# MCG-NJU/SparseBEV

Hardware: AMD Instinct MI355X
Metric: decoder samples/sec (6-cam T=8 900q r50_704x256, 6 layers, features resident in HBM) (higher is better)
Workload: dtype f32 (the two mixing GEMMs: f16x3 = fp32-class (default): fp32 operands as scaled fp16 hi + lo images, 3 products (hl, lh, hh), f32 accumulate on the 16-bit matrix core (csrc/gemm_bf16s.hip); max and rms error vs fp64 below the exact f32 MFMA kernels (tests/test_gpu_bf16s.py); mixing generator + out-; 1 GPU; c2: r50_704x256, 900 queries, T=8, bs=1 per GPU, 6 decoder layers, random-init weights, NCHW (reference layout, relayout inside the step: on demand -- only the feature units the sample points read) feature input; global_batch=1, parallelism=sample-sharded x1, launches_per_layer=6, query_order=False, shuffled_queries=False, relayout=on-demand

## Files before the change

### include/sbev_hip.h

```cpp
#ifndef SBEV_HIP_H
#define SBEV_HIP_H

#include <stdint.h>

#ifdef __cplusplus
extern "C" {
#endif

#define SBEV_ABI_VERSION 1
#define SBEV_MAX_LEVELS 5
#define SBEV_MAX_POINTS 32
#define SBEV_MAX_FRAMES 16

typedef void* sbev_stream_t;

enum sbev_status {
    SBEV_OK = 0,
    SBEV_EINVAL = -1,
    SBEV_ELAUNCH = -2,
    SBEV_ENODEV = -3,
    SBEV_EFAULT = -4
};

enum sbev_dtype { SBEV_F32 = 0, SBEV_BF16 = 1, SBEV_F16 = 2, SBEV_U8 = 3 };
// ... 108 lines not shown
int sbev_adaptive_mixing_f32(const float* x, const float* params, float* y,
                             int64_t BQ, int G, int Pin, int C, int Pout, float eps, sbev_stream_t stream);

int sbev_sasa_f32(const float* qkvt, int64_t ld, const float* query_bbox, const double* pc_range,
                  const uint8_t* mask, float* out, int B, int Q, int H, int head_dim, sbev_stream_t stream);

int sbev_refine_bbox(const float* query_bbox, const float* reg, const float* vel_div, float* out,
                     int B, int Q, int code_size, sbev_stream_t stream);


int sbev_head_prepare(const float* init_query_bbox, const float* label_row, float* query_bbox, float* query_feat,
                      int B, int Q, int D, sbev_stream_t stream);

int sbev_head_denorm(const float* bbox_norm, const double* pc_range, float* out, int64_t n, sbev_stream_t stream);

int sbev_nms_free_decode(const float* cls_scores, const float* bbox_preds, int B, int Q, int num_classes, int max_num,
                         float score_threshold, int use_score_threshold, const double* post_center_range,
                         int bottom_center, float* boxes, float* scores, int32_t* labels, int32_t* count,
                         sbev_stream_t stream);


int sbev_head_dn_prepare(const float* init_query_bbox, const float* label_enc, const float* gt_boxes, const int32_t* gt_labels,
                         const int32_t* gt_offsets, const float* u_box, const float* u_lab, const int32_t* new_lab,
                         const double* pc_range, float box_noise_scale, float label_noise_scale, int B, int Q, int D,
                         int num_classes, int G, int N, int single, float* query_bbox, float* query_feat,
                         int32_t* noised_label, uint8_t* attn_mask, sbev_stream_t stream);

int sbev_head_dn_prepare_bwd(const float* grad_query_bbox, const float* grad_query_feat, const int32_t* noised_label,
                             const int32_t* gt_offsets, int B, int Q, int D, int num_classes, int G, int N, int single,
                             float* grad_init_query_bbox, float* grad_label_enc, sbev_stream_t stream);

int sbev_head_match_cost(const float* cls_scores, const float* bbox_preds, int64_t ld_rows, const float* gt_boxes,
                         const int32_t* gt_labels, const int32_t* gt_offsets, const float* code_weights, float w_cls,
                         float w_reg, float alpha, float gamma, int L, int B, int Q, int num_classes, int Gmax, float* cost,
                         sbev_stream_t stream);

int sbev_lsa_solve(const float* cost, int64_t ld, int n_rows, int n_cols, int32_t* col_of_row);

int sbev_head_assign(const float* cost, const int32_t* gt_counts, int L, int B, int Q, int Gmax, int32_t* assign);

int64_t sbev_head_assign_device_workspace(int L, int B, int Q, int Gmax);
int sbev_head_assign_device_plan(int Q, int Gmax);
int sbev_head_assign_device(const float* cost, const int32_t* gt_offsets, int L, int B, int Q, int Gmax,
                            int32_t* assign, int32_t* status, void* workspace, sbev_stream_t stream);

int sbev_head_capacity_plan(const int32_t* gt_offsets, int B, int Q, int capacity, int N, double bg_cls_weight, int32_t* codes,
                            float* avg_factors, int32_t* status, sbev_stream_t stream);

#define SBEV_OPTIM_CHUNK 8192
#define SBEV_OPTIM_MAX_TENSORS 64
#define SBEV_OPTIM_MAX_GROUPS 16
#define SBEV_OPTIM_HYPER_FLOATS 68
#define SBEV_OPTIM_HEADER_BYTES 64
int sbev_optim_plan(const int64_t* numel, int n, int64_t* out);
int sbev_optim_sumsq(const void* const* g, const int64_t* numel, int n, const float* hyper, float* partials, sbev_stream_t stream);
int sbev_optim_finish(const float* partials, int64_t n_partials, const float* hyper, void* header, double beta1, double beta2,
                      sbev_stream_t stream);
int sbev_optim_adamw(void* const* p, const void* const* g, void* const* m, void* const* v, const int64_t* numel, const int32_t* group,
                     int n, int n_groups, double beta1, double beta2, double eps, const float* hyper, const void* header,
                     sbev_stream_t stream);

int64_t sbev_head_set_loss_workspace(int B, int rows);

int sbev_head_set_loss(const float* cls_scores, const float* bbox_preds, int64_t ld_rows, const int32_t* codes,
                       int64_t code_layer_stride, const float* gt_boxes, const int32_t* gt_labels, const int32_t* gt_offsets,
                       const float* code_weights, const float* avg_factors, float w_focal, float alpha, float gamma,
                       float w_l1, float scale, int L, int B, int rows, int num_classes, float* loss, float* loss_finite,
                       float* grad_cls, float* grad_bbox, float* workspace, sbev_stream_t stream);


int sbev_nchw_to_nhwc_f32(const float* in, float* out, int64_t n_images, int channels, int hw, sbev_stream_t stream);

int sbev_nchw_to_nhwc_f32_indirect(const void* const* table, int index, float* out, int64_t n_images, int channels, int hw,
                                   sbev_stream_t stream);
int sbev_nchw_to_nhwc_f32_multi_indirect(const void* const* table, int n_levels, const int32_t* index, float* const* out,
                                         int64_t n_images, int channels, const int32_t* hw, sbev_stream_t stream);
int sbev_nchw_to_nhwc_b16(const void* in, void* out, int64_t n_images, int channels, int hw, sbev_stream_t stream);
int sbev_nchw_to_nhwc_b16_indirect(const void* const* table, int index, void* out, int64_t n_images, int channels, int hw,
                                   sbev_stream_t stream);
int sbev_copy_indirect(const void* const* table, int nseg, const int32_t* index, void* const* dst, const int64_t* nbytes,
                       sbev_stream_t stream);

int sbev_finish_outputs(const float* cls_src, const float* box_src, float* cls_dst, float* box_dst, int64_t n_cls, int64_t n_box,
                        sbev_stream_t stream);
int sbev_finish_outputs_indirect(const void* const* table, int idx_cls, int idx_box, const float* cls_src, const float* box_src,
                                 int64_t n_cls, int64_t n_box, sbev_stream_t stream);


int sbev_linear3_ln_relu_f32(const float* x, int64_t ldx, const float* w, const float* b,
                             const float* ln_w, const float* ln_b, float eps, float* y,
                             int64_t M, int N, sbev_stream_t stream);

int sbev_splitk_reduce_f32(const float* slabs, int splits, const float* bias, const float* residual,
                           const float* ln_w, const float* ln_b, float ln_eps, float* Y,
                           int64_t M, int N, int relu, sbev_stream_t stream);

int sbev_split_bf16x3_weights(const float* W, uint16_t* W2, int64_t N, int K, sbev_stream_t stream);
int sbev_linear_bf16x3(const float* X, const uint16_t* W2, const float* bias, const float* residual, float* Y,
                       int64_t M, int N, int K, int64_t ldx, int64_t ldy, int relu, sbev_stream_t stream);
int sbev_linear_bf16x3_strip_ok(int64_t M, int N, int K);
int sbev_linear_bf16x3_strip(const uint16_t* X2, const uint16_t* W2, const float* bias, float* Y, int64_t M, int N, int K,
                             int64_t ldy, int relu, sbev_stream_t stream);
int sbev_linear_splitk_bf16x3(const float* X, const uint16_t* W2, const float* bias, const float* residual,
                              const float* ln_w, const float* ln_b, float ln_eps, float* Y,
                              int64_t M, int N, int K, int64_t ldx, int relu, int splits, float* workspace,
                              sbev_stream_t stream);

int64_t sbev_bf16s_image_elems(int64_t rows, int K, int nimg);
int sbev_split_bf16s_rows(const float* X, int64_t ldx, uint16_t* out, int64_t rows, int K, int nimg, sbev_stream_t stream);
int sbev_pack_bf16s_frags(const float* W, int64_t ldw, uint16_t* out, int N, int K, int nimg, sbev_stream_t stream);
int sbev_linear_bf16s_gen_ok(int64_t M, int N, int K);
int sbev_linear_bf16s_gen(const uint16_t* Xs, const uint16_t* Ws, const float* bias, float* Y, int64_t M, int N, int K,
                          int64_t ldy, int relu, int nimg, sbev_stream_t stream);
int sbev_linear_bf16s_out_ok(int64_t M, int N, int K);
int sbev_linear_bf16s_out_plan(int64_t M, int N, int K);
int sbev_linear_gen_plan(int64_t M, int N, int K, int64_t ldy, int nimg, int weight_stationary, int cus, int32_t* out, int capacity);
int sbev_linear_splitk_bf16s(const float* X, const uint16_t* Wp, const float* bias, const float* residual,
                             const float* ln_w, const float* ln_b, float ln_eps, float* Y,
                             int64_t M, int N, int K, int64_t ldx, int relu, int nimg, float* workspace,
                             sbev_stream_t stream);

int sbev_pack_f16s_frags(const float* W, int64_t ldw, uint16_t* out, float* scales, int N, int K, int per_tensor, sbev_stream_t stream);
int sbev_linear_f16s_gen(const uint16_t* Xs, const float* xscale, const uint16_t* Ws, const float* wdown, const float* bias, float* Y,
                         int64_t M, int N, int K, int64_t ldy, int relu, int nprod, sbev_stream_t stream);

int sbev_linear_gen_weight_stationary(int enable);

int sbev_linear_splitk_f16s(const float* X, int x_is_pairs, int x_up_log2, const uint16_t* Wp, const float* nscale, const float* bias, const float* residual,
                            const float* ln_w, const float* ln_b, float ln_eps, float* Y,
                            int64_t M, int N, int K, int64_t ldx, int relu, int nprod, float* workspace, sbev_stream_t stream);
int sbev_f16s_out_scale(const float* wdown, int x_up_log2, float* nscale, int N, sbev_stream_t stream);
int sbev_linear_splitk_f16s_xdev(const float* X, const float* x_scale, const uint16_t* Wp, const float* wdown, const float* bias,
                                 const float* residual, const float* ln_w, const float* ln_b, float ln_eps, float* Y,
                                 int64_t M, int N, int K, int64_t ldx, int relu, int nprod, float* workspace, sbev_stream_t stream);
int sbev_f16s_pairs(const float* X, void* out, int64_t n, int up_log2, sbev_stream_t stream);
int sbev_f16s_tensor_scale(const float* X, int64_t ldx, int64_t rows, int K, float* updown, sbev_stream_t stream);
int sbev_adaptive_mixing_pairs_f16(const float* x, const float* params, void* y, int64_t BQ, int G, int Pin, int Cg, int Pout, float eps,
                                   int up_log2, sbev_stream_t stream);
int sbev_sample_mix_pairs_f16(const void* const* feats, const int32_t* hw, int L, int feat_dtype,
                              int64_t B, int N, int Q, int T, int G, int P, int Cg,
                              const int64_t* stride_bo, int64_t stride_g, const int64_t* stride_v, int64_t stride_px,
                              const float* loc, const float* weights, const int32_t* frame_slots, int n_slots,
                              const float* params, void* y, int Pout, float eps, int up_log2, sbev_stream_t stream);

int sbev_copy_widen_f32(const void* src, int src_dtype, float* dst, int64_t n, sbev_stream_t stream);

int sbev_sample_mix_supported(int L, int C, int P, int T, int gdiv, int G);
int sbev_sample_mix_slabs_ok(const int32_t* hw, int L, int feat_dtype, int N, int C, const int64_t* stride_v, int64_t stride_px);
int sbev_sample_mix_f32(const void* const* feats, const int32_t* hw, int L, int feat_dtype,
                        int64_t B, int N, int Q, int T, int G, int P, int C,
                        const int64_t* stride_bo, int64_t stride_g, const int64_t* stride_v, int64_t stride_px,
                        const float* loc, const float* weights, const int32_t* frame_slots, int n_slots,
                        const float* params, float* y, int Pout, float eps, sbev_stream_t stream);
int sbev_decoder_fuse_sample_mix(int enable);

int sbev_query_order_max(void);
int sbev_query_order(const float* query_bbox, int64_t ld, const double* pc_range, int B, int Q, int32_t* order, sbev_stream_t stream);
int sbev_sample_mix_f32_ordered(const void* const* feats, const int32_t* hw, int L, int feat_dtype,
                                int64_t B, int N, int Q, int T, int G, int P, int C,
                                const int64_t* stride_bo, int64_t stride_g, const int64_t* stride_v, int64_t stride_px,
                                const float* loc, const float* weights, const int32_t* frame_slots, int n_slots,
                                const float* params, float* y, int Pout, float eps, const int32_t* order, sbev_stream_t stream);
int sbev_sample_mix_pairs_f16_ordered(const void* const* feats, const int32_t* hw, int L, int feat_dtype,
                                      int64_t B, int N, int Q, int T, int G, int P, int Cg,
                                      const int64_t* stride_bo, int64_t stride_g, const int64_t* stride_v, int64_t stride_px,
                                      const float* loc, const float* weights, const int32_t* frame_slots, int n_slots,
                                      const float* params, void* y, int Pout, float eps, int up_log2, const int32_t* order,
                                      sbev_stream_t stream);
int sbev_decoder_query_order(int enable);
int sbev_sample_mix_pool(const void* const* feats, const int32_t* hw, int L, int feat_dtype,
                         int64_t B, int N, int Q, int T, int G, int P, int C,
                         const int64_t* stride_bo, int64_t stride_g, const int64_t* stride_v, int64_t stride_px,
                         const float* loc, const float* weights, const int32_t* frame_slots, const int32_t* slot_table_dev, int n_slots,
                         const float* params, void* y, int Pout, float eps, int y_pairs, int up_log2, const int32_t* order,
                         sbev_stream_t stream);


int64_t sbev_gemm_f32_workspace(int64_t M, int N, int64_t K);
int sbev_gemm_f32(const float* A, int a_kmajor, int64_t lda, const float* B, int b_kmajor, int64_t ldb,
                  float* C, int64_t ldc, int64_t M, int N, int64_t K, int accumulate,
                  float* workspace, sbev_stream_t stream);
int64_t sbev_gemm_f32_multi_workspace(int64_t M, int N, int64_t K, int nseg);
int sbev_gemm_f32_multi(const float* const* A, int a_kmajor, int64_t lda, const float* const* B, int b_kmajor, int64_t ldb,
                        int nseg, float* C, int64_t ldc, int64_t M, int N, int64_t K, int accumulate,
                        float* workspace, sbev_stream_t stream);

int sbev_gemm_tn_f16s_ok(int64_t M, int64_t N, int64_t K);
int sbev_gemm_tn_f16s(const float* A, int64_t lda, const float* a_scale, const float* B, int64_t ldb, const float* b_scale,
                      float* C, int64_t ldc, int64_t M, int64_t N, int64_t K, int accumulate, sbev_stream_t stream);

int64_t sbev_colsum_workspace(int64_t M, int N);
int sbev_bias_relu_bwd(const float* dY, const float* Y, float* dZ, float* db, int64_t M, int N, int64_t ld,
                       float* workspace, sbev_stream_t stream);

int64_t sbev_layer_norm_bwd_workspace(int64_t M, int N);
int sbev_layer_norm_bwd(const float* dY, const float* X, const float* gamma, const float* beta, float eps, int relu,
                        float* dX, float* dgamma, float* dbeta, float* workspace, int64_t M, int N, sbev_stream_t stream);
int sbev_layer_norm_bwd_rows(const float* dY, const float* X, const float* gamma, const float* beta, float eps, int relu,
                             float* dX, float* workspace, int64_t M, int N, sbev_stream_t stream);
int sbev_layer_norm_param_group(const float* const* dYs, const float* const* Xs, const float* const* stats,
                                const float* const* gammas, const float* const* betas, float* const* dgammas, float* const* dbetas,
                                const int32_t* Ns, const int32_t* nsegs, const int32_t* relus, const int32_t* accumulate,
                                int ng, int64_t M, sbev_stream_t stream);
int sbev_colsum_group(const float* const* segs, float* const* outs, const int32_t* Ns, const int32_t* nsegs,
                      const int32_t* accumulate, int ng, int64_t M, sbev_stream_t stream);
int sbev_bias_relu_bwd_acc(const float* dY, const float* Y, float* dZ, float* db, int64_t M, int N, int64_t ld,
                           float* workspace, int accumulate, sbev_stream_t stream);
int sbev_layer_norm_bwd_acc(const float* dY, const float* X, const float* gamma, const float* beta, float eps, int relu,
                            float* dX, float* dgamma, float* dbeta, float* workspace, int64_t M, int N, int accumulate, sbev_stream_t stream);

int sbev_linear3_ln_relu_ex_f32(const float* x, int64_t ldx, const float* w, const float* b,
                                const float* ln_w, const float* ln_b, float eps, float* y, float* pre,
                                int64_t M, int N, sbev_stream_t stream);

int sbev_adaptive_mixing_bwd_f32(const float* x, const float* params, const float* grad_y, float* grad_x, float* grad_params,
                                 int64_t BQ, int G, int Pin, int C, int Pout, float eps, sbev_stream_t stream);
int sbev_adaptive_mixing_bwd_max_f32(const float* x, const float* params, const float* grad_y, float* grad_x, float* grad_params,
                                     float* item_max, int64_t BQ, int G, int Pin, int C, int Pout, float eps, sbev_stream_t stream);

int sbev_sasa_train_fwd_f32(const float* qkvt, int64_t ld, const float* query_bbox, const double* pc_range,
                            const uint8_t* mask, float* out, int B, int Q, int H, int head_dim,
                            float attn_drop, uint64_t seed, sbev_stream_t stream);
int sbev_sasa_bwd_f32(const float* qkvt, int64_t ld, const float* query_bbox, const double* pc_range,
                      const uint8_t* mask, const float* out, const float* grad_out, float* grad_qkvt,
                      float* workspace, int B, int Q, int H, int head_dim, float attn_drop, uint64_t seed,
                      sbev_stream_t stream);

int sbev_msmv_bwd_ex(const void* const* feats, void* const* grad_feats, const int32_t* hw, int L,
                     int64_t Bp, int N, int C, int Q, int P,
                     int gdiv, const int64_t* stride_bo, int64_t stride_g, const int64_t* stride_v, int64_t stride_px,
                     const float* loc, const float* weights, const float* grad_out, int grad_out_layout, int T, int G,
                     float* grad_loc, float* grad_weights, sbev_stream_t stream);

int64_t sbev_msmv_bwd_tap_count(int64_t Bp, int Q, int P, int L);
int sbev_msmv_bwd_taps(const void* const* feats, const int32_t* hw, int L,
                       int64_t Bp, int N, int C, int Q, int P,
                       int gdiv, const int64_t* stride_bo, int64_t stride_g, const int64_t* stride_v, int64_t stride_px,
                       const float* loc, const float* weights, int64_t* keys, float* coefs, sbev_stream_t stream);
int sbev_msmv_bwd_sum_sorted(void* const* grad_feats, int L, const int64_t* sorted_keys, const int64_t* order,
                             const float* coefs, int64_t n, const float* grad_out, int grad_out_layout,
                             int64_t Bp, int C, int Q, int P, int T, int G, sbev_stream_t stream);

int sbev_project_select_bwd(const float* sample_points, const float* lidar2img, const float* grad_loc,
                            int B, int Q, int T, int N, int G, int P, float image_h, float image_w, float eps,
                            float* grad_points, sbev_stream_t stream);

int sbev_sampling_front_bwd(const float* query_bbox, const float* offset, int64_t ld_off, const float* logits, int64_t ld_logit,
                            const double* pc_range, int B, int Q, int T, int G, int P, int L,
                            const float* grad_points, const float* grad_weights_bp,
                            float* grad_offset, float* grad_logits, int64_t ld_grad, float* grad_bbox, sbev_stream_t stream);

int sbev_refine_bbox_bwd(const float* grad_out, const float* out, const float* query_bbox, const float* vel_div,
                         float* grad_reg, float* grad_bbox, int B, int Q, sbev_stream_t stream);

int sbev_dropout_f32(const float* x, float* y, int64_t n, uint64_t seed, float p, sbev_stream_t stream);

int sbev_sasa_train_fwd_f32_ds(const float* qkvt, int64_t ld, const float* query_bbox, const double* pc_range, const uint8_t* mask,
                               float* out, int B, int Q, int H, int head_dim, float attn_drop, uint64_t seed, const uint64_t* seed_dev,
                               sbev_stream_t stream);
int sbev_sasa_bwd_f32_ds(const float* qkvt, int64_t ld, const float* query_bbox, const double* pc_range, const uint8_t* mask,
                         const float* out, const float* grad_out, float* grad_qkvt, float* workspace, int B, int Q, int H, int head_dim,
                         float attn_drop, uint64_t seed, const uint64_t* seed_dev, sbev_stream_t stream);
int sbev_dropout_f32_ds(const float* x, float* y, int64_t n, uint64_t seed, const uint64_t* seed_dev, float p, sbev_stream_t stream);

typedef struct sbev_decoder_config {
    int32_t B, Q, T, N, G, P, L;
    int32_t D, H, ffn;
    int32_t num_classes, code_size, num_layers, out_points;
    int32_t attn_in_rows;
    int32_t feat_dtype;
    int32_t hw[SBEV_MAX_LEVELS][2];
    float image_h, image_w, eps_homo;
    int32_t gemm_mode;
    int32_t n_slots;
    int32_t frame_slots[SBEV_MAX_FRAMES];
    int32_t overlap;
    double pc_range[6];
    const int32_t* slot_table;
} sbev_decoder_config;

typedef struct sbev_decoder_weights {
    const float *pe0_w, *pe0_b, *pe1_g, *pe1_b, *pe3_w, *pe3_b, *pe4_g, *pe4_b;
    const float *attn_in_w, *attn_in_b;
    const float *attn_out_w, *attn_out_b;
    const float *samp_w, *samp_b;
    const float *pg_w, *pg_b, *op_w, *op_b;
    const uint16_t *pg_w2, *op_w2;
    const float *ffn0_w, *ffn0_b, *ffn1_w, *ffn1_b;
    const float *norm1_g, *norm1_b, *norm2_g, *norm2_b, *norm3_g, *norm3_b;
    const float *cls0_w, *cls0_b, *cls1_g, *cls1_b, *cls3_w, *cls3_b, *cls4_g, *cls4_b, *cls6_w, *cls6_b;
    const float *reg0_w, *reg0_b, *reg2_w, *reg2_b, *reg4_w, *reg4_b;
    const float *chain_pack;
    const uint16_t *pg_ws;
    const uint16_t *op_wp;
    const float *pg_wdown;
    const float *op_nscale;
    const float *pg_xscale;
} sbev_decoder_weights;

int64_t sbev_decoder_chain_pack_floats(const sbev_decoder_config* cfg);
int sbev_decoder_chain_pack(const sbev_decoder_config* cfg, const sbev_decoder_weights* weights, float* out, sbev_stream_t stream);
int sbev_decoder_row_chain(int enable);
int sbev_decoder_chain_plan(const sbev_decoder_config* cfg, int kind, int with_front, int pair_ok, int cus, int32_t* out, int capacity);

int sbev_decoder_chain_pair(int enable);
int64_t sbev_decoder_chain_pair_timeouts(void);
int64_t sbev_decoder_chain_pair_faults(void);
int64_t sbev_decoder_chain_pair_faults_ack(void);
int sbev_decoder_out_fold(int enable);
int sbev_linear_out8_min_rows(int rows);
int sbev_debug_out_fold_drop(int enable);
int sbev_init(void);
int sbev_debug_chain_pair_drop(int enable);

int sbev_decoder_launches_per_layer(const sbev_decoder_config* cfg, const sbev_decoder_weights* weights);

int sbev_decoder_switches(int32_t* out, int capacity);

int sbev_decoder_mixed_up_log2(const sbev_decoder_config* cfg);

int64_t sbev_decoder_workspace_bytes(const sbev_decoder_config* cfg);

int sbev_decoder_forward(const sbev_decoder_config* cfg, const sbev_decoder_weights* weights,
                         const void* const* feats_nhwc, const float* query_bbox, const float* query_feat,
                         const float* time_diff, const float* lidar2img, const float* vel_div,
                         const uint8_t* attn_mask, float* cls_out, float* bbox_out,
                         void* workspace, int64_t workspace_bytes, sbev_stream_t stream);

typedef struct sbev_lazy_feats {
    const void* const* table;
    int32_t index[SBEV_MAX_LEVELS];
    const void* src[SBEV_MAX_LEVELS];
} sbev_lazy_feats;
int sbev_decoder_lazy_supported(const sbev_decoder_config* cfg);
int sbev_decoder_lazy_scan_launch(int enable);
int sbev_decoder_forward_lazy(const sbev_decoder_config* cfg, const sbev_decoder_weights* weights, void* const* feats_nhwc,
                              const sbev_lazy_feats* lazy, const float* query_bbox, const float* query_feat,
                              const float* time_diff, const float* lidar2img, const float* vel_div,
                              const uint8_t* attn_mask, float* cls_out, float* bbox_out,
                              void* workspace, int64_t workspace_bytes, sbev_stream_t stream);
int64_t sbev_prefix_cache_bytes(const sbev_decoder_config* cfg);
int sbev_decoder_forward_cached(const sbev_decoder_config* cfg, const sbev_decoder_weights* weights, void* const* feats_nhwc,
                                const sbev_lazy_feats* lazy, const float* query_bbox, const float* query_feat,
                                const float* time_diff, const float* lidar2img, const float* vel_div,
                                const uint8_t* attn_mask, float* cls_out, float* bbox_out,
                                void* workspace, int64_t workspace_bytes, sbev_stream_t stream, void* cache, int64_t cache_bytes);
int sbev_decoder_prefix_planned(const sbev_decoder_config* cfg, const sbev_decoder_weights* weights, int cache_given, int mask_given,
                                int lazy_given);
int64_t sbev_lazy_relayout_tiles(int n_levels, const int32_t* hw_pixels, int64_t n_images, int channels);
int sbev_sample_and_project_touch(const float* query_bbox, const float* offset, int64_t ld_offset,
                                  const float* scale_logits, int64_t ld_logits,
                                  const float* time_diff, const float* lidar2img, const double* pc_range,
                                  int B, int Q, int T, int N, int G, int P, int L,
                                  float image_h, float image_w, float eps,
                                  float* loc_bp, float* weights_bp, const int32_t* hw, uint32_t* need, sbev_stream_t stream);
int sbev_nchw_to_nhwc_lazy(const void* const* table, const int32_t* index, const void* const* src, void* const* out, int n_levels,
                           const int32_t* hw_pixels, int64_t n_images, int channels, int dtype, uint32_t* need, uint32_t* done, int first,
                           int last, sbev_stream_t stream);

typedef struct sbev_graph sbev_graph;
int sbev_decoder_capture(const sbev_decoder_config* cfg, const sbev_decoder_weights* weights,
                         const void* const* feats_nhwc, const float* query_bbox, const float* query_feat,
                         const float* time_diff, const float* lidar2img, const float* vel_div,
                         const uint8_t* attn_mask, float* cls_out, float* bbox_out,
                         void* workspace, int64_t workspace_bytes, sbev_stream_t stream, sbev_graph** out);
int sbev_capture_begin(sbev_stream_t stream);
int sbev_capture_end(sbev_stream_t stream, sbev_graph** out);
int sbev_graph_launch(sbev_graph* graph, sbev_stream_t stream);
int64_t sbev_graph_num_nodes(const sbev_graph* graph);
int sbev_graph_destroy(sbev_graph* graph);

int sbev_profile_sampler(int enable);
int sbev_profile_sampler_read(float* ms, int max_n);
int sbev_profile_stride(int every_n_calls);
int sbev_profile_read(int kind, float* ms, int max_n);

enum sbev_frames_layout { SBEV_FRAMES_NCHW = 0, SBEV_FRAMES_NHWC = 1 };
int sbev_pool_insert_frames(const void* const* table, const int32_t* index, const void* const* src, void* const* out, int n_frames,
                            int n_levels, const int32_t* hw_pixels, int B, int n_views, int channels, int src_layout, int src_dtype,
                            int dst_dtype, const int32_t* insert, int n_slots, sbev_stream_t stream);

int sbev_pool_insert(const void* const* table, const int32_t* index, const void* const* src, void* const* out, int n_levels,
                     const int32_t* hw_pixels, int B, int n_views, int channels, int dtype, const int32_t* insert, int n_slots,
                     sbev_stream_t stream);

#define SBEV_FRONT_ROW_BYTES 64
int sbev_image_front_plan(int n, int H, int W, int div, int64_t* out);
int sbev_image_front(const void* src, int src_dtype, void* dst, int dst_dtype, int n, int H, int W, int div, const float* mean,
                     const float* std, int to_rgb, int colour_on, const void* table, sbev_stream_t stream);

#define SBEV_GEOM_KMAX 16
int sbev_image_geom_plan(int H, int W, int fH, int fW, int resize_w, int resize_h, int crop_x, int crop_y, int flip, int32_t* table_out,
                         int64_t* out);
int sbev_image_geom(const void* src, void* dst, int n, int H, int W, int fH, int fW, const void* table, const void* image_rows,
                    int n_transforms, sbev_stream_t stream);

#define SBEV_FPN_MAX_IN 4
#define SBEV_FPN_MAX_OUT 5
#define SBEV_FPN_PLAN_WORDS 18
int sbev_fpn_plan(int n_levels, const int32_t* chw, int64_t n, int num_outs, int64_t* out);
int sbev_fpn_pack_weights(int n_levels, const int32_t* chw, const void* const* lateral_w, const void* const* fpn_w, int w_dtype, void* pack,
                          sbev_stream_t stream);
int sbev_fpn_forward(int n_levels, const int32_t* chw, int64_t n, int num_outs, const void* const* inputs, int in_dtype, const void* pack,
                     const float* const* lateral_bias, const float* const* fpn_bias, void* workspace, void* const* outs, int out_dtype,
                     sbev_stream_t stream);

#define SBEV_FPN_GRAD_WINDOW_LOG2 3
#define SBEV_FPN_BWD_PLAN_WORDS 16
int sbev_fpn_backward_plan(int n_levels, const int32_t* chw, int64_t n, int num_outs, int want_input_grads, int64_t* out);
int sbev_fpn_pack_weights_bwd(int n_levels, const int32_t* chw, const void* const* lateral_w, const void* const* fpn_w, int w_dtype,
                              void* pack, sbev_stream_t stream);
int sbev_fpn_backward(int n_levels, const int32_t* chw, int64_t n, int num_outs, const void* const* inputs, int in_dtype,
                      const void* merged, const void* const* grad_outs, int g_dtype, const void* pack_bwd, void* workspace,
                      void* const* grad_inputs, float* const* grad_lateral_w, float* const* grad_lateral_bias, float* const* grad_fpn_w,
                      float* const* grad_fpn_bias, sbev_stream_t stream);

#define SBEV_RESNET_MAX_LAYERS 160
#define SBEV_RESNET_PLAN_HEAD 18
#define SBEV_RESNET_LAYER_WORDS 12
#define SBEV_RESNET_PLAN_WORDS (SBEV_RESNET_PLAN_HEAD + SBEV_RESNET_LAYER_WORDS * SBEV_RESNET_MAX_LAYERS)
int sbev_resnet_plan(int depth, const int32_t* stage_blocks, int num_stages, int base_channels, int64_t n, int H, int W, int n_out,
                     const int32_t* out_indices, int keep, int64_t* out);
int sbev_resnet_pack_weights(int n_layers, const int32_t* desc, const void* const* w, const float* const* gamma, const float* const* beta,
                             const float* const* mean, const float* const* var, float eps, int w_dtype, void* pack, sbev_stream_t stream);
int sbev_conv_f16(const void* x, const void* pack, const void* residual, void* y, int64_t n, int H, int W, int Cin, int Cout, int taps,
                  int stride, int epilogue, int col_tile, sbev_stream_t stream);
int sbev_resnet_forward(int depth, const int32_t* stage_blocks, int num_stages, int base_channels, int64_t n, int H, int W, int n_out,
                        const int32_t* out_indices, int keep, const void* x, int x_dtype, const void* pack, void* workspace,
                        void* const* outs, sbev_stream_t stream);

#define SBEV_RESNET_GRAD_WINDOW_LOG2 3
#define SBEV_RESNET_BWD_PLAN_HEAD 16
#define SBEV_RESNET_BWD_LAYER_WORDS 6
#define SBEV_RESNET_BWD_PLAN_WORDS (SBEV_RESNET_BWD_PLAN_HEAD + SBEV_RESNET_BWD_LAYER_WORDS * SBEV_RESNET_MAX_LAYERS)
int sbev_resnet_backward_plan(int depth, const int32_t* stage_blocks, int num_stages, int base_channels, int64_t n, int H, int W, int n_out,
                              const int32_t* out_indices, int first_trainable_stage, int64_t* out);
int sbev_resnet_forward_train(int depth, const int32_t* stage_blocks, int num_stages, int base_channels, int64_t n, int H, int W, int n_out,
                              const int32_t* out_indices, int first_trainable_stage, const void* x, int x_dtype, const void* pack,
                              void* workspace, void* acts, void* const* outs, sbev_stream_t stream);
int sbev_resnet_pack_weights_bwd(int n_layers, const int32_t* desc, const void* const* w, const float* const* gamma, const float* const* var,
                                 float eps, int w_dtype, void* pack, sbev_stream_t stream);
int sbev_resnet_backward(int depth, const int32_t* stage_blocks, int num_stages, int base_channels, int64_t n, int H, int W, int n_out,
                         const int32_t* out_indices, int first_trainable_stage, const void* acts, const void* const* outs,
                         const void* const* grad_outs, int g_dtype, const void* pack_bwd, void* workspace, const void* const* w, int w_dtype,
                         const float* const* gamma, const float* const* mean, const float* const* var, float eps, float* const* grad_w,
                         float* const* grad_gamma, float* const* grad_beta, sbev_stream_t stream);
int sbev_conv_dgrad_f16(const void* gy, const void* gy2, const void* pack, const void* mask, const void* res, const void* gp, int gp_dtype,
                        const float* scale, void* gx, int64_t n, int H, int W, int Cin, int Cout, int taps, int stride, int Cout2, int stride2,
                        int col_tile, sbev_stream_t stream);
int sbev_conv_wgrad_f16(const void* gy, const void* x, float* part, int64_t n, int H, int W, int Cin, int Cout, int taps, int stride,
                        int slab_len, sbev_stream_t stream);
int sbev_bn_fold_backward(const float* part, int slabs, const float* scale, const void* w, int w_dtype, const float* gamma, const float* mean,
                          const float* var, float eps, int Cin, int Cout, int taps, float* grad_w, float* grad_gamma, float* grad_beta,
                          sbev_stream_t stream);

#ifdef __cplusplus
}
#endif
#endif
```

### sparsebev_amd/_lib.py

```python
import ctypes
import os

import torch

_HERE = os.path.dirname(os.path.abspath(__file__))
LIB_PATH = os.environ.get('SBEV_LIB_PATH') or os.path.join(_HERE, 'csrc', 'libsbev_hip.so')

_c_i64p = ctypes.POINTER(ctypes.c_int64)
_c_i32p = ctypes.POINTER(ctypes.c_int32)
_vp = ctypes.c_void_p

SIGNATURES = {
    'sbev_abi_version': (ctypes.c_int, []),
    'sbev_set_box_convention': (ctypes.c_int, [ctypes.c_int]),
    'sbev_get_box_convention': (ctypes.c_int, []),
    'sbev_last_error': (ctypes.c_char_p, []),
    'sbev_device_count': (ctypes.c_int, []),
    'sbev_msmv_fwd': (ctypes.c_int, [ctypes.POINTER(_vp), _c_i32p, ctypes.c_int, ctypes.c_int,
                                     ctypes.c_int64, ctypes.c_int, ctypes.c_int, ctypes.c_int, ctypes.c_int,
                                     ctypes.c_int, _c_i64p, ctypes.c_int64, _c_i64p, ctypes.c_int64,
                                     _vp, _vp, _vp, ctypes.c_int, ctypes.c_int, ctypes.c_int, _vp]),
    'sbev_project_select': (ctypes.c_int, [_vp, _vp, ctypes.c_int, ctypes.c_int, ctypes.c_int, ctypes.c_int,
                                           ctypes.c_int, ctypes.c_int, ctypes.c_float, ctypes.c_float, ctypes.c_float,
                                           _vp, _vp, _vp, _vp, _vp]),
    'sbev_sampling_front': (ctypes.c_int, [_vp, _vp, ctypes.c_int64, _vp, ctypes.c_int64, _vp, ctypes.POINTER(ctypes.c_double),
                                           ctypes.c_int, ctypes.c_int, ctypes.c_int, ctypes.c_int, ctypes.c_int, ctypes.c_int,
                                           _vp, _vp, _vp]),
    'sbev_linear_f32': (ctypes.c_int, [_vp, _vp, _vp, _vp, _vp, ctypes.c_int64, ctypes.c_int, ctypes.c_int,
                                       ctypes.c_int64, ctypes.c_int64, ctypes.c_int64, ctypes.c_int, _vp]),
    'sbev_linear_splitk_workspace': (ctypes.c_int64, [ctypes.c_int64, ctypes.c_int, ctypes.c_int]),
    'sbev_linear_splitk_f32': (ctypes.c_int, [_vp, _vp, _vp, _vp, _vp, _vp, ctypes.c_float, _vp,
                                              ctypes.c_int64, ctypes.c_int, ctypes.c_int, ctypes.c_int64, ctypes.c_int64,
                                              ctypes.c_int, ctypes.c_int, _vp, _vp]),
    'sbev_layer_norm_f32': (ctypes.c_int, [_vp, _vp, _vp, ctypes.c_float, _vp, _vp, ctypes.c_int64, ctypes.c_int,
                                           ctypes.c_int, _vp]),
    'sbev_ln_linear_f32': (ctypes.c_int, [_vp, _vp, _vp, ctypes.c_float, ctypes.c_int, _vp, _vp, _vp, _vp, _vp, _vp,
                                          ctypes.c_int64, ctypes.c_int, ctypes.c_int, ctypes.c_int64, ctypes.c_int64,
                                          ctypes.c_int, _vp]),
    'sbev_adaptive_mixing_f32': (ctypes.c_int, [_vp, _vp, _vp, ctypes.c_int64, ctypes.c_int, ctypes.c_int, ctypes.c_int,
                                                ctypes.c_int, ctypes.c_float, _vp]),
    'sbev_sasa_f32': (ctypes.c_int, [_vp, ctypes.c_int64, _vp, ctypes.POINTER(ctypes.c_double), _vp, _vp,
                                     ctypes.c_int, ctypes.c_int, ctypes.c_int, ctypes.c_int, _vp]),
    'sbev_refine_bbox': (ctypes.c_int, [_vp, _vp, _vp, _vp, ctypes.c_int, ctypes.c_int, ctypes.c_int, _vp]),
    'sbev_nchw_to_nhwc_f32': (ctypes.c_int, [_vp, _vp, ctypes.c_int64, ctypes.c_int, ctypes.c_int, _vp]),
    'sbev_nchw_to_nhwc_f32_indirect': (ctypes.c_int, [_vp, ctypes.c_int, _vp, ctypes.c_int64, ctypes.c_int, ctypes.c_int, _vp]),
    'sbev_nchw_to_nhwc_f32_multi_indirect': (ctypes.c_int, [_vp, ctypes.c_int, _c_i32p, ctypes.POINTER(_vp), ctypes.c_int64, ctypes.c_int, _c_i32p, _vp]),
    'sbev_nchw_to_nhwc_b16': (ctypes.c_int, [_vp, _vp, ctypes.c_int64, ctypes.c_int, ctypes.c_int, _vp]),
    'sbev_nchw_to_nhwc_b16_indirect': (ctypes.c_int, [_vp, ctypes.c_int, _vp, ctypes.c_int64, ctypes.c_int, ctypes.c_int, _vp]),
    'sbev_copy_indirect': (ctypes.c_int, [_vp, ctypes.c_int, _c_i32p, ctypes.POINTER(_vp), _c_i64p, _vp]),
    'sbev_finish_outputs': (ctypes.c_int, [_vp, _vp, _vp, _vp, ctypes.c_int64, ctypes.c_int64, _vp]),
    'sbev_finish_outputs_indirect': (ctypes.c_int, [_vp, ctypes.c_int, ctypes.c_int, _vp, _vp, ctypes.c_int64, ctypes.c_int64, _vp]),
    'sbev_linear3_ln_relu_f32': (ctypes.c_int, [_vp, ctypes.c_int64, _vp, _vp, _vp, _vp, ctypes.c_float, _vp,
                                                ctypes.c_int64, ctypes.c_int, _vp]),
    'sbev_decoder_workspace_bytes': (ctypes.c_int64, [_vp]),
    'sbev_decoder_launches_per_layer': (ctypes.c_int, [_vp, _vp]),
    'sbev_decoder_switches': (ctypes.c_int, [_c_i32p, ctypes.c_int]),
    'sbev_decoder_forward': (ctypes.c_int, [_vp, _vp, ctypes.POINTER(_vp), _vp, _vp, _vp, _vp, _vp, _vp, _vp, _vp,
                                            _vp, ctypes.c_int64, _vp]),
    'sbev_decoder_forward_lazy': (ctypes.c_int, [_vp, _vp, ctypes.POINTER(_vp), _vp, _vp, _vp, _vp, _vp, _vp, _vp, _vp, _vp,
                                                 _vp, ctypes.c_int64, _vp]),
    'sbev_decoder_forward_cached': (ctypes.c_int, [_vp, _vp, ctypes.POINTER(_vp), _vp, _vp, _vp, _vp, _vp, _vp, _vp, _vp, _vp,
                                                   _vp, ctypes.c_int64, _vp, _vp, ctypes.c_int64]),
    'sbev_prefix_cache_bytes': (ctypes.c_int64, [_vp]),
    'sbev_decoder_prefix_planned': (ctypes.c_int, [_vp, _vp, ctypes.c_int, ctypes.c_int, ctypes.c_int]),
    'sbev_decoder_lazy_supported': (ctypes.c_int, [_vp]),
    'sbev_decoder_lazy_scan_launch': (ctypes.c_int, [ctypes.c_int]),
    'sbev_lazy_relayout_tiles': (ctypes.c_int64, [ctypes.c_int, _c_i32p, ctypes.c_int64, ctypes.c_int]),
    'sbev_sample_and_project_touch': (ctypes.c_int, [_vp, _vp, ctypes.c_int64, _vp, ctypes.c_int64, _vp, _vp,
                                                     ctypes.POINTER(ctypes.c_double), ctypes.c_int, ctypes.c_int, ctypes.c_int,
                                                     ctypes.c_int, ctypes.c_int, ctypes.c_int, ctypes.c_int,
                                                     ctypes.c_float, ctypes.c_float, ctypes.c_float, _vp, _vp, _c_i32p, _vp, _vp]),
    'sbev_nchw_to_nhwc_lazy': (ctypes.c_int, [_vp, _c_i32p, ctypes.POINTER(_vp), ctypes.POINTER(_vp), ctypes.c_int, _c_i32p, ctypes.c_int64,
                                              ctypes.c_int, ctypes.c_int, _vp, _vp, ctypes.c_int, ctypes.c_int, _vp]),
    'sbev_init': (ctypes.c_int, []),
    'sbev_decoder_out_fold': (ctypes.c_int, [ctypes.c_int]),
    'sbev_linear_out8_min_rows': (ctypes.c_int, [ctypes.c_int]),
    'sbev_debug_out_fold_drop': (ctypes.c_int, [ctypes.c_int]),
    'sbev_profile_sampler': (ctypes.c_int, [ctypes.c_int]),
    'sbev_profile_stride': (ctypes.c_int, [ctypes.c_int]),
    'sbev_profile_sampler_read': (ctypes.c_int, [ctypes.POINTER(ctypes.c_float), ctypes.c_int]),
    'sbev_splitk_reduce_f32': (ctypes.c_int, [_vp, ctypes.c_int, _vp, _vp, _vp, _vp, ctypes.c_float, _vp, ctypes.c_int64,
                                              ctypes.c_int, ctypes.c_int, _vp]),
    'sbev_split_bf16x3_weights': (ctypes.c_int, [_vp, _vp, ctypes.c_int64, ctypes.c_int, _vp]),
    'sbev_linear_bf16x3_strip_ok': (ctypes.c_int, [ctypes.c_int64, ctypes.c_int, ctypes.c_int]),
    'sbev_linear_bf16x3_strip': (ctypes.c_int, [_vp, _vp, _vp, _vp, ctypes.c_int64, ctypes.c_int, ctypes.c_int, ctypes.c_int64,
                                                ctypes.c_int, _vp]),
    'sbev_linear_bf16x3': (ctypes.c_int, [_vp, _vp, _vp, _vp, _vp, ctypes.c_int64, ctypes.c_int, ctypes.c_int,
                                          ctypes.c_int64, ctypes.c_int64, ctypes.c_int, _vp]),
    'sbev_linear_splitk_bf16x3': (ctypes.c_int, [_vp, _vp, _vp, _vp, _vp, _vp, ctypes.c_float, _vp, ctypes.c_int64, ctypes.c_int,
                                                 ctypes.c_int, ctypes.c_int64, ctypes.c_int, ctypes.c_int, _vp, _vp]),
    'sbev_bf16s_image_elems': (ctypes.c_int64, [ctypes.c_int64, ctypes.c_int, ctypes.c_int]),
    'sbev_split_bf16s_rows': (ctypes.c_int, [_vp, ctypes.c_int64, _vp, ctypes.c_int64, ctypes.c_int, ctypes.c_int, _vp]),
    'sbev_pack_bf16s_frags': (ctypes.c_int, [_vp, ctypes.c_int64, _vp, ctypes.c_int, ctypes.c_int, ctypes.c_int, _vp]),
    'sbev_linear_gen_weight_stationary': (ctypes.c_int, [ctypes.c_int]),
    'sbev_linear_bf16s_gen_ok': (ctypes.c_int, [ctypes.c_int64, ctypes.c_int, ctypes.c_int]),
    'sbev_linear_bf16s_gen': (ctypes.c_int, [_vp, _vp, _vp, _vp, ctypes.c_int64, ctypes.c_int, ctypes.c_int, ctypes.c_int64,
                                             ctypes.c_int, ctypes.c_int, _vp]),
    'sbev_decoder_mixed_up_log2': (ctypes.c_int, [_vp]),
    'sbev_pack_f16s_frags': (ctypes.c_int, [_vp, ctypes.c_int64, _vp, _vp, ctypes.c_int, ctypes.c_int, ctypes.c_int, _vp]),
    'sbev_linear_f16s_gen': (ctypes.c_int, [_vp, _vp, _vp, _vp, _vp, _vp, ctypes.c_int64, ctypes.c_int, ctypes.c_int, ctypes.c_int64,
                                            ctypes.c_int, ctypes.c_int, _vp]),
    'sbev_f16s_pairs': (ctypes.c_int, [_vp, _vp, ctypes.c_int64, ctypes.c_int, _vp]),
    'sbev_f16s_tensor_scale': (ctypes.c_int, [_vp, ctypes.c_int64, ctypes.c_int64, ctypes.c_int, _vp, _vp]),
    'sbev_gemm_tn_f16s_ok': (ctypes.c_int, [ctypes.c_int64, ctypes.c_int64, ctypes.c_int64]),
    'sbev_gemm_tn_f16s': (ctypes.c_int, [_vp, ctypes.c_int64, _vp, _vp, ctypes.c_int64, _vp, _vp, ctypes.c_int64,
                                         ctypes.c_int64, ctypes.c_int64, ctypes.c_int64, ctypes.c_int, _vp]),
    'sbev_adaptive_mixing_bwd_max_f32': (ctypes.c_int, [_vp, _vp, _vp, _vp, _vp, _vp, ctypes.c_int64, ctypes.c_int, ctypes.c_int, ctypes.c_int,
                                                        ctypes.c_int, ctypes.c_float, _vp]),
    'sbev_adaptive_mixing_pairs_f16': (ctypes.c_int, [_vp, _vp, _vp, ctypes.c_int64, ctypes.c_int, ctypes.c_int, ctypes.c_int, ctypes.c_int,
                                                      ctypes.c_float, ctypes.c_int, _vp]),
    'sbev_linear_splitk_f16s': (ctypes.c_int, [_vp, ctypes.c_int, ctypes.c_int, _vp, _vp, _vp, _vp, _vp, _vp, ctypes.c_float, _vp, ctypes.c_int64, ctypes.c_int,
                                               ctypes.c_int, ctypes.c_int64, ctypes.c_int, ctypes.c_int, _vp, _vp]),
    'sbev_f16s_out_scale': (ctypes.c_int, [_vp, ctypes.c_int, _vp, ctypes.c_int, _vp]),
    'sbev_linear_splitk_f16s_xdev': (ctypes.c_int, [_vp, _vp, _vp, _vp, _vp, _vp, _vp, _vp, ctypes.c_float, _vp, ctypes.c_int64, ctypes.c_int,
                                                    ctypes.c_int, ctypes.c_int64, ctypes.c_int, ctypes.c_int, _vp, _vp]),
    'sbev_linear_bf16s_out_ok': (ctypes.c_int, [ctypes.c_int64, ctypes.c_int, ctypes.c_int]),
    'sbev_linear_bf16s_out_plan': (ctypes.c_int, [ctypes.c_int64, ctypes.c_int, ctypes.c_int]),
    'sbev_linear_gen_plan': (ctypes.c_int, [ctypes.c_int64, ctypes.c_int, ctypes.c_int, ctypes.c_int64, ctypes.c_int, ctypes.c_int, ctypes.c_int,
                                            _c_i32p, ctypes.c_int]),
    'sbev_linear_splitk_bf16s': (ctypes.c_int, [_vp, _vp, _vp, _vp, _vp, _vp, ctypes.c_float, _vp, ctypes.c_int64, ctypes.c_int,
                                                ctypes.c_int, ctypes.c_int64, ctypes.c_int, ctypes.c_int, _vp, _vp]),
    'sbev_msmv_bwd': (ctypes.c_int, [ctypes.POINTER(_vp), ctypes.POINTER(_vp), _c_i32p, ctypes.c_int,
                                     ctypes.c_int64, ctypes.c_int, ctypes.c_int, ctypes.c_int, ctypes.c_int,
                                     ctypes.c_int, _c_i64p, ctypes.c_int64, _c_i64p, ctypes.c_int64,
                                     _vp, _vp, _vp, _vp, _vp, _vp]),
    'sbev_msmv_fwd_ring': (ctypes.c_int, [ctypes.POINTER(_vp), _c_i32p, ctypes.c_int, ctypes.c_int,
                                          ctypes.c_int64, ctypes.c_int, ctypes.c_int, ctypes.c_int, ctypes.c_int,
                                          ctypes.c_int, _c_i64p, ctypes.c_int64, _c_i64p, ctypes.c_int64,
                                          _vp, _vp, _vp, ctypes.c_int, ctypes.c_int, ctypes.c_int, _c_i32p, ctypes.c_int, _vp]),
    'sbev_msmv_fwd_pool': (ctypes.c_int, [ctypes.POINTER(_vp), _c_i32p, ctypes.c_int, ctypes.c_int,
                                          ctypes.c_int64, ctypes.c_int, ctypes.c_int, ctypes.c_int, ctypes.c_int,
                                          ctypes.c_int, _c_i64p, ctypes.c_int64, _c_i64p, ctypes.c_int64,
                                          _vp, _vp, _vp, ctypes.c_int, ctypes.c_int, ctypes.c_int, _vp, ctypes.c_int, _vp]),
    'sbev_sample_mix_pool': (ctypes.c_int, [ctypes.POINTER(_vp), _c_i32p, ctypes.c_int, ctypes.c_int,
                                            ctypes.c_int64, ctypes.c_int, ctypes.c_int, ctypes.c_int, ctypes.c_int, ctypes.c_int, ctypes.c_int,
                                            _c_i64p, ctypes.c_int64, _c_i64p, ctypes.c_int64, _vp, _vp, _c_i32p, _vp, ctypes.c_int,
                                            _vp, _vp, ctypes.c_int, ctypes.c_float, ctypes.c_int, ctypes.c_int, _vp, _vp]),
    'sbev_sample_and_project': (ctypes.c_int, [_vp, _vp, ctypes.c_int64, _vp, ctypes.c_int64, _vp, _vp,
                                               ctypes.POINTER(ctypes.c_double), ctypes.c_int, ctypes.c_int, ctypes.c_int,
                                               ctypes.c_int, ctypes.c_int, ctypes.c_int, ctypes.c_int,
                                               ctypes.c_float, ctypes.c_float, ctypes.c_float, _vp, _vp, _vp]),
    'sbev_decoder_capture': (ctypes.c_int, [_vp, _vp, ctypes.POINTER(_vp), _vp, _vp, _vp, _vp, _vp, _vp, _vp, _vp, _vp, ctypes.c_int64, _vp, _vp]),
    'sbev_capture_begin': (ctypes.c_int, [_vp]),
    'sbev_capture_end': (ctypes.c_int, [_vp, _vp]),
    'sbev_graph_launch': (ctypes.c_int, [_vp, _vp]),
    'sbev_graph_num_nodes': (ctypes.c_int64, [_vp]),
    'sbev_graph_destroy': (ctypes.c_int, [_vp]),
    'sbev_head_prepare': (ctypes.c_int, [_vp, _vp, _vp, _vp, ctypes.c_int, ctypes.c_int, ctypes.c_int, _vp]),
    'sbev_head_denorm': (ctypes.c_int, [_vp, ctypes.POINTER(ctypes.c_double), _vp, ctypes.c_int64, _vp]),
    'sbev_nms_free_decode': (ctypes.c_int, [_vp, _vp, ctypes.c_int, ctypes.c_int, ctypes.c_int, ctypes.c_int, ctypes.c_float, ctypes.c_int,
                                            ctypes.POINTER(ctypes.c_double), ctypes.c_int, _vp, _vp, _vp, _vp, _vp]),
    'sbev_head_dn_prepare': (ctypes.c_int, [_vp] * 8 + [ctypes.POINTER(ctypes.c_double), ctypes.c_float, ctypes.c_float] + [ctypes.c_int] * 7
                             + [_vp] * 5),
    'sbev_head_dn_prepare_bwd': (ctypes.c_int, [_vp] * 4 + [ctypes.c_int] * 7 + [_vp] * 3),
    'sbev_head_match_cost': (ctypes.c_int, [_vp, _vp, ctypes.c_int64, _vp, _vp, _vp, _vp] + [ctypes.c_float] * 4 + [ctypes.c_int] * 5 + [_vp, _vp]),
    'sbev_lsa_solve': (ctypes.c_int, [_vp, ctypes.c_int64, ctypes.c_int, ctypes.c_int, _vp]),
    'sbev_head_assign': (ctypes.c_int, [_vp, _vp, ctypes.c_int, ctypes.c_int, ctypes.c_int, ctypes.c_int, _vp]),
    'sbev_head_assign_device_workspace': (ctypes.c_int64, [ctypes.c_int] * 4),
    'sbev_head_assign_device_plan': (ctypes.c_int, [ctypes.c_int, ctypes.c_int]),
    'sbev_head_assign_device': (ctypes.c_int, [_vp, _vp, ctypes.c_int, ctypes.c_int, ctypes.c_int, ctypes.c_int, _vp, _vp, _vp, _vp]),
    'sbev_head_capacity_plan': (ctypes.c_int, [_vp] + [ctypes.c_int] * 4 + [ctypes.c_double] + [_vp] * 4),
    'sbev_head_set_loss_workspace': (ctypes.c_int64, [ctypes.c_int, ctypes.c_int]),
    'sbev_head_set_loss': (ctypes.c_int, [_vp, _vp, ctypes.c_int64, _vp, ctypes.c_int64, _vp, _vp, _vp, _vp, _vp] + [ctypes.c_float] * 5
                           + [ctypes.c_int] * 4 + [_vp] * 6),
    'sbev_optim_plan': (ctypes.c_int, [_c_i64p, ctypes.c_int, _c_i64p]),
    'sbev_optim_sumsq': (ctypes.c_int, [ctypes.POINTER(_vp), _c_i64p, ctypes.c_int, _vp, _vp, _vp]),
    'sbev_optim_finish': (ctypes.c_int, [_vp, ctypes.c_int64, _vp, _vp, ctypes.c_double, ctypes.c_double, _vp]),
    'sbev_optim_adamw': (ctypes.c_int, [ctypes.POINTER(_vp)] * 4 + [_c_i64p, _c_i32p, ctypes.c_int, ctypes.c_int] + [ctypes.c_double] * 3
                         + [_vp, _vp, _vp]),
    'sbev_image_front_plan': (ctypes.c_int, [ctypes.c_int] * 4 + [_c_i64p]),
    'sbev_image_front': (ctypes.c_int, [_vp, ctypes.c_int, _vp, ctypes.c_int] + [ctypes.c_int] * 4 + [ctypes.POINTER(ctypes.c_float)] * 2
                         + [ctypes.c_int, ctypes.c_int, _vp, _vp]),
    'sbev_image_geom_plan': (ctypes.c_int, [ctypes.c_int] * 9 + [_c_i32p, _c_i64p]),
    'sbev_image_geom': (ctypes.c_int, [_vp, _vp] + [ctypes.c_int] * 5 + [_vp, _vp, ctypes.c_int, _vp]),
    'sbev_fpn_plan': (ctypes.c_int, [ctypes.c_int, _c_i32p, ctypes.c_int64, ctypes.c_int, _c_i64p]),
    'sbev_fpn_pack_weights': (ctypes.c_int, [ctypes.c_int, _c_i32p, ctypes.POINTER(_vp), ctypes.POINTER(_vp), ctypes.c_int, _vp, _vp]),
    'sbev_fpn_forward': (ctypes.c_int, [ctypes.c_int, _c_i32p, ctypes.c_int64, ctypes.c_int, ctypes.POINTER(_vp), ctypes.c_int, _vp,
                                        ctypes.POINTER(_vp), ctypes.POINTER(_vp), _vp, ctypes.POINTER(_vp), ctypes.c_int, _vp]),
    'sbev_fpn_backward_plan': (ctypes.c_int, [ctypes.c_int, _c_i32p, ctypes.c_int64, ctypes.c_int, ctypes.c_int, _c_i64p]),
    'sbev_fpn_pack_weights_bwd': (ctypes.c_int, [ctypes.c_int, _c_i32p, ctypes.POINTER(_vp), ctypes.POINTER(_vp), ctypes.c_int, _vp, _vp]),
    'sbev_fpn_backward': (ctypes.c_int, [ctypes.c_int, _c_i32p, ctypes.c_int64, ctypes.c_int, ctypes.POINTER(_vp), ctypes.c_int, _vp,
                                         ctypes.POINTER(_vp), ctypes.c_int, _vp, _vp] + [ctypes.POINTER(_vp)] * 5 + [_vp]),
    'sbev_resnet_plan': (ctypes.c_int, [ctypes.c_int, _c_i32p, ctypes.c_int, ctypes.c_int, ctypes.c_int64, ctypes.c_int, ctypes.c_int,
                                        ctypes.c_int, _c_i32p, ctypes.c_int, _c_i64p]),
    'sbev_resnet_pack_weights': (ctypes.c_int, [ctypes.c_int, _c_i32p] + [ctypes.POINTER(_vp)] * 5 + [ctypes.c_float, ctypes.c_int, _vp, _vp]),
    'sbev_conv_f16': (ctypes.c_int, [_vp, _vp, _vp, _vp, ctypes.c_int64] + [ctypes.c_int] * 8 + [_vp]),
    'sbev_resnet_forward': (ctypes.c_int, [ctypes.c_int, _c_i32p, ctypes.c_int, ctypes.c_int, ctypes.c_int64, ctypes.c_int, ctypes.c_int,
                                           ctypes.c_int, _c_i32p, ctypes.c_int, _vp, ctypes.c_int, _vp, _vp, ctypes.POINTER(_vp), _vp]),
    'sbev_resnet_backward_plan': (ctypes.c_int, [ctypes.c_int, _c_i32p, ctypes.c_int, ctypes.c_int, ctypes.c_int64, ctypes.c_int, ctypes.c_int,
                                                 ctypes.c_int, _c_i32p, ctypes.c_int, _c_i64p]),
    'sbev_resnet_forward_train': (ctypes.c_int, [ctypes.c_int, _c_i32p, ctypes.c_int, ctypes.c_int, ctypes.c_int64, ctypes.c_int, ctypes.c_int,
                                                 ctypes.c_int, _c_i32p, ctypes.c_int, _vp, ctypes.c_int, _vp, _vp, _vp, ctypes.POINTER(_vp), _vp]),
    'sbev_resnet_pack_weights_bwd': (ctypes.c_int, [ctypes.c_int, _c_i32p] + [ctypes.POINTER(_vp)] * 3 + [ctypes.c_float, ctypes.c_int, _vp, _vp]),
    'sbev_resnet_backward': (ctypes.c_int, [ctypes.c_int, _c_i32p, ctypes.c_int, ctypes.c_int, ctypes.c_int64, ctypes.c_int, ctypes.c_int,
                                            ctypes.c_int, _c_i32p, ctypes.c_int, _vp, ctypes.POINTER(_vp), ctypes.POINTER(_vp), ctypes.c_int, _vp, _vp,
                                            ctypes.POINTER(_vp), ctypes.c_int] + [ctypes.POINTER(_vp)] * 3 + [ctypes.c_float] +
                                           [ctypes.POINTER(_vp)] * 3 + [_vp]),
    'sbev_conv_dgrad_f16': (ctypes.c_int, [_vp] * 6 + [ctypes.c_int, _vp, _vp, ctypes.c_int64] + [ctypes.c_int] * 9 + [_vp]),
    'sbev_conv_wgrad_f16': (ctypes.c_int, [_vp, _vp, _vp, ctypes.c_int64] + [ctypes.c_int] * 7 + [_vp]),
    'sbev_bn_fold_backward': (ctypes.c_int, [_vp, ctypes.c_int, _vp, _vp, ctypes.c_int, _vp, _vp, _vp, ctypes.c_float] + [ctypes.c_int] * 3 +
                                            [_vp] * 4),
    'sbev_profile_read': (ctypes.c_int, [ctypes.c_int, _vp, ctypes.c_int]),
    'sbev_linear_splitk_plan': (ctypes.c_int, [ctypes.c_int64, ctypes.c_int, ctypes.c_int]),
    'sbev_linear_f32_path': (ctypes.c_int, [ctypes.c_int64, ctypes.c_int, ctypes.c_int, ctypes.c_int64, ctypes.c_int, ctypes.c_int]),
    'sbev_linear_splitk_path': (ctypes.c_int, [ctypes.c_int64, ctypes.c_int, ctypes.c_int, ctypes.c_int, _c_i32p]),
    'sbev_linear_group_f32': (ctypes.c_int, [_vp, ctypes.c_int, _vp]),
    'sbev_copy_widen_f32': (ctypes.c_int, [_vp, ctypes.c_int, _vp, ctypes.c_int64, _vp]),
    'sbev_msmv_buffer_taps': (ctypes.c_int, [ctypes.c_int]),
    'sbev_sample_mix_supported': (ctypes.c_int, [ctypes.c_int] * 6),
    'sbev_sample_mix_slabs_ok': (ctypes.c_int, [_c_i32p, ctypes.c_int, ctypes.c_int, ctypes.c_int, ctypes.c_int, _c_i64p, ctypes.c_int64]),
    'sbev_sample_mix_f32': (ctypes.c_int, [ctypes.POINTER(_vp), _c_i32p, ctypes.c_int, ctypes.c_int,
                                           ctypes.c_int64, ctypes.c_int, ctypes.c_int, ctypes.c_int, ctypes.c_int, ctypes.c_int, ctypes.c_int,
                                           _c_i64p, ctypes.c_int64, _c_i64p, ctypes.c_int64, _vp, _vp, _c_i32p, ctypes.c_int,
                                           _vp, _vp, ctypes.c_int, ctypes.c_float, _vp]),
    'sbev_sample_mix_pairs_f16': (ctypes.c_int, [ctypes.POINTER(_vp), _c_i32p, ctypes.c_int, ctypes.c_int,
                                                 ctypes.c_int64, ctypes.c_int, ctypes.c_int, ctypes.c_int, ctypes.c_int, ctypes.c_int, ctypes.c_int,
                                                 _c_i64p, ctypes.c_int64, _c_i64p, ctypes.c_int64, _vp, _vp, _c_i32p, ctypes.c_int,
                                                 _vp, _vp, ctypes.c_int, ctypes.c_float, ctypes.c_int, _vp]),
    'sbev_decoder_fuse_sample_mix': (ctypes.c_int, [ctypes.c_int]),
    'sbev_query_order_max': (ctypes.c_int, []),
    'sbev_query_order': (ctypes.c_int, [_vp, ctypes.c_int64, ctypes.POINTER(ctypes.c_double), ctypes.c_int, ctypes.c_int, _vp, _vp]),
    'sbev_sample_mix_f32_ordered': (ctypes.c_int, [ctypes.POINTER(_vp), _c_i32p, ctypes.c_int, ctypes.c_int,
                                                   ctypes.c_int64, ctypes.c_int, ctypes.c_int, ctypes.c_int, ctypes.c_int, ctypes.c_int, ctypes.c_int,
                                                   _c_i64p, ctypes.c_int64, _c_i64p, ctypes.c_int64, _vp, _vp, _c_i32p, ctypes.c_int,
                                                   _vp, _vp, ctypes.c_int, ctypes.c_float, _vp, _vp]),
    'sbev_sample_mix_pairs_f16_ordered': (ctypes.c_int, [ctypes.POINTER(_vp), _c_i32p, ctypes.c_int, ctypes.c_int,
                                                         ctypes.c_int64, ctypes.c_int, ctypes.c_int, ctypes.c_int, ctypes.c_int, ctypes.c_int, ctypes.c_int,
                                                         _c_i64p, ctypes.c_int64, _c_i64p, ctypes.c_int64, _vp, _vp, _c_i32p, ctypes.c_int,
                                                         _vp, _vp, ctypes.c_int, ctypes.c_float, ctypes.c_int, _vp, _vp]),
    'sbev_decoder_query_order': (ctypes.c_int, [ctypes.c_int]),
    'sbev_decoder_chain_pack_floats': (ctypes.c_int64, [_vp]),
    'sbev_decoder_chain_pack': (ctypes.c_int, [_vp, _vp, _vp, _vp]),
    'sbev_decoder_chain_plan': (ctypes.c_int, [_vp, ctypes.c_int, ctypes.c_int, ctypes.c_int, ctypes.c_int, _c_i32p, ctypes.c_int]),
    'sbev_decoder_row_chain': (ctypes.c_int, [ctypes.c_int]),
    'sbev_decoder_chain_pair': (ctypes.c_int, [ctypes.c_int]),
    'sbev_decoder_chain_pair_timeouts': (ctypes.c_int64, []),
    'sbev_decoder_chain_pair_faults': (ctypes.c_int64, []),
    'sbev_decoder_chain_pair_faults_ack': (ctypes.c_int64, []),
    'sbev_debug_chain_pair_drop': (ctypes.c_int, [ctypes.c_int]),
    'sbev_gemm_f32_workspace': (ctypes.c_int64, [ctypes.c_int64, ctypes.c_int, ctypes.c_int64]),
    'sbev_gemm_f32': (ctypes.c_int, [_vp, ctypes.c_int, ctypes.c_int64, _vp, ctypes.c_int, ctypes.c_int64, _vp, ctypes.c_int64,
                                     ctypes.c_int64, ctypes.c_int, ctypes.c_int64, ctypes.c_int, _vp, _vp]),
    'sbev_colsum_workspace': (ctypes.c_int64, [ctypes.c_int64, ctypes.c_int]),
    'sbev_layer_norm_bwd_workspace': (ctypes.c_int64, [ctypes.c_int64, ctypes.c_int]),
    'sbev_gemm_f32_multi_workspace': (ctypes.c_int64, [ctypes.c_int64, ctypes.c_int, ctypes.c_int64, ctypes.c_int]),
    'sbev_gemm_f32_multi': (ctypes.c_int, [ctypes.POINTER(_vp), ctypes.c_int, ctypes.c_int64, ctypes.POINTER(_vp), ctypes.c_int, ctypes.c_int64,
                                           ctypes.c_int, _vp, ctypes.c_int64, ctypes.c_int64, ctypes.c_int, ctypes.c_int64, ctypes.c_int, _vp, _vp]),
    'sbev_layer_norm_bwd_rows': (ctypes.c_int, [_vp, _vp, _vp, _vp, ctypes.c_float, ctypes.c_int, _vp, _vp, ctypes.c_int64, ctypes.c_int, _vp]),
    'sbev_layer_norm_param_group': (ctypes.c_int, [ctypes.POINTER(_vp)] * 7 + [_c_i32p] * 4 + [ctypes.c_int, ctypes.c_int64, _vp]),
    'sbev_colsum_group': (ctypes.c_int, [ctypes.POINTER(_vp), ctypes.POINTER(_vp), _c_i32p, _c_i32p, _c_i32p, ctypes.c_int, ctypes.c_int64, _vp]),
    'sbev_bias_relu_bwd_acc': (ctypes.c_int, [_vp, _vp, _vp, _vp, ctypes.c_int64, ctypes.c_int, ctypes.c_int64, _vp, ctypes.c_int, _vp]),
    'sbev_layer_norm_bwd_acc': (ctypes.c_int, [_vp, _vp, _vp, _vp, ctypes.c_float, ctypes.c_int, _vp, _vp, _vp, _vp,
                                               ctypes.c_int64, ctypes.c_int, ctypes.c_int, _vp]),
    'sbev_bias_relu_bwd': (ctypes.c_int, [_vp, _vp, _vp, _vp, ctypes.c_int64, ctypes.c_int, ctypes.c_int64, _vp, _vp]),
    'sbev_layer_norm_bwd': (ctypes.c_int, [_vp, _vp, _vp, _vp, ctypes.c_float, ctypes.c_int, _vp, _vp, _vp, _vp,
                                           ctypes.c_int64, ctypes.c_int, _vp]),
    'sbev_linear3_ln_relu_ex_f32': (ctypes.c_int, [_vp, ctypes.c_int64, _vp, _vp, _vp, _vp, ctypes.c_float, _vp, _vp,
                                                   ctypes.c_int64, ctypes.c_int, _vp]),
    'sbev_adaptive_mixing_bwd_f32': (ctypes.c_int, [_vp, _vp, _vp, _vp, _vp, ctypes.c_int64, ctypes.c_int, ctypes.c_int, ctypes.c_int,
                                                    ctypes.c_int, ctypes.c_float, _vp]),
    'sbev_sasa_train_fwd_f32': (ctypes.c_int, [_vp, ctypes.c_int64, _vp, ctypes.POINTER(ctypes.c_double), _vp, _vp,
                                               ctypes.c_int, ctypes.c_int, ctypes.c_int, ctypes.c_int, ctypes.c_float, ctypes.c_uint64, _vp]),
    'sbev_sasa_bwd_f32': (ctypes.c_int, [_vp, ctypes.c_int64, _vp, ctypes.POINTER(ctypes.c_double), _vp, _vp, _vp, _vp, _vp,
                                         ctypes.c_int, ctypes.c_int, ctypes.c_int, ctypes.c_int, ctypes.c_float, ctypes.c_uint64, _vp]),
    'sbev_msmv_bwd_ex': (ctypes.c_int, [ctypes.POINTER(_vp), ctypes.POINTER(_vp), _c_i32p, ctypes.c_int,
                                        ctypes.c_int64, ctypes.c_int, ctypes.c_int, ctypes.c_int, ctypes.c_int,
                                        ctypes.c_int, _c_i64p, ctypes.c_int64, _c_i64p, ctypes.c_int64,
                                        _vp, _vp, _vp, ctypes.c_int, ctypes.c_int, ctypes.c_int, _vp, _vp, _vp]),
    'sbev_msmv_bwd_tap_count': (ctypes.c_int64, [ctypes.c_int64, ctypes.c_int, ctypes.c_int, ctypes.c_int]),
    'sbev_msmv_bwd_taps': (ctypes.c_int, [ctypes.POINTER(_vp), _c_i32p, ctypes.c_int,
                                          ctypes.c_int64, ctypes.c_int, ctypes.c_int, ctypes.c_int, ctypes.c_int,
                                          ctypes.c_int, _c_i64p, ctypes.c_int64, _c_i64p, ctypes.c_int64,
                                          _vp, _vp, _vp, _vp, _vp]),
    'sbev_msmv_bwd_sum_sorted': (ctypes.c_int, [ctypes.POINTER(_vp), ctypes.c_int, _vp, _vp, _vp, ctypes.c_int64, _vp, ctypes.c_int,
                                                ctypes.c_int64, ctypes.c_int, ctypes.c_int, ctypes.c_int, ctypes.c_int, ctypes.c_int, _vp]),
    'sbev_project_select_bwd': (ctypes.c_int, [_vp, _vp, _vp, ctypes.c_int, ctypes.c_int, ctypes.c_int, ctypes.c_int, ctypes.c_int,
                                               ctypes.c_int, ctypes.c_float, ctypes.c_float, ctypes.c_float, _vp, _vp]),
    'sbev_sampling_front_bwd': (ctypes.c_int, [_vp, _vp, ctypes.c_int64, _vp, ctypes.c_int64, ctypes.POINTER(ctypes.c_double),
                                               ctypes.c_int, ctypes.c_int, ctypes.c_int, ctypes.c_int, ctypes.c_int, ctypes.c_int,
                                               _vp, _vp, _vp, _vp, ctypes.c_int64, _vp, _vp]),
    'sbev_refine_bbox_bwd': (ctypes.c_int, [_vp, _vp, _vp, _vp, _vp, _vp, ctypes.c_int, ctypes.c_int, _vp]),
    'sbev_dropout_f32': (ctypes.c_int, [_vp, _vp, ctypes.c_int64, ctypes.c_uint64, ctypes.c_float, _vp]),
    'sbev_sasa_train_fwd_f32_ds': (ctypes.c_int, [_vp, ctypes.c_int64, _vp, ctypes.POINTER(ctypes.c_double), _vp, _vp,
                                                  ctypes.c_int, ctypes.c_int, ctypes.c_int, ctypes.c_int, ctypes.c_float, ctypes.c_uint64, _vp, _vp]),
    'sbev_sasa_bwd_f32_ds': (ctypes.c_int, [_vp, ctypes.c_int64, _vp, ctypes.POINTER(ctypes.c_double), _vp, _vp, _vp, _vp, _vp,
                                            ctypes.c_int, ctypes.c_int, ctypes.c_int, ctypes.c_int, ctypes.c_float, ctypes.c_uint64, _vp, _vp]),
    'sbev_dropout_f32_ds': (ctypes.c_int, [_vp, _vp, ctypes.c_int64, ctypes.c_uint64, _vp, ctypes.c_float, _vp]),
    'sbev_pool_insert_frames': (ctypes.c_int, [_vp, _c_i32p, ctypes.POINTER(_vp), ctypes.POINTER(_vp), ctypes.c_int, ctypes.c_int, _c_i32p, ctypes.c_int,
                                               ctypes.c_int, ctypes.c_int, ctypes.c_int, ctypes.c_int, ctypes.c_int, _vp, ctypes.c_int, _vp]),
    'sbev_pool_insert': (ctypes.c_int, [_vp, _c_i32p, ctypes.POINTER(_vp), ctypes.POINTER(_vp), ctypes.c_int, _c_i32p, ctypes.c_int, ctypes.c_int,
                                        ctypes.c_int, ctypes.c_int, _vp, ctypes.c_int, _vp]),
}

_lib = None


class SbevError(RuntimeError):
    """A libsbev_hip.so entry point returned a negative status (message from sbev_last_error())."""


def load():
    global _lib
    if _lib is not None:
        return _lib
    if not os.path.exists(LIB_PATH):
        try:
            from .csrc import build as _build
            _build.build()
        except Exception as e:
            raise ImportError(
                'sparsebev_amd: %s not found and building it failed (%s). Build it with `python -m sparsebev_amd.csrc.build` '
                '(needs hipcc, targets gfx950). There is no CPU / PyTorch fallback for this path.' % (LIB_PATH, e))
    lib = ctypes.CDLL(LIB_PATH)
    for name, (res, args) in SIGNATURES.items():
        fn = getattr(lib, name)
        fn.restype = res
        fn.argtypes = args
    if lib.sbev_abi_version() != 1:
        raise ImportError('sparsebev_amd: libsbev_hip.so ABI %d != 1 (stale build?)' % lib.sbev_abi_version())
    _lib = lib
    if torch.cuda.is_available() and torch.cuda.is_initialized():
        lib.sbev_init()
    return lib


class PairFaultError(SbevError):
    """SBEV_EFAULT: an EARLIER decoder step lost a pair-mode hand-off (the GPU was shared or preempted for about a second) -- that
    step's outputs are invalid.  By the time this is raised pair mode is off and the fault acknowledged: repeat the step(s) since
    the last result you synchronised on and verified with ``runtime.check_pair_faults()``."""


EFAULT = -4


def check(status, what):
    if status == EFAULT:
        from . import runtime
        msg = load().sbev_last_error().decode('utf-8', 'replace')
        runtime._on_pair_fault()
        raise PairFaultError('%s refused (%d): %s' % (what, status, msg))
    if status != 0:
        msg = load().sbev_last_error().decode('utf-8', 'replace')
        raise SbevError('%s failed (%d): %s' % (what, status, msg))
```

### sparsebev_amd/csrc/row_chain.hip

```cpp
#include "sbev_common.hpp"
#include "sample_point.hpp"
#include <atomic>
#include <cstdlib>

namespace {

constexpr int NWAVE = 8;
constexpr int DM = 256, FF = 512;
constexpr int LDX = DM + 8;
constexpr int LDH = FF + 8;
static_assert(2 * LDX >= LDH, "branch rows alias the ffn hidden rows");

constexpr int PV_OP_B = 0, PV_N2G = 256, PV_N2B = 512, PV_FFN0_B = 768, PV_FFN1_B = 1280, PV_N3G = 1536, PV_N3B = 1792,
              PV_CLS0_B = 2048, PV_CLS1G = 2304, PV_CLS1B = 2560, PV_CLS3_B = 2816, PV_CLS4G = 3072, PV_CLS4B = 3328,
              PV_CLS6_B = 3584, PV_REG0_B = 3648, PV_REG2_B = 3904, PV_REG4_B = 4160, PV_TAIL_END = 4224;
constexpr int PV_PE0_W = PV_TAIL_END, PV_PE0_B = PV_PE0_W + 768, PV_PE1G = PV_PE0_B + 256, PV_PE1B = PV_PE1G + 256,
              PV_PE3_B = PV_PE1B + 256, PV_PE4G = PV_PE3_B + 256, PV_PE4B = PV_PE4G + 256, PV_QKV_B = PV_PE4B + 256, PV_QKV_PAD = 832,
              PV_FRONT_END = PV_QKV_B + PV_QKV_PAD;
constexpr int PV_AOUT_B = 0, PV_N1G = 256, PV_N1B = 512, PV_SAMP_B = 768, PV_ATTN_END = 1024;
constexpr int PV_IMAGE_FLOATS = PV_FRONT_END + PV_ATTN_END;

enum Epi { EPI_FFN0, EPI_FFN1, EPI_BR1, EPI_BR2, EPI_OUT, EPI_PE3, EPI_QKV, EPI_AOUT, EPI_SAMP };
enum Pre { PRE_SLABS, PRE_FRONT, PRE_ATT };

struct Lin {
    const float* wp;
    int in_off, ld;
    int KH;
    int items;
    int chunks;
    int kh0, KHT;
};
struct Unit {
    Lin a, b;
    int epi;
    int col0;
};

#ifdef SBEV_CHAIN_TRACE
#define SBEV_TRACE(i) if ((blockIdx.x == 7 || blockIdx.x == 15) && lane == 0) a.trace[(blockIdx.x == 15 ? 64 * 512 : 0) + wave * 64 + (i)] = (long long)__builtin_amdgcn_s_memrealtime();
#else
#define SBEV_TRACE(i)
#endif

struct ChainArgs {
#ifdef SBEV_CHAIN_TRACE
    long long* trace;
#endif
    Unit units[8];
    Unit units_b[8];
    int n_units, pre, front;
    int n_pairs;
    float* pair_x;
    unsigned* pair_sync;
    unsigned* zero_words; int n_zero;
    int debug_drop;
    const float* warm;
    int warm_lines;
    const float* vec;
    int vec_off, vec_n;
    long long M;
    int Q;
    const float* slabs; int splits;
    const float* x1;
    float* x3;
    const float* bbox;
    const float* vel_div;
    float* cls_out;
    float* box_out;
    int num_classes;
    const float* feat;
    float* x;
    float* qkvt; int attn_in_rows;
    const float* att;
    float* x1_out;
    unsigned short* x1_frag;
    const float* x1_scale;
    float* so; int soN;
    sbev_ops::SamplePointArgs proj;
    float eps;
    uint32_t* skip_hdr;
};

constexpr int RING_SLOTS = 3;
constexpr int CHUNK_FLOATS = 1024;

template <int RG>
struct Lay {
    static constexpr int R = 4 * RG;
    static constexpr bool WIDE = RG > 1;
    static constexpr int MAX_SLOTS = WIDE ? 12 : 16;
    static constexpr int OFF_X2 = 0;
    static constexpr int OFF_X3 = OFF_X2 + R * LDX;
    static constexpr int OFF_H = OFF_X3 + R * LDX;
    static constexpr int OFF_C = OFF_H;
    static constexpr int OFF_R = OFF_H + R * LDX;
    static constexpr int OFF_P = OFF_H + 2 * R * LDX;
    static constexpr int LDS_FLOATS = OFF_P + MAX_SLOTS * R * 64;
    static constexpr int OFF_RING = LDS_FLOATS;
    static constexpr int OFF_DUMP = OFF_RING + (WIDE ? 0 : NWAVE * RING_SLOTS * CHUNK_FLOATS);
    static constexpr int OFF_PARAM = OFF_DUMP + NWAVE * 64;
    static constexpr int LDS_TOTAL_FLOATS = OFF_PARAM + PV_FRONT_END;
    static constexpr int RPW = (R + NWAVE - 1) / NWAVE;
    static_assert(LDS_TOTAL_FLOATS * 4 <= 160 * 1024, "LDS budget of one CU");
};
struct Offs { int x2, x3, h, c, r; };
template <int RG> constexpr Offs offs_of() { return Offs{Lay<RG>::OFF_X2, Lay<RG>::OFF_X3, Lay<RG>::OFF_H, Lay<RG>::OFF_C, Lay<RG>::OFF_R}; }

template <int RG>
__device__ __forceinline__ void warm_l2(const ChainArgs& a, int wave, int lane) {
    const int per_xcd = ((int)gridDim.x + 7) / 8;
    const int parts = per_xcd < 32 ? per_xcd : 32;
    const int part = ((int)blockIdx.x / 8) % parts;
    const int n = (a.warm_lines + parts - 1) / parts;
    const int l0 = part * n;
    const int l1 = min(a.warm_lines, l0 + n);
    const unsigned dump = (unsigned)(Lay<RG>::OFF_DUMP + wave * 64) * 4u;
    for (int l = l0 + wave * 64; l < l1; l += NWAVE * 64) {
        const int line = min(l + lane, l1 - 1);
        const unsigned voff = (unsigned)line * 128u;
        asm volatile(
            "s_mov_b32 m0, %0\n\t"
            "s_nop 0\n\t"
            "global_load_lds_dword %1, %2\n\t"
            :
            : "s"(dump), "v"(voff), "s"(a.warm)
            : "memory");
    }
}

struct Walk {
    int u, it, step;
};

__device__ __forceinline__ int unit_items(const Unit* U, int u) { return U[u].a.items + U[u].b.items; }

__device__ __forceinline__ void walk_settle(const ChainArgs& a, const Unit* U, Walk& w, int wave) {
    while (w.u < a.n_units && w.it >= unit_items(U, w.u)) {
        ++w.u;
        w.it = wave;
    }
}

__device__ __forceinline__ const float* item_weights(const Unit& un, int it) {
    const bool second = it >= un.a.items;
    const Lin& l = second ? un.b : un.a;
    const int j = it - (second ? un.a.items : 0);
    const int piece = l.KHT == l.KH ? j : (j / l.KH) * l.KHT + l.kh0 + j % l.KH;
    return l.wp + (long long)piece * (l.chunks * CHUNK_FLOATS);
}

__device__ __forceinline__ void issue_chunk(const float* g, unsigned lds_byte, unsigned voff) {
    asm volatile(
        "s_mov_b32 m0, %0\n\t"
        "s_nop 0\n\t"
        "global_load_lds_dwordx4 %1, %2\n\t"
        "global_load_lds_dwordx4 %1, %2 offset:1024\n\t"
        "global_load_lds_dwordx4 %1, %2 offset:2048\n\t"
        "global_load_lds_dwordx4 %1, %2 offset:3072\n\t"
        :
        : "s"(lds_byte), "v"(voff), "s"(g)
        : "memory");
}

struct Stream {
    const Unit* U;
    Walk iw;
    const float* g;
    int nchunk;
    int issued, used;
    int islot, uslot;
    unsigned ring_byte;
    unsigned voff;
};

__device__ __forceinline__ void stream_seek(const ChainArgs& a, Stream& st, int wave) {
    walk_settle(a, st.U, st.iw, wave);
    st.iw.step = 0;
    if (st.iw.u < a.n_units) {
        const Unit& un = st.U[st.iw.u];
        st.g = item_weights(un, st.iw.it);
        st.nchunk = st.iw.it >= un.a.items ? un.b.chunks : un.a.chunks;
    }
}

__device__ __forceinline__ void stream_issue(const ChainArgs& a, Stream& st, int wave) {
    if (st.iw.u >= a.n_units) return;
    issue_chunk(st.g + st.iw.step * CHUNK_FLOATS, st.ring_byte + (unsigned)st.islot * (CHUNK_FLOATS * 4), st.voff);
    ++st.issued;
    st.islot = st.islot == RING_SLOTS - 1 ? 0 : st.islot + 1;
    if (++st.iw.step == st.nchunk) {
        st.iw.it += NWAVE;
        stream_seek(a, st, wave);
    }
}

struct RChunk { float4 q[4]; };
__device__ __forceinline__ void stream_load(const ChainArgs& a, Stream& st, int wave, int lane, RChunk& c) {
    const float* g = st.g + st.iw.step * CHUNK_FLOATS + lane * 4;
#pragma unroll
    for (int m = 0; m < 4; ++m) c.q[m] = *reinterpret_cast<const float4*>(g + 256 * m);
    if (st.iw.u < a.n_units && ++st.iw.step == st.nchunk) {
        st.iw.it += NWAVE;
        stream_seek(a, st, wave);
    }
}
constexpr int RDEPTH = 4;

#define SBEV_MF(KK, BV) acc[(KK) & 1] = __builtin_amdgcn_mfma_f32_4x4x1f32(av, BV, acc[(KK) & 1], 4, KK, 0);
#define SBEV_MSTEP(m, q) SBEV_MF(4 * (m) + 0, q.x) SBEV_MF(4 * (m) + 1, q.y) SBEV_MF(4 * (m) + 2, q.z) SBEV_MF(4 * (m) + 3, q.w)

typedef float f32x4 __attribute__((ext_vector_type(4)));

__device__ __forceinline__ void mma_item(const ChainArgs& a, Stream& st, const Lin& l, int j, float* smem, int pslot, int lane, int wave) {
    constexpr int R = 4, OFF_RING = Lay<1>::OFF_RING, OFF_P = Lay<1>::OFF_P;
    f32x4 acc[2] = {{0.f, 0.f, 0.f, 0.f}, {0.f, 0.f, 0.f, 0.f}};
    const int kh = j % l.KH;
    const float* arow = smem + l.in_off + kh * 128 + (lane & 3) * l.ld + (lane >> 2);
    const float* ring = smem + OFF_RING + wave * (RING_SLOTS * CHUNK_FLOATS) + lane * 4;
    for (int s = 0; s < 8; ++s) {
        const int ahead = st.issued - st.used;
        if (ahead >= 3) asm volatile("s_waitcnt vmcnt(8)" ::: "memory");
        else if (ahead == 2) asm volatile("s_waitcnt vmcnt(4)" ::: "memory");
        else asm volatile("s_waitcnt vmcnt(0)" ::: "memory");
        const float av = arow[s * 16];
        const float* slot = ring + st.uslot * CHUNK_FLOATS;
        const float4 q0 = *reinterpret_cast<const float4*>(slot);
        const float4 q1 = *reinterpret_cast<const float4*>(slot + 256);
        const float4 q2 = *reinterpret_cast<const float4*>(slot + 512);
        const float4 q3 = *reinterpret_cast<const float4*>(slot + 768);
        asm volatile("s_waitcnt lgkmcnt(0)" ::: "memory");
        ++st.used;
        st.uslot = st.uslot == RING_SLOTS - 1 ? 0 : st.uslot + 1;
        stream_issue(a, st, wave);
        __builtin_amdgcn_sched_barrier(0);
        SBEV_MSTEP(0, q0) SBEV_MSTEP(1, q1) SBEV_MSTEP(2, q2) SBEV_MSTEP(3, q3)
    }
    const f32x4 t = acc[0] + acc[1];
    float* p = smem + OFF_P + pslot * (R * 64) + lane;
    p[0] = t.x; p[64] = t.y; p[128] = t.z; p[192] = t.w;
}

template <int RG>
__device__ __forceinline__ void mma_item_wide(const ChainArgs& a, Stream& st, RChunk (&rb)[RDEPTH], const Lin& l, int j, float* smem, int pslot,
                                              int lane, int wave) {
    constexpr int NACC = RG >= 4 ? 1 : 2;
    f32x4 acc[RG][NACC];
#pragma unroll
    for (int rg = 0; rg < RG; ++rg)
#pragma unroll
        for (int i = 0; i < NACC; ++i) acc[rg][i] = f32x4{0.f, 0.f, 0.f, 0.f};
    const int kh = l.kh0 + j % l.KH;
    const float* arow = smem + l.in_off + kh * (l.chunks * 16) + (lane & 3) * l.ld + (lane >> 2);
    float avn[RG];
#pragma unroll
    for (int rg = 0; rg < RG; ++rg) avn[rg] = arow[rg * 4 * l.ld];
    for (int s0 = 0; s0 < l.chunks; s0 += RDEPTH) {
#pragma unroll
        for (int d = 0; d < RDEPTH; ++d) {
            float av[RG];
            const int nxt = min(s0 + d + 1, l.chunks - 1);
#pragma unroll
            for (int rg = 0; rg < RG; ++rg) { av[rg] = avn[rg]; avn[rg] = arow[nxt * 16 + rg * 4 * l.ld]; }
            __builtin_amdgcn_sched_barrier(0);
#define SBEV_MW(KK, BV)                                                                                                     \
    _Pragma("unroll") for (int rg = 0; rg < RG; ++rg)                                                                        \
        acc[rg][(KK) % NACC] = __builtin_amdgcn_mfma_f32_4x4x1f32(av[rg], BV, acc[rg][(KK) % NACC], 4, KK, 0);
#define SBEV_MWSTEP(m, q) SBEV_MW(4 * (m) + 0, q.x) SBEV_MW(4 * (m) + 1, q.y) SBEV_MW(4 * (m) + 2, q.z) SBEV_MW(4 * (m) + 3, q.w)
            SBEV_MWSTEP(0, rb[d].q[0]) SBEV_MWSTEP(1, rb[d].q[1]) SBEV_MWSTEP(2, rb[d].q[2]) SBEV_MWSTEP(3, rb[d].q[3])
#undef SBEV_MWSTEP
#undef SBEV_MW
            __builtin_amdgcn_sched_barrier(0);
            stream_load(a, st, wave, lane, rb[d]);
        }
    }
    float* p = smem + Lay<RG>::OFF_P + pslot * (Lay<RG>::R * 64) + lane;
#pragma unroll
    for (int rg = 0; rg < RG; ++rg) {
        f32x4 t = acc[rg][0];
        if (NACC == 2) t += acc[rg][NACC - 1];
        p[(rg * 4 + 0) * 64] = t.x; p[(rg * 4 + 1) * 64] = t.y; p[(rg * 4 + 2) * 64] = t.z; p[(rg * 4 + 3) * 64] = t.w;
    }
}

__device__ __forceinline__ float wsum(float v) { return sbev::wave_sum_dpp(v); }

struct LnW {
    float g[4], b[4];
    __device__ __forceinline__ LnW(const float* gp, const float* bp, int lane) {
#pragma unroll
        for (int c = 0; c < 4; ++c) { g[c] = gp[lane + 64 * c]; b[c] = bp[lane + 64 * c]; }
    }
};
__device__ __forceinline__ void ln4(float (&v)[4], const LnW& w, float eps, bool relu) {
    const float mean = wsum((v[0] + v[1]) + (v[2] + v[3])) * (1.f / DM);
    float q = 0.f;
#pragma unroll
    for (int c = 0; c < 4; ++c) { const float d = v[c] - mean; q += d * d; }
    const float rstd = rsqrtf(wsum(q) * (1.f / DM) + eps);
#pragma unroll
    for (int c = 0; c < 4; ++c) {
        float o = (v[c] - mean) * rstd * w.g[c] + w.b[c];
        v[c] = relu ? fmaxf(o, 0.f) : o;
    }
}

template <int KH, int R>
__device__ __forceinline__ void gather4_t(float (&v)[4], const float* P, int base, int cg0, int row, int lane, const float* bias, int bias0) {
    float t[4][KH];
#pragma unroll
    for (int c = 0; c < 4; ++c)
#pragma unroll
        for (int kh = 0; kh < KH; ++kh) t[c][kh] = P[(base + (cg0 + c) * KH + kh) * (R * 64) + row * 64 + lane];
#pragma unroll
    for (int c = 0; c < 4; ++c) {
        float s = 0.f;
#pragma unroll
        for (int kh = 0; kh < KH; ++kh) s += t[c][kh];
        v[c] = s + bias[bias0 + lane + 64 * c];
    }
}
template <int R>
__device__ __forceinline__ void gather4(float (&v)[4], const float* P, int base, int KH, int cg0, int row, int lane, const float* bias,
                                        int bias0) {
    if (KH == 1) gather4_t<1, R>(v, P, base, cg0, row, lane, bias, bias0);
    else if (KH == 2) gather4_t<2, R>(v, P, base, cg0, row, lane, bias, bias0);
    else gather4_t<4, R>(v, P, base, cg0, row, lane, bias, bias0);
}

template <int R>
__device__ __forceinline__ void gather4_raw(float (&v)[4], const float* P, int KH, int row, int lane) {
#pragma unroll
    for (int c = 0; c < 4; ++c) {
        float s = 0.f;
        for (int kh = 0; kh < KH; ++kh) s += P[(c * KH + kh) * (R * 64) + row * 64 + lane];
        v[c] = s;
    }
}

__device__ unsigned g_chain_pair_timeouts;
__device__ unsigned* g_chain_pair_fault_host;
constexpr unsigned PAIR_POLL_LIMIT = 1u << 20;

__device__ __forceinline__ void pair_store4(float* p, const float (&v)[4]) {
    const f32x4 q = {v[0], v[1], v[2], v[3]};
    asm volatile("global_store_dwordx4 %0, %1, off sc0 sc1\n\ts_nop 1" ::"v"(p), "v"(q) : "memory");
}
__device__ __forceinline__ void pair_load4(const float* p, float (&v)[4]) {
    f32x4 q;
    asm volatile("global_load_dwordx4 %0, %1, off sc0 sc1\n\ts_waitcnt vmcnt(0)" : "=v"(q) : "v"(p) : "memory");
    v[0] = q.x; v[1] = q.y; v[2] = q.z; v[3] = q.w;
}
__device__ __forceinline__ void pair_arrive(unsigned* word) {
    asm volatile("s_waitcnt vmcnt(0)" ::: "memory");
    __syncthreads();
    if (threadIdx.x == 0) __hip_atomic_fetch_add(word, 1u, __ATOMIC_RELAXED, __HIP_MEMORY_SCOPE_AGENT);
}
__device__ __forceinline__ void pair_wait(unsigned* word, unsigned arrivals) {
    if (threadIdx.x == 0) {
        unsigned n = 0;
        while (__hip_atomic_load(word, __ATOMIC_RELAXED, __HIP_MEMORY_SCOPE_AGENT) < arrivals) {
            __builtin_amdgcn_s_sleep(2);
            if (++n > PAIR_POLL_LIMIT) {
                __hip_atomic_fetch_add(&g_chain_pair_timeouts, 1u, __ATOMIC_RELAXED, __HIP_MEMORY_SCOPE_AGENT);
                unsigned* const host_word = g_chain_pair_fault_host;
                if (host_word) __hip_atomic_fetch_add(host_word, 1u, __ATOMIC_RELAXED, __HIP_MEMORY_SCOPE_SYSTEM);
                break;
            }
        }
    }
    __syncthreads();
}

__device__ __forceinline__ void store_rows(float* smem, int off, int ld, int row, int lane, const float (&v)[4]) {
#pragma unroll
    for (int c = 0; c < 4; ++c) smem[off + row * ld + lane + 64 * c] = v[c];
}

template <int RG>
__device__ __forceinline__ void pe0_row(const ChainArgs& a, float* smem, int row, int lane, float x0, float x1, float x2) {
    constexpr int OFF_PARAM = Lay<RG>::OFF_PARAM, OFF_C = Lay<RG>::OFF_C;
    const float* pv = smem + OFF_PARAM;
    const LnW lw(pv + PV_PE1G, pv + PV_PE1B, lane);
    float v[4];
#pragma unroll
    for (int c = 0; c < 4; ++c) {
        const int n = lane + 64 * c;
        const float* w = pv + PV_PE0_W + n * 3;
        v[c] = ((x0 * w[0] + x1 * w[1]) + x2 * w[2]) + pv[PV_PE0_B + n];
    }
    ln4(v, lw, a.eps, true);
    store_rows(smem, OFF_C, LDX, row, lane, v);
}

template <int PRE, int RG, bool PAIR = false>
__global__ __launch_bounds__(64 * NWAVE) void row_chain_kernel(const ChainArgs a) {
    using L = Lay<RG>;
    static_assert(!PAIR || (PRE == PRE_SLABS && RG > 1), "pair mode: the tail, wide row blocks");
    constexpr int R = L::R, RPW = L::RPW, OFF_X2 = L::OFF_X2, OFF_X3 = L::OFF_X3, OFF_H = L::OFF_H, OFF_C = L::OFF_C, OFF_R = L::OFF_R,
                  OFF_P = L::OFF_P, OFF_PARAM = L::OFF_PARAM;
    extern __shared__ __attribute__((aligned(16))) float smem[];
    const int lane = threadIdx.x & 63;
    const int wave = __builtin_amdgcn_readfirstlane(threadIdx.x >> 6);
    int pair = (int)blockIdx.x, member = 0;
    if constexpr (PAIR) {
        const int li = (int)blockIdx.x >> 3;
        pair = (li >> 1) * 8 + ((int)blockIdx.x & 7);
        member = li & 1;
        if (pair >= a.n_pairs) return;
        if (a.debug_drop && pair == 0 && member == 1) return;
    }
    const Unit* const U = (PAIR && member) ? a.units_b : a.units;
    unsigned* const pword = PAIR ? a.pair_sync + pair : nullptr;
    float* const px = PAIR ? a.pair_x + (long long)pair * (3 * R * DM) : nullptr;
    const long long row0 = (long long)pair * R;
    float* P = smem + OFF_P;
    if constexpr (PRE == PRE_FRONT) {
        if (a.skip_hdr) {
            const bool clean = sbev::prefix_clean(a.skip_hdr);
            if (blockIdx.x == 0 && threadIdx.x == 0) {
                uint32_t* n = a.skip_hdr + (clean ? sbev::PFX_HITS : sbev::PFX_MISSES);
                *n = *n + 1u;
            }
            if (clean) return;
        }
    }
    if (PRE == PRE_ATT && a.zero_words && blockIdx.x == 0)
        for (int i = threadIdx.x; i < a.n_zero; i += 64 * NWAVE) a.zero_words[i] = 0u;

    SBEV_TRACE(0)
    warm_l2<RG>(a, wave, lane);
    Stream st;
    st.U = U;
    st.iw = Walk{0, wave, 0};
    st.issued = st.used = st.islot = st.uslot = 0;
    st.ring_byte = (unsigned)(L::OFF_RING + wave * (RING_SLOTS * CHUNK_FLOATS)) * 4u;
    st.voff = (unsigned)lane * 16u;
    st.g = a.warm;
    st.nchunk = 8;
    stream_seek(a, st, wave);
    RChunk rb[RDEPTH];
    if constexpr (L::WIDE) {
#pragma unroll
        for (int d = 0; d < RDEPTH; ++d) {
#pragma unroll
            for (int m = 0; m < 4; ++m) rb[d].q[m] = make_float4(0.f, 0.f, 0.f, 0.f);
            stream_load(a, st, wave, lane, rb[d]);
        }
    } else {
        stream_issue(a, st, wave);
        stream_issue(a, st, wave);
        stream_issue(a, st, wave);
    }

    const float* pv = smem + OFF_PARAM;
    constexpr int PASSES = (PV_FRONT_END / 4 + 64 * NWAVE - 1) / (64 * NWAVE);
    float4 pq[PASSES];
#pragma unroll
    for (int j = 0; j < PASSES; ++j) {
        const int i4 = (int)threadIdx.x + j * 64 * NWAVE;
        pq[j] = *reinterpret_cast<const float4*>(a.vec + 4 * min(i4, a.vec_n / 4 - 1));
    }
    float4 t[RPW], r4[RPW];
    float v0[RPW][4], v1[RPW][4];
    float bx[RPW], by[RPW], bz[RPW];
    bool plive[RPW];
#pragma unroll
    for (int pi = 0; pi < RPW; ++pi) {
        const int prow = wave + pi * NWAVE;
        const long long pg = row0 + prow;
        plive[pi] = prow < R && pg < a.M;
        t[pi] = make_float4(0.f, 0.f, 0.f, 0.f); r4[pi] = t[pi];
#pragma unroll
        for (int c = 0; c < 4; ++c) v0[pi][c] = v1[pi][c] = 0.f;
        bx[pi] = by[pi] = bz[pi] = 0.f;
        if (PRE == PRE_SLABS) {
            if (plive[pi]) r4[pi] = *reinterpret_cast<const float4*>(a.x1 + pg * DM + lane * 4);
        } else if (plive[pi]) {
            const float* src = PRE == PRE_FRONT ? a.feat : a.att;
#pragma unroll
            for (int c = 0; c < 4; ++c) v0[pi][c] = src[pg * DM + lane + 64 * c];
            if (PRE == PRE_FRONT) { bx[pi] = a.bbox[pg * 10]; by[pi] = a.bbox[pg * 10 + 1]; bz[pi] = a.bbox[pg * 10 + 2]; }
            if (PRE == PRE_ATT) {
#pragma unroll
                for (int c = 0; c < 4; ++c) v1[pi][c] = a.x[pg * DM + lane + 64 * c];
            }
        }
    }
    if (PRE == PRE_SLABS) {
        constexpr int NB = 32 / RPW;
        for (int z0 = 0; z0 < a.splits; z0 += NB) {
            float4 q[RPW][NB];
#pragma unroll
            for (int pi = 0; pi < RPW; ++pi) {
                const long long pg = min(row0 + wave + pi * NWAVE, a.M - 1);
#pragma unroll
                for (int j = 0; j < NB; ++j)
                    q[pi][j] = *reinterpret_cast<const float4*>(a.slabs + ((long long)min(z0 + j, a.splits - 1) * a.M + pg) * DM + lane * 4);
            }
#pragma unroll
            for (int pi = 0; pi < RPW; ++pi)
#pragma unroll
                for (int j = 0; j < NB; ++j) asm volatile("" ::"v"(q[pi][j].x), "v"(q[pi][j].y), "v"(q[pi][j].z), "v"(q[pi][j].w));
#pragma unroll
            for (int pi = 0; pi < RPW; ++pi)
#pragma unroll
                for (int j = 0; j < NB; ++j) {
                    const float m = (z0 + j < a.splits && plive[pi]) ? 1.f : 0.f;
                    t[pi].x += q[pi][j].x * m; t[pi].y += q[pi][j].y * m; t[pi].z += q[pi][j].z * m; t[pi].w += q[pi][j].w * m;
                }
        }
    }
#pragma unroll
    for (int j = 0; j < PASSES; ++j) asm volatile("" ::"v"(pq[j].x), "v"(pq[j].y), "v"(pq[j].z), "v"(pq[j].w));
#pragma unroll
    for (int j = 0; j < PASSES; ++j) {
        const int i4 = (int)threadIdx.x + j * 64 * NWAVE;
        if (i4 < a.vec_n / 4) *reinterpret_cast<float4*>(smem + OFF_PARAM + a.vec_off + 4 * i4) = pq[j];
    }
    __syncthreads();
#pragma unroll
    for (int pi = 0; pi < RPW; ++pi) {
        const int prow = wave + pi * NWAVE;
        if (prow >= R) continue;
        if (PRE == PRE_SLABS) {
            float4 tt = t[pi];
            const float4 rr = r4[pi];
            const float4 b4 = *reinterpret_cast<const float4*>(pv + PV_OP_B + lane * 4);
            if (plive[pi]) { tt.x = (tt.x + b4.x) + rr.x; tt.y = (tt.y + b4.y) + rr.y; tt.z = (tt.z + b4.z) + rr.z; tt.w = (tt.w + b4.w) + rr.w; }
            const float mean = wsum((tt.x + tt.y) + (tt.z + tt.w)) * (1.f / DM);
            const float dx = tt.x - mean, dy = tt.y - mean, dz = tt.z - mean, dw = tt.w - mean;
            const float rstd = rsqrtf(wsum((dx * dx + dy * dy) + (dz * dz + dw * dw)) * (1.f / DM) + a.eps);
            const float4 g4 = *reinterpret_cast<const float4*>(pv + PV_N2G + lane * 4);
            const float4 n4 = *reinterpret_cast<const float4*>(pv + PV_N2B + lane * 4);
            *reinterpret_cast<float4*>(smem + OFF_X2 + prow * LDX + lane * 4) =
                make_float4(dx * rstd * g4.x + n4.x, dy * rstd * g4.y + n4.y, dz * rstd * g4.z + n4.z, dw * rstd * g4.w + n4.w);
        } else {
            store_rows(smem, PRE == PRE_FRONT ? OFF_X3 : OFF_X2, LDX, prow, lane, v0[pi]);
            if (PRE == PRE_ATT) store_rows(smem, OFF_R, LDX, prow, lane, v1[pi]);
            if (PRE == PRE_FRONT) pe0_row<RG>(a, smem, prow, lane, bx[pi], by[pi], bz[pi]);
        }
    }
    __syncthreads();

    SBEV_TRACE(1)
    for (int u = 0; u < a.n_units; ++u) {
        const Unit& un = U[u];
        const int items = un.a.items + un.b.items;
        for (int it = wave; it < items; it += NWAVE) {
            const bool second = it >= un.a.items;
            if constexpr (L::WIDE) mma_item_wide<RG>(a, st, rb, second ? un.b : un.a, it - (second ? un.a.items : 0), smem, it, lane, wave);
            else mma_item(a, st, second ? un.b : un.a, it - (second ? un.a.items : 0), smem, it, lane, wave);
        }
        SBEV_TRACE(2 + 4 * u)
        __syncthreads();
        SBEV_TRACE(3 + 4 * u)
        if constexpr (PAIR) {
            if (un.epi == EPI_FFN1) {
                for (int row = wave; row < R; row += NWAVE) {
                    float v[4];
                    gather4_raw<R>(v, P, un.a.KH, row, lane);
                    pair_store4(px + (member * R + row) * DM + lane * 4, v);
                }
                pair_arrive(pword);
                pair_wait(pword, 2u);
            } else if (un.epi == EPI_PE3 && member == 0) {
                pair_wait(pword, 3u);
            }
        }
        for (int task = wave; task < 2 * R; task += NWAVE) {
            const int row = task % R, side = task / R;
            const long long g = row0 + row;
            const bool live = g < a.M;
            float v[4];
            if (PAIR && side != member && (un.epi == EPI_FFN0 || un.epi == EPI_BR1 || un.epi == EPI_BR2 || un.epi == EPI_OUT)) continue;
            switch (un.epi) {
            case EPI_FFN0: {
                gather4<R>(v, P, 0, un.a.KH, PAIR ? 0 : side * 4, row, lane, pv + PV_FFN0_B, side * 256);
#pragma unroll
                for (int c = 0; c < 4; ++c) smem[OFF_H + row * LDH + side * 256 + lane + 64 * c] = fmaxf(v[c], 0.f);
            } break;
            case EPI_FFN1: {
                if (side) break;
                const LnW lw(pv + PV_N3G, pv + PV_N3B, lane);
                float res[4];
#pragma unroll
                for (int c = 0; c < 4; ++c) res[c] = smem[OFF_X2 + row * LDX + lane + 64 * c];
                if constexpr (PAIR) {
                    float own[4], oth[4];
                    gather4_raw<R>(own, P, un.a.KH, row, lane);
                    pair_load4(px + ((1 - member) * R + row) * DM + lane * 4, oth);
#pragma unroll
                    for (int c = 0; c < 4; ++c) v[c] = ((member ? oth[c] : own[c]) + (member ? own[c] : oth[c])) + pv[PV_FFN1_B + lane + 64 * c];
                } else {
                    gather4<R>(v, P, 0, un.a.KH, 0, row, lane, pv + PV_FFN1_B, 0);
                }
#pragma unroll
                for (int c = 0; c < 4; ++c) v[c] += res[c];
                ln4(v, lw, a.eps, false);
                store_rows(smem, OFF_X3, LDX, row, lane, v);
                if (live && member == 0) {
#pragma unroll
                    for (int c = 0; c < 4; ++c) a.x3[g * DM + lane + 64 * c] = v[c];
                }
            } break;
            case EPI_BR1:
            case EPI_BR2: {
                const bool first = un.epi == EPI_BR1;
                if (side == 0) {
                    const LnW lw(pv + (first ? PV_CLS1G : PV_CLS4G), pv + (first ? PV_CLS1B : PV_CLS4B), lane);
                    gather4<R>(v, P, 0, un.a.KH, 0, row, lane, pv + (first ? PV_CLS0_B : PV_CLS3_B), 0);
                    ln4(v, lw, a.eps, true);
                    store_rows(smem, OFF_C, LDX, row, lane, v);
                } else {
                    gather4<R>(v, P, un.a.items, un.b.KH, 0, row, lane, pv + (first ? PV_REG0_B : PV_REG2_B), 0);
#pragma unroll
                    for (int c = 0; c < 4; ++c) v[c] = fmaxf(v[c], 0.f);
                    store_rows(smem, OFF_R, LDX, row, lane, v);
                }
            } break;
            case EPI_OUT: {
                if (side == 0) {
                    if (lane < a.num_classes) {
                        float s = 0.f;
                        for (int kh = 0; kh < un.a.KH; ++kh) s += P[kh * (R * 64) + row * 64 + lane];
                        if (live) a.cls_out[g * a.num_classes + lane] = s + pv[PV_CLS6_B + lane];
                    }
                } else {
                    float o = 0.f;
                    if (lane < 10) {
                        float s = 0.f;
                        for (int kh = 0; kh < un.b.KH; ++kh) s += P[(un.a.items + kh) * (R * 64) + row * 64 + lane];
                        const float r = s + pv[PV_REG4_B + lane];
                        const long long gi = live ? g : 0;
                        if (lane < 3) {
                            float p = a.bbox[gi * 10 + lane];
                            p = fminf(fmaxf(p, 0.f), 1.f);
                            const float logit = logf(fmaxf(p, 1e-5f) / fmaxf(1.f - p, 1e-5f));
                            o = 1.f / (1.f + expf(-(r + logit)));
                        } else {
                            o = r;
                            if (lane >= 8 && a.vel_div) o = r / a.vel_div[(unsigned)gi / (unsigned)a.Q];
                        }
                        if (live) a.box_out[g * 10 + lane] = o;
                    }
                    if (a.front) {
                        const int ob = (int)__float_as_uint(o);
                        const float x0 = __uint_as_float((unsigned)__builtin_amdgcn_readlane(ob, 0));
                        const float x1 = __uint_as_float((unsigned)__builtin_amdgcn_readlane(ob, 1));
                        const float x2 = __uint_as_float((unsigned)__builtin_amdgcn_readlane(ob, 2));
                        pe0_row<RG>(a, smem, row, lane, x0, x1, x2);
                    }
                }
            } break;
            case EPI_PE3: {
                if (side) break;
                if (PAIR && member == 0) {
                    pair_load4(px + (2 * R + row) * DM + lane * 4, v);
                    store_rows(smem, OFF_X2, LDX, row, lane, v);
                    break;
                }
                const LnW lw(pv + PV_PE4G, pv + PV_PE4B, lane);
                float res[4];
#pragma unroll
                for (int c = 0; c < 4; ++c) res[c] = smem[OFF_X3 + row * LDX + lane + 64 * c];
                gather4<R>(v, P, 0, un.a.KH, 0, row, lane, pv + PV_PE3_B, 0);
                ln4(v, lw, a.eps, true);
#pragma unroll
                for (int c = 0; c < 4; ++c) v[c] += res[c];
                store_rows(smem, OFF_X2, LDX, row, lane, v);
                if (PAIR) pair_store4(px + (2 * R + row) * DM + lane * 4, v);
                if (live) {
#pragma unroll
                    for (int c = 0; c < 4; ++c) a.x[g * DM + lane + 64 * c] = v[c];
                }
            } break;
            case EPI_QKV: {
                const int ncg = un.a.items / un.a.KH;
#pragma unroll
                for (int c = 0; c < 4; ++c) {
                    const int cg = side * 4 + c;
                    const int n = un.col0 + cg * 64 + lane;
                    if (cg < ncg && n < a.attn_in_rows) {
                        float s = 0.f;
                        for (int kh = 0; kh < un.a.KH; ++kh) s += P[(cg * un.a.KH + kh) * (R * 64) + row * 64 + lane];
                        if (live) a.qkvt[g * a.attn_in_rows + n] = s + pv[PV_QKV_B + n];
                    }
                }
            } break;
            case EPI_AOUT: {
                if (side) break;
                const LnW lw(pv + PV_N1G, pv + PV_N1B, lane);
                float res[4];
#pragma unroll
                for (int c = 0; c < 4; ++c) res[c] = smem[OFF_R + row * LDX + lane + 64 * c];
                gather4<R>(v, P, 0, un.a.KH, 0, row, lane, pv + PV_AOUT_B, 0);
#pragma unroll
                for (int c = 0; c < 4; ++c) v[c] += res[c];
                ln4(v, lw, a.eps, false);
                store_rows(smem, OFF_X3, LDX, row, lane, v);
                if (live) {
#pragma unroll
                    for (int c = 0; c < 4; ++c) a.x1_out[g * DM + lane + 64 * c] = v[c];
                }
                if (a.x1_frag && live) {
                    __builtin_amdgcn_wave_barrier();
                    const int k8 = lane & 31, im = lane >> 5;
                    const float up = a.x1_scale[0];
                    const float4 p0 = *reinterpret_cast<const float4*>(smem + OFF_X3 + row * LDX + 8 * k8);
                    const float4 p1 = *reinterpret_cast<const float4*>(smem + OFF_X3 + row * LDX + 8 * k8 + 4);
                    const float f[8] = {p0.x * up, p0.y * up, p0.z * up, p0.w * up, p1.x * up, p1.y * up, p1.z * up, p1.w * up};
                    unsigned w4[4];
#pragma unroll
                    for (int i = 0; i < 4; ++i) {
                        const _Float16 h0 = (_Float16)f[2 * i], h1 = (_Float16)f[2 * i + 1];
                        const _Float16 l0 = (_Float16)(f[2 * i] - (float)h0), l1 = (_Float16)(f[2 * i + 1] - (float)h1);
                        const _Float16 e0 = im ? l0 : h0, e1 = im ? l1 : h1;
                        w4[i] = (unsigned)__builtin_bit_cast(unsigned short, e0) | ((unsigned)__builtin_bit_cast(unsigned short, e1) << 16);
                    }
                    const long long frag = ((g >> 5) * (DM / 16) + (k8 >> 1)) * 2 + im;
                    uint4* dst = reinterpret_cast<uint4*>(a.x1_frag + frag * 512 + (((int)(g & 31) + 32 * (k8 & 1)) * 8));
                    *dst = make_uint4(w4[0], w4[1], w4[2], w4[3]);
                }
            } break;
            case EPI_SAMP: {
                if (side) break;
                const int ncg = un.a.items / un.a.KH;
#pragma unroll
                for (int c = 0; c < 4; ++c) {
                    const int n = c * 64 + lane;
                    if (c < ncg && n < a.soN) {
                        float s = 0.f;
                        for (int kh = 0; kh < un.a.KH; ++kh) s += P[(c * un.a.KH + kh) * (R * 64) + row * 64 + lane];
                        s += pv[PV_SAMP_B + n];
                        smem[OFF_H + row * 256 + n] = s;
                        if (live && a.so) a.so[g * a.soN + n] = s;
                    }
                }
            } break;
            }
        }
        SBEV_TRACE(4 + 4 * u)
        if (PAIR && un.epi == EPI_PE3 && member == 1) pair_arrive(pword);
        __syncthreads();
        SBEV_TRACE(5 + 4 * u)
    }
    if (PRE == PRE_ATT && a.proj.loc_bp) {
        const int GP = a.proj.G * a.proj.P;
        for (int i = threadIdx.x; i < R * a.proj.T * GP; i += 64 * NWAVE) {
            const int p = i % a.proj.P;
            const int row = (i / a.proj.P) % R;
            const int tg = i / (a.proj.P * R);
            const int gq = tg % a.proj.G, t = tg / a.proj.G;
            const long long g = row0 + row;
            if (g >= a.M) continue;
            const int b = (int)((unsigned)g / (unsigned)a.Q), q = (int)((unsigned)g - (unsigned)b * (unsigned)a.Q);
            const int gp = gq * a.proj.P + p;
            const float* so = smem + OFF_H + row * 256;
            sbev_ops::sample_point(a.proj, b, t, q, gp, a.proj.bbox + g * 10, so + gp * 3, so + GP * 3 + gp * a.proj.L);
        }
    }
}

__global__ void pack_kernel(const float* W, long long ld, int N, int K, float* out) {
    const long long i = (long long)blockIdx.x * 256 + threadIdx.x;
    const long long total = (long long)((N + 63) / 64) * K * 16;
    if (i >= total) return;
    const int lane = (int)(i & 63);
    const long long t = i >> 6;
    const int m = (int)(t & 3);
    const long long t2 = t >> 2;
    const int steps = K / 16;
    const int s = (int)(t2 % steps);
    const int cg = (int)(t2 / steps);
    const int n = cg * 64 + lane;
    float4 v = make_float4(0.f, 0.f, 0.f, 0.f);
    if (n < N) v = *reinterpret_cast<const float4*>(W + (long long)n * ld + 16 * s + 4 * m);
    reinterpret_cast<float4*>(out)[i] = v;
}

__global__ void copy_pad_kernel(const float* src, int n, float* dst, int slot) {
    const int i = blockIdx.x * 256 + threadIdx.x;
    if (i < slot) dst[i] = i < n ? src[i] : 0.f;
}

using Cfg = sbev_decoder_config;

enum Mat { M_FFN0, M_FFN1, M_CLS0, M_REG0, M_CLS3, M_REG2, M_CLS6, M_REG4, M_PE3, M_ATTN_IN, M_ATTN_OUT, M_SAMP, N_MAT };
int so_cols(const Cfg& c) { return c.G * c.P * (3 + c.L); }
int n_embed(const Cfg& c) { return c.D; }
int n_ffn(const Cfg& c) { return c.ffn; }
int n_cls(const Cfg& c) { return c.num_classes; }
int n_code(const Cfg& c) { return c.code_size; }
int n_qkv(const Cfg& c) { return c.attn_in_rows; }
struct MatDesc {
    const float* sbev_decoder_weights::*w;
    int (*N)(const Cfg&);
    int (*K)(const Cfg&);
};
const MatDesc kMats[N_MAT] = {
    {&sbev_decoder_weights::ffn0_w, n_ffn, n_embed},      {&sbev_decoder_weights::ffn1_w, n_embed, n_ffn},
    {&sbev_decoder_weights::cls0_w, n_embed, n_embed},    {&sbev_decoder_weights::reg0_w, n_embed, n_embed},
    {&sbev_decoder_weights::cls3_w, n_embed, n_embed},    {&sbev_decoder_weights::reg2_w, n_embed, n_embed},
    {&sbev_decoder_weights::cls6_w, n_cls, n_embed},      {&sbev_decoder_weights::reg4_w, n_code, n_embed},
    {&sbev_decoder_weights::pe3_w, n_embed, n_embed},     {&sbev_decoder_weights::attn_in_w, n_qkv, n_embed},
    {&sbev_decoder_weights::attn_out_w, n_embed, n_embed}, {&sbev_decoder_weights::samp_w, so_cols, n_embed}};

long long packed_floats(int N, int K) { return (long long)((N + 63) / 64) * 64 * K; }

struct PackMap {
    long long at[N_MAT + 1];
    long long vec() const { return at[N_MAT]; }
    long long total() const { return at[N_MAT] + PV_IMAGE_FLOATS; }
    int lines(int first, int last) const { return (int)((at[last + 1] - at[first]) / 32); }
};
PackMap pack_map(const Cfg& c) {
    PackMap m{};
    for (int i = 0; i < N_MAT; ++i) m.at[i + 1] = m.at[i] + packed_floats(kMats[i].N(c), kMats[i].K(c));
    return m;
}

struct Inst {
    int pre, rg;
    bool pair;
    void (*kern)(ChainArgs);
    int rows, lds;
    std::atomic<unsigned long long> raised;
};
template <int PRE, int RG, bool PAIR = false>
Inst inst() { return Inst{PRE, RG, PAIR, row_chain_kernel<PRE, RG, PAIR>, Lay<RG>::R, Lay<RG>::LDS_TOTAL_FLOATS * 4, {0}}; }
Inst kInst[] = {inst<PRE_SLABS, 1>(), inst<PRE_FRONT, 1>(), inst<PRE_ATT, 1>(), inst<PRE_SLABS, 2>(), inst<PRE_FRONT, 2>(), inst<PRE_ATT, 2>(),
                inst<PRE_SLABS, 4>(), inst<PRE_FRONT, 4>(), inst<PRE_ATT, 4>(), inst<PRE_SLABS, 2, true>(), inst<PRE_SLABS, 4, true>()};
Inst* find_inst(int pre, int rg, bool pair) {
    for (Inst& i : kInst)
        if (i.pre == pre && i.rg == rg && i.pair == pair) return &i;
    return nullptr;
}
hipError_t raise_lds(Inst& i) {
    int dev = 0;
    if (hipGetDevice(&dev) != hipSuccess) return hipErrorInvalidDevice;
    const unsigned long long bit = 1ull << (dev & 63);
    if (i.raised.load(std::memory_order_acquire) & bit) return hipSuccess;
    const hipError_t e = hipFuncSetAttribute(reinterpret_cast<const void*>(i.kern), hipFuncAttributeMaxDynamicSharedMemorySize, i.lds);
    if (e == hipSuccess) i.raised.fetch_or(bit, std::memory_order_release);
    return e;
}

struct PLin { long long w; int in_off, ld, KH, items, chunks, kh0, KHT; };
struct PUnit { PLin a, b; int epi, col0; };
const PLin kNone{-1, 0, LDX, 1, 0, 8, 0, 1};

struct ChainPlan {
    int pre, rg, pair;
    unsigned grid;
    int lds;
    int n_units;
    PUnit units[2][8];
    int n_pairs;
    long long warm;
    int warm_lines;
    long long vec;
    int vec_off, vec_n;
};

int pieces(int rg, int cgs, int K) {
    if (rg == 1) return 0;
    static const bool tie_large = getenv("SBEV_CHAIN_TIE_SMALL") == nullptr;
    int best = 1;
    double best_cost = 1e30;
    for (int kh = 1; kh <= 4 && cgs * kh <= 12 && K / kh >= 16 * RDEPTH; kh *= 2) {
        const int items = cgs * kh, full = items / NWAVE, rest = items % NWAVE;
        const double cost = (K / (16.0 * kh)) * (full + (rest == 0 ? 0.0 : rest <= 4 ? 0.5 : 1.0));
        if (tie_large ? cost < best_cost + 1e-9 : cost < best_cost - 1e-9) { best_cost = cost; best = kh; }
    }
    return best;
}

int row_groups(long long rows) {
    static const int forced = getenv("SBEV_CHAIN_RG") ? atoi(getenv("SBEV_CHAIN_RG")) : 0;
    if ((forced == 1 && rows <= 256 * 4) || (forced == 2 && rows <= 256 * 8) || forced == 4) return forced;
    return rows <= 256 * 4 ? 1 : rows <= 256 * 8 ? 2 : 4;
}
Offs offs(int rg) { return rg == 1 ? offs_of<1>() : rg == 2 ? offs_of<2>() : offs_of<4>(); }

int pair_blocks(long long rows, int rg) {
    const long long pairs = (rows + 4 * rg - 1) / (4 * rg);
    return (int)(16 * ((pairs + 7) / 8));
}
int pair_row_groups(long long rows, bool pair_ok, int cus) {
    if (!pair_ok || rows > 256 * 16) return 0;
    static const int max_rg = getenv("SBEV_CHAIN_PAIR16") ? 4 : 2;
    for (int rg = 2; rg <= max_rg; rg *= 2)
        if (pair_blocks(rows, rg) <= cus) return rg;
    return 0;
}

enum Share { WHOLE = -1, MEMBER0 = 0, MEMBER1 = 1 };

struct UnitTables {
    const Cfg& c;
    const PackMap& m;
    int rg;
    Offs o;

    PLin lin(int mat, int in_off, int ld, int kh = 0, int cg0 = 0, int ncg = -1) const {
        const int N = kMats[mat].N(c), K = kMats[mat].K(c);
        const int KH = kh > 0 ? kh : K / 128;
        if (ncg < 0) ncg = (N + 63) / 64 - cg0;
        return PLin{m.at[mat] + (long long)cg0 * K * 64, in_off, ld, KH, ncg * KH, K / (16 * KH), 0, KH};
    }
    PLin lin_khalf(int mat, int in_off, int ld, int kh, int half) const {
        const int N = kMats[mat].N(c), K = kMats[mat].K(c);
        return PLin{m.at[mat], in_off, ld, kh, ((N + 63) / 64) * kh, K / (32 * kh), half * kh, 2 * kh};
    }

    int front_units(PUnit* u, int n, Share sh) const {
        const int dcg = c.D / 64, qcg = (c.attn_in_rows + 63) / 64;
        u[n++] = PUnit{sh != MEMBER0 ? lin(M_PE3, o.c, LDX, pieces(rg, dcg, c.D)) : kNone, kNone, EPI_PE3, 0};
        static const int q0_forced = getenv("SBEV_CHAIN_PAIR_Q0") ? atoi(getenv("SBEV_CHAIN_PAIR_Q0")) : -1;
        const int q0 = q0_forced >= 0 && q0_forced <= qcg ? q0_forced : (qcg > 8 ? qcg - 8 : qcg / 2);
        const int lo = sh == MEMBER1 ? q0 : 0, hi = sh == MEMBER0 ? q0 : qcg;
        const int cut = sh == WHOLE ? 8 : qcg + 1;
        if (sh != WHOLE && lo == hi) u[n++] = PUnit{kNone, kNone, EPI_QKV, lo * 64};
        for (int cg0 = lo; cg0 < hi; cg0 += cut) {
            const int n_here = hi - cg0 < cut ? hi - cg0 : cut;
            u[n++] = PUnit{lin(M_ATTN_IN, o.x2, LDX, pieces(rg, n_here, c.D), cg0, n_here), kNone, EPI_QKV, cg0 * 64};
        }
        return n;
    }

    int tail_units(PUnit* u, Share sh, bool with_front) const {
        const int dcg = c.D / 64, fcg = c.ffn / 64;
        const bool cls = sh != MEMBER1, reg = sh != MEMBER0;
        const int sides = (cls ? 1 : 0) + (reg ? 1 : 0);
        const int f_ncg = sh == WHOLE ? fcg : fcg / 2, f_cg0 = sh == WHOLE ? 0 : sh * f_ncg;
        int n = 0;
        u[n++] = PUnit{lin(M_FFN0, o.x2, LDX, pieces(rg, f_ncg, c.D), f_cg0, f_ncg), kNone, EPI_FFN0, 0};
        u[n++] = PUnit{sh == WHOLE ? lin(M_FFN1, o.h, LDH, pieces(rg, dcg, c.ffn)) : lin_khalf(M_FFN1, o.h, LDH, pieces(rg, dcg, c.ffn / 2), sh),
                       kNone, EPI_FFN1, 0};
        const auto branch = [&](int mat_c, int in_c, int mat_r, int in_r, int cgs_side, int epi) {
            const int kh = pieces(rg, sides * cgs_side, c.D);
            return PUnit{cls ? lin(mat_c, in_c, LDX, kh) : kNone, reg ? lin(mat_r, in_r, LDX, kh) : kNone, epi, 0};
        };
        u[n++] = branch(M_CLS0, o.x3, M_REG0, o.x3, dcg, EPI_BR1);
        u[n++] = branch(M_CLS3, o.c, M_REG2, o.r, dcg, EPI_BR2);
        u[n++] = branch(M_CLS6, o.c, M_REG4, o.r, 1, EPI_OUT);
        return with_front ? front_units(u, n, sh) : n;
    }
};

ChainPlan chain_plan(const Cfg& c, int pre, bool with_front, bool pair_ok, int cus) {
    const long long rows = (long long)c.B * c.Q;
    const PackMap m = pack_map(c);
    ChainPlan p{};
    p.pre = pre;
    const int prg = pre == PRE_SLABS ? pair_row_groups(rows, pair_ok, cus) : 0;
    p.pair = prg != 0;
    p.rg = p.pair ? prg : row_groups(rows);
    const Inst& in = *find_inst(p.pre, p.rg, p.pair);
    const long long blocks = (rows + in.rows - 1) / in.rows;
    p.grid = p.pair ? (unsigned)pair_blocks(rows, p.rg) : (unsigned)blocks;
    p.lds = in.lds;
    p.n_pairs = p.pair ? (int)blocks : 0;
    const UnitTables t{c, m, p.rg, offs(p.rg)};
    int first = 0, last = 0;
    if (pre == PRE_FRONT) {
        p.n_units = t.front_units(p.units[0], 0, WHOLE);
        first = M_PE3; last = M_ATTN_IN;
        p.vec = m.vec() + PV_TAIL_END; p.vec_off = PV_TAIL_END; p.vec_n = PV_FRONT_END - PV_TAIL_END;
    } else if (pre == PRE_ATT) {
        p.units[0][0] = PUnit{t.lin(M_ATTN_OUT, t.o.x2, LDX, pieces(p.rg, c.D / 64, c.D)), kNone, EPI_AOUT, 0};
        p.units[0][1] = PUnit{t.lin(M_SAMP, t.o.x3, LDX, pieces(p.rg, (so_cols(c) + 63) / 64, c.D)), kNone, EPI_SAMP, 0};
        p.n_units = 2;
        first = M_ATTN_OUT; last = M_SAMP;
        p.vec = m.vec() + PV_FRONT_END; p.vec_off = 0; p.vec_n = PV_ATTN_END;
    } else {
        p.n_units = t.tail_units(p.units[0], p.pair ? MEMBER0 : WHOLE, with_front);
        if (p.pair) (void)t.tail_units(p.units[1], MEMBER1, with_front);
        first = M_FFN0; last = with_front ? M_ATTN_IN : M_REG4;
        p.vec = m.vec(); p.vec_off = 0; p.vec_n = with_front ? PV_FRONT_END : PV_TAIL_END;
    }
    p.warm = m.at[first];
    p.warm_lines = m.lines(first, last);
    return p;
}

std::atomic<int> g_chain_pair{getenv("SBEV_NO_CHAIN_PAIR") ? 0 : 1};
std::atomic<int> g_chain_pair_drop{0};

int device_cus() {
    static std::atomic<int> cus[64];
    int dev = 0;
    if (hipGetDevice(&dev) != hipSuccess) return 0;
    int v = cus[dev & 63].load(std::memory_order_relaxed);
    if (v == 0) {
        if (hipDeviceGetAttribute(&v, hipDeviceAttributeMultiprocessorCount, dev) != hipSuccess) return 0;
        cus[dev & 63].store(v, std::memory_order_relaxed);
    }
    return v;
}

}

namespace sbev {

long long chain_pair_floats(long long rows) { return 3 * (rows + 15) * DM; }
long long chain_pair_sync_words(long long rows) { return (rows + 7) / 8 + 64; }
long long chain_fold_sync_offset(long long rows) { return (rows + 7) / 8; }
bool chain_pair_enabled() { return g_chain_pair.load(std::memory_order_relaxed) != 0; }

bool chain_pair_install(void* host_word_dev) {
    return hipMemcpyToSymbol(HIP_SYMBOL(g_chain_pair_fault_host), &host_word_dev, sizeof(host_word_dev)) == hipSuccess;
}
long long chain_pair_timeouts() {
    unsigned v = 0;
    if (hipMemcpyFromSymbol(&v, HIP_SYMBOL(g_chain_pair_timeouts), sizeof(v)) != hipSuccess) return -1;
    return (long long)v;
}

bool row_chain_supported(const sbev_decoder_config& c) {
    return c.D == DM && c.ffn == FF && c.code_size == 10 && c.num_classes >= 1 && c.num_classes <= 64 &&
           c.attn_in_rows <= PV_QKV_PAD && so_cols(c) <= 256 && (long long)c.B * c.Q < 0x7fffffffLL;
}

bool row_chain_pays(long long rows) {
    static const long long limit = getenv("SBEV_CHAIN_MAX_ROWS") ? atoll(getenv("SBEV_CHAIN_MAX_ROWS")) : 256 * 16;
    return rows <= limit && rows <= 256 * 16;
}

bool chain_lds_ready() {
    for (Inst& i : kInst)
        if (raise_lds(i) != hipSuccess) return false;
    return true;
}

static ChainArgs chain_args(const Cfg& c, float eps) {
    ChainArgs a{};
    a.M = (long long)c.B * c.Q;
    a.Q = c.Q;
    a.eps = eps;
    a.num_classes = c.num_classes;
    a.attn_in_rows = c.attn_in_rows;
    a.soN = so_cols(c);
    return a;
}

static Lin bound(const PLin& l, const float* pk) { return Lin{l.w < 0 ? nullptr : pk + l.w, l.in_off, l.ld, l.KH, l.items, l.chunks, l.kh0, l.KHT}; }

static int launch(const ChainPlan& p, ChainArgs& a, const float* pk, hipStream_t s, const char* what) {
    Inst& in = *find_inst(p.pre, p.rg, p.pair);
    const hipError_t attr = raise_lds(in);
    if (attr != hipSuccess) {
        set_error("%s: hipFuncSetAttribute(%d bytes of LDS): %s", what, in.lds, hipGetErrorString(attr));
        return SBEV_ELAUNCH;
    }
    for (int mem = 0; mem <= p.pair; ++mem)
        for (int u = 0; u < p.n_units; ++u) {
            const PUnit& pu = p.units[mem][u];
            (mem ? a.units_b : a.units)[u] = Unit{bound(pu.a, pk), bound(pu.b, pk), pu.epi, pu.col0};
        }
    a.n_units = p.n_units;
    a.pre = p.pre;
    a.n_pairs = p.n_pairs;
    static const bool no_warm = getenv("SBEV_CHAIN_NO_WARM") != nullptr;
    a.warm = pk + p.warm;
    a.warm_lines = no_warm ? 0 : p.warm_lines;
    a.vec = pk + p.vec; a.vec_off = p.vec_off; a.vec_n = p.vec_n;
#ifdef SBEV_CHAIN_TRACE
    static long long* tr = nullptr;
    static int calls = 0;
    static const Inst* who[13];
    if (!tr) { (void)hipMalloc(&tr, 2 * 64 * 8 * 8 * 64); (void)hipMemset(tr, 0, 2 * 64 * 8 * 8 * 64); }
    a.trace = tr + (calls % 64) * 512;
    if (calls < 13) who[calls] = &in;
#endif
    hipLaunchKernelGGL(in.kern, dim3(p.grid), dim3(64 * NWAVE), in.lds, s, a);
#ifdef SBEV_CHAIN_TRACE
    if (++calls == 13) {
        (void)hipDeviceSynchronize();
        static long long h[2 * 64 * 512];
        (void)hipMemcpy(h, tr, sizeof(h), hipMemcpyDeviceToHost);
        for (int c = 0; c < 13; ++c) {
            const long long* t = h + c * 512;
            printf("launch %d (PRE %d RG %d PAIR %d; 10 ns ticks):", c, who[c]->pre, who[c]->rg, (int)who[c]->pair);
            for (int blk = 0; blk < 2; ++blk)
                for (int w = 0; w < 8; w += 7) {
                    const long long* tb = t + blk * 64 * 512;
                    printf(" [b%d w%d]", blk ? 15 : 7, w);
                    for (int i = 0; i < 2 + 4 * 8 && tb[w * 64 + i]; ++i) printf(" %lld", tb[w * 64 + i] - t[0]);
                }
            printf("\n");
        }
    }
#endif
    return check_launch(what);
}

int launch_chain_front(const sbev_decoder_config& c, const sbev_decoder_weights& w, const float* bbox, const float* feat, float* x,
                       float* qkvt, float eps, hipStream_t s, uint32_t* skip_hdr) {
    ChainArgs a = chain_args(c, eps);
    a.bbox = bbox; a.feat = feat; a.x = x; a.qkvt = qkvt; a.skip_hdr = skip_hdr;
    return launch(chain_plan(c, PRE_FRONT, false, false, 0), a, w.chain_pack, s, "row chain (front)");
}

int launch_chain_attn(const sbev_decoder_config& c, const sbev_decoder_weights& w, const float* att, const float* x, float* x1,
                      const float* bbox, const float* time_diff, const float* lidar2img, float* loc_bp, float* w_bp, float eps,
                      hipStream_t s, uint16_t* x1_frag, const float* x1_scale, uint32_t* pair_sync, const LazyPlan* touch, uint32_t* touch_need) {
    ChainArgs a = chain_args(c, eps);
    a.zero_words = pair_sync;
    a.n_zero = pair_sync ? (int)chain_pair_sync_words(a.M) : 0;
    a.att = att; a.x = const_cast<float*>(x); a.x1_out = x1; a.so = nullptr;
    a.x1_frag = x1_frag; a.x1_scale = x1_scale;
    a.proj = sbev_ops::sample_point_args(bbox, time_diff, lidar2img, c.pc_range, c.B, c.Q, c.T, c.N, c.G, c.P, c.L, c.image_h, c.image_w,
                                         c.eps_homo, loc_bp, w_bp);
    if (touch && touch_need) sbev_ops::sample_point_touch(a.proj, *touch, c.hw, touch_need);
    return launch(chain_plan(c, PRE_ATT, false, false, 0), a, w.chain_pack, s, "row chain (attention)");
}

int launch_chain_tail(const sbev_decoder_config& c, const sbev_decoder_weights& w, const float* slabs, int splits, const float* x1,
                      const float* bbox, const float* vel_div, float* x3, float* cls_out, float* box_out, int with_front, float* x,
                      float* qkvt, float eps, hipStream_t s, float* pair_x, uint32_t* pair_sync) {
    ChainArgs a = chain_args(c, eps);
    a.slabs = slabs; a.splits = splits; a.x1 = x1; a.bbox = bbox; a.vel_div = vel_div;
    a.x3 = x3; a.cls_out = cls_out; a.box_out = box_out; a.front = with_front; a.x = x; a.qkvt = qkvt;
    const bool pair_ok = pair_x && pair_sync && chain_pair_enabled() && a.M <= 256 * 16 && chain_fault_word_ready();
    const ChainPlan p = chain_plan(c, PRE_SLABS, with_front != 0, pair_ok, pair_ok ? device_cus() : 0);
    if (p.pair) {
        a.pair_x = pair_x;
        a.pair_sync = pair_sync;
        a.debug_drop = g_chain_pair_drop.load(std::memory_order_relaxed);
    }
    return launch(p, a, w.chain_pack, s, p.pair ? "row chain (tail, pairs)" : "row chain (tail)");
}

}

extern "C" int sbev_decoder_chain_pair(int enable) { return g_chain_pair.exchange(enable != 0 ? 1 : 0); }

extern "C" int sbev_debug_chain_pair_drop(int enable) { return g_chain_pair_drop.exchange(enable != 0 ? 1 : 0); }

extern "C" int64_t sbev_decoder_chain_pack_floats(const sbev_decoder_config* cfg) {
    if (!cfg || !sbev::row_chain_supported(*cfg)) return 0;
    return pack_map(*cfg).total();
}

extern "C" int sbev_decoder_chain_plan(const sbev_decoder_config* cfg, int kind, int with_front, int pair_ok, int cus, int32_t* out, int capacity) {
    SBEV_REQUIRE(cfg && sbev::row_chain_supported(*cfg) && cfg->B >= 1 && cfg->Q >= 1 && (long long)cfg->B * cfg->Q <= 256 * 16 &&
                     kind >= PRE_SLABS && kind <= PRE_ATT && cus >= 0,
                 "sbev_decoder_chain_plan: config not covered by the row chains (1 .. 4096 rows), or kind / cus out of range");
    const ChainPlan p = chain_plan(*cfg, kind, with_front != 0, pair_ok != 0, cus);
    const int members = p.pair ? 2 : 1;
    const long long words = 12 + 18LL * members * p.n_units;
    SBEV_REQUIRE(out && capacity >= words, "sbev_decoder_chain_plan: %lld words needed", words);
    for (int v : {p.pre, p.rg, p.pair, (int)p.grid, p.lds, p.n_units, p.n_pairs, (int)p.warm, p.warm_lines, (int)p.vec, p.vec_off, p.vec_n}) *out++ = v;
    for (int mem = 0; mem < members; ++mem)
        for (int u = 0; u < p.n_units; ++u) {
            const PUnit& pu = p.units[mem][u];
            *out++ = pu.epi;
            *out++ = pu.col0;
            for (const PLin* l : {&pu.a, &pu.b})
                for (int v : {(int)l->w, l->in_off, l->ld, l->KH, l->items, l->chunks, l->kh0, l->KHT}) *out++ = v;
        }
    return (int)words;
}

extern "C" int sbev_decoder_chain_pack(const sbev_decoder_config* cfg, const sbev_decoder_weights* w, float* out, sbev_stream_t stream) {
    SBEV_REQUIRE(cfg && w && out, "sbev_decoder_chain_pack: null pointer");
    SBEV_REQUIRE(sbev::row_chain_supported(*cfg), "sbev_decoder_chain_pack: config not covered by the row-chain kernels (embed_dims 256, ffn 512, code_size 10)");
    SBEV_REQUIRE((((uintptr_t)out) & 15) == 0, "sbev_decoder_chain_pack: output must be 16-byte aligned");
    const sbev_decoder_config& c = *cfg;
    const PackMap m = pack_map(c);
    hipStream_t s = reinterpret_cast<hipStream_t>(stream);
    SBEV_REQUIRE(sbev::chain_lds_ready(), "sbev_decoder_chain_pack: the device refuses %d bytes of LDS per workgroup", Lay<1>::LDS_TOTAL_FLOATS * 4);
    for (int i = 0; i < N_MAT; ++i) {
        const float* W = w->*kMats[i].w;
        const int N = kMats[i].N(c), K = kMats[i].K(c);
        SBEV_REQUIRE(W && (((uintptr_t)W) & 15) == 0, "sbev_decoder_chain_pack: null / unaligned weight");
        const long long n4 = (long long)((N + 63) / 64) * K * 16;
        hipLaunchKernelGGL(pack_kernel, dim3((unsigned)((n4 + 255) / 256)), dim3(256), 0, s, W, (long long)K, N, K, out + m.at[i]);
    }
    float* pv = out + m.vec();
    struct Vec { const float* p; int off, n, slot; };
    const int soN = so_cols(c);
    const Vec vecs[] = {
        {w->op_b, PV_OP_B, c.D, 256}, {w->norm2_g, PV_N2G, c.D, 256}, {w->norm2_b, PV_N2B, c.D, 256}, {w->ffn0_b, PV_FFN0_B, c.ffn, 512},
        {w->ffn1_b, PV_FFN1_B, c.D, 256}, {w->norm3_g, PV_N3G, c.D, 256}, {w->norm3_b, PV_N3B, c.D, 256},
        {w->cls0_b, PV_CLS0_B, c.D, 256}, {w->cls1_g, PV_CLS1G, c.D, 256}, {w->cls1_b, PV_CLS1B, c.D, 256},
        {w->cls3_b, PV_CLS3_B, c.D, 256}, {w->cls4_g, PV_CLS4G, c.D, 256}, {w->cls4_b, PV_CLS4B, c.D, 256},
        {w->cls6_b, PV_CLS6_B, c.num_classes, 64}, {w->reg0_b, PV_REG0_B, c.D, 256}, {w->reg2_b, PV_REG2_B, c.D, 256},
        {w->reg4_b, PV_REG4_B, c.code_size, 64},
        {w->pe0_w, PV_PE0_W, 3 * c.D, 768}, {w->pe0_b, PV_PE0_B, c.D, 256}, {w->pe1_g, PV_PE1G, c.D, 256}, {w->pe1_b, PV_PE1B, c.D, 256},
        {w->pe3_b, PV_PE3_B, c.D, 256}, {w->pe4_g, PV_PE4G, c.D, 256}, {w->pe4_b, PV_PE4B, c.D, 256},
        {w->attn_in_b, PV_QKV_B, c.attn_in_rows, PV_QKV_PAD},
        {w->attn_out_b, PV_FRONT_END + PV_AOUT_B, c.D, 256}, {w->norm1_g, PV_FRONT_END + PV_N1G, c.D, 256},
        {w->norm1_b, PV_FRONT_END + PV_N1B, c.D, 256}, {w->samp_b, PV_FRONT_END + PV_SAMP_B, soN, 256}};
    for (const Vec& v : vecs) {
        SBEV_REQUIRE(v.p, "sbev_decoder_chain_pack: null bias / LayerNorm pointer");
        hipLaunchKernelGGL(copy_pad_kernel, dim3((unsigned)((v.slot + 255) / 256)), dim3(256), 0, s, v.p, v.n, pv + v.off, v.slot);
    }
    return sbev::check_launch("sbev_decoder_chain_pack");
}
```

### sparsebev_amd/runtime.py

```python
import ctypes
import math
import os
import warnings
import weakref
from collections import namedtuple

import torch

from . import _lib
from .utils import frame_source

MAX_LEVELS = 5
GEMM_F32, GEMM_BF16X3, GEMM_BF16X6, GEMM_BF16X3S, GEMM_F16X3, GEMM_F16X4 = 0, 1, 2, 3, 4, 5
F16_MAX_HEADROOM_LOG2 = 12
GEMM_MODES = {'f32': GEMM_F32, 'bf16x3': GEMM_BF16X3, 'bf16x6': GEMM_BF16X6, 'bf16x3s': GEMM_BF16X3S, 'f16x3': GEMM_F16X3, 'f16x4': GEMM_F16X4}
_f = ctypes.c_void_p


class DecoderConfig(ctypes.Structure):
    _fields_ = [(n, ctypes.c_int32) for n in ('B', 'Q', 'T', 'N', 'G', 'P', 'L', 'D', 'H', 'ffn', 'num_classes',
                                              'code_size', 'num_layers', 'out_points', 'attn_in_rows', 'feat_dtype')] + \
               [('hw', (ctypes.c_int32 * 2) * MAX_LEVELS), ('image_h', ctypes.c_float), ('image_w', ctypes.c_float),
                ('eps_homo', ctypes.c_float), ('gemm_mode', ctypes.c_int32), ('n_slots', ctypes.c_int32),
                ('frame_slots', ctypes.c_int32 * 16), ('overlap', ctypes.c_int32),
# ... 398 lines not shown
            self._destroy(e)

    def _never_replayed(self):
        sig = self._weights()
        return [k for k, e in self.entries.items() if isinstance(e, CapturedStep) and e.pinned and e.replays == 0 and k.weights == sig]

    def _unproven(self):
        return max(self.wasted, 0) + len(self._never_replayed())

    def admit(self, key, ident, pinned):
        e = self.entries.get(key)
        sighted = isinstance(e, _FirstSighting)
        if e is None or (sighted and not e.same(ident)):
            if pinned and self._unproven() >= self.MAX_WASTED:
                self._refuse()
                return EAGER, None
            if e is None and len(self.entries) >= self.MAX:
                self._drop(next(iter(self.entries)))
            self.entries[key] = _FirstSighting(ident)
            return SIGHTED, None
        return (CAPTURE if sighted else REPLAY), e

    def _refuse(self):
        self._refused += 1
        if self._refused % self.RETRY_EVERY == 0:
            if self.wasted > 0:
                self.wasted -= 1
            else:
                stale = next(iter(self._never_replayed()), None)
                if stale is not None:
                    self._drop(stale)
                    self.wasted = max(self.wasted - 1, 0)
        if not self._warned:
            warnings.warn('sparsebev_amd: %d step graphs keyed on input addresses were captured and never replayed (the caller '
                          'passes new channels-last / pyramid buffers every call): no further address-keyed graphs; pass fp32 '
                          'NCHW feature lists or reuse the buffers' % self._unproven())
            self._warned = True

    def captured(self, key, step):
        self.entries[key] = step
        self.captures += 1

    def launch(self, key, step):
        self.entries[key] = self.entries.pop(key)
        step.graph.replay()
        step.replays += 1
        self.replays += 1
        if step.pinned and step.replays > 0:
            self.wasted = 0


class StepGraphs(StepBook):

    def __init__(self, runtime):
        super().__init__(lambda: runtime._sig, lambda step: runtime._release_graph_ws(step.ws_key))
        self.rt = runtime

    @staticmethod
    def _relayout_ok(f):
        return f.dim() == 5 and f.dtype in (torch.float32, torch.bfloat16, torch.float16) and f.is_contiguous() and f.data_ptr() % 16 == 0 and \
            not f.permute(0, 1, 3, 4, 2).is_contiguous()

    def _feat_key(self, feats, src):
        if src.kind != 'list':
            table = src.slot_table
            fi = src.insert
            ins = None if fi is None else (tuple((tuple(f.shape), f.dtype) for f in fi.frames), fi.rows.data_ptr(), fi.K, fi.nhwc)
            return ('pyr', tuple((f.data_ptr(), tuple(f.shape), f.dtype) for f in feats.levels), src.frame_slots, src.n_slots,
                    None if table is None else (table.data_ptr(), tuple(table.shape)), ins), [], False
        if all(self._relayout_ok(f) for f in feats):
            return ('nchw', tuple((tuple(f.shape), f.dtype) for f in feats)), [], True
        return ('list', tuple((f.data_ptr(), tuple(f.shape), tuple(f.stride()), f.dtype) for f in feats)), list(feats), False

    def run(self, query_bbox, query_feat, mlvl_feats, attn_mask, img_metas, finish=False, src=None):
        rt = self.rt
        if _STATE['profile'] or not (query_bbox.is_cuda and query_bbox.is_contiguous() and query_feat.is_contiguous()):
            return None
        if query_bbox.data_ptr() % 16 or query_feat.data_ptr() % 16:
            return None
        if attn_mask is not None and not (attn_mask.is_cuda and attn_mask.dtype == torch.uint8 and attn_mask.is_contiguous() and attn_mask.data_ptr() % 16 == 0):
            return None
        src = src or frame_source(mlvl_feats)
        if src.kind == 'list' and not all(torch.is_tensor(f) and f.is_cuda for f in mlvl_feats):
            return None
        from . import transformer as TR
        check_pair_faults()
        sig = rt._ensure_bound()
        fkey, ident, staged = self._feat_key(mlvl_feats, src)
        key = StepKey(tuple(query_bbox.shape), tuple(query_feat.shape), fkey, None if attn_mask is None else tuple(attn_mask.shape), sig,
                      torch.cuda.current_device(), _switch_key(), rt.decoder.num_layers, tuple(rt.decoder.pc_range),
                      torch.cuda.current_stream(query_bbox.device).cuda_stream, bool(finish))
        verdict, e = self.admit(key, ident, pinned=not staged and not src.resident)
        if e is None:
            return None
        B, Q = query_bbox.shape[:2]
        packed, layout, ih, iw = consts = TR.DecoderContext.pack(img_metas, B)
        outs = None
        if finish:
            nl, nc, cs = rt.decoder.num_layers, rt.decoder.decoder_layer.num_classes, rt.decoder.decoder_layer.code_size
            outs = (torch.empty(nl, B, Q, nc, device=query_bbox.device, dtype=torch.float32),
                    torch.empty(nl, B, Q, cs, device=query_bbox.device, dtype=torch.float32))
        call = StepInputs(query_bbox, query_feat, mlvl_feats, attn_mask, outs, None if src.insert is None else src.insert.frames)
        if verdict == CAPTURE:
            e = self._capture(key, call, consts, staged, src)
            if e is None:
                return None
        else:
            if layout != e.layout or (ih, iw) != e.image:
                return None
            TR._upload(self._with_table(packed, e.n_packed, e.staged, call), query_bbox.device, out=e.ctx_buf)
        self.launch(key, e)
        return outs if outs is not None else (e.graph.cls, e.graph.box)

    @staticmethod
    def _with_table(packed, n_packed, staged, call):
        import numpy as np
        ptrs = [call.bbox.data_ptr(), call.feat.data_ptr(), call.mask.data_ptr() if call.mask is not None else 0]
        if staged:
            ptrs += [f.data_ptr() for f in call.feats]
        elif call.frames is not None:
            ptrs += [f.data_ptr() for f in call.frames]
        if call.outs is not None:
            ptrs += [call.outs[0].data_ptr(), call.outs[1].data_ptr()]
        full = np.empty(n_packed + 2 * len(ptrs), dtype=np.float32)
        full[:packed.size] = packed
        full[packed.size:n_packed] = 0.0
        full[n_packed:].view(np.int64)[:] = ptrs
        return full

    def _capture(self, key, call, consts, staged, src):
        from . import transformer as TR
        rt, dev = self.rt, call.bbox.device
        packed, layout, ih, iw = consts
        qb, qf = torch.empty_like(call.bbox), torch.empty_like(call.feat)
        mask = torch.empty_like(call.mask) if call.mask is not None else None
        pyramid = TR.FeaturePyramid.for_graph(call.feats, staged) if src.kind == 'list' else call.feats
        if pyramid is None:
            return None
        insert = None
        if src.insert is not None:
            pyramid = pyramid.resident()
            insert = (list(range(3, 3 + len(call.frames))), src.insert, pyramid)
        n_packed = (packed.size + 3) // 4 * 4
        ctx = TR.DecoderContext.from_packed(self._with_table(packed, n_packed, staged, call), layout, ih, iw, dev)
        args, keep, cls, box = rt._prepare(qb, qf, pyramid, ctx, mask, own_workspace=True)
        try:
            segs = [(0, qb), (1, qf)] + ([(2, mask)] if mask is not None else [])
            relayout = [(3 + l, buf) for l, buf in enumerate(pyramid.levels)] if staged else []
            lazy = len(relayout) > 0 and _STATE['lazy'] and bool(_lib.load().sbev_decoder_lazy_supported(args.config))
            need = _prefix_cache_for(keep.cfg, rt._weights, mask, lazy, dev)
            prefix = PrefixCache(need, dev) if need else None
            handle = self._record(args, ctypes.c_void_p(ctx.buffer.data_ptr() + 4 * n_packed), segs, relayout, lazy,
                                  (cls, box) if call.outs is not None else None, insert, prefix)
        except BaseException:
            rt._release_graph_ws(keep.ws_key)
            raise
        graph = DecoderGraph(handle, (keep, qb, qf, mask, ctx, None if staged else (None if insert else call.feats, pyramid)), cls, box)
        e = CapturedStep(graph, not staged and not src.resident, staged, ctx.buffer, n_packed, layout, (ih, iw), keep.ws_key, prefix)
        self.captured(key, e)
        return e

    @staticmethod
    def _record(args, table, segs, relayout, lazy, finish, insert=None, prefix=None):
        lib = _lib.load()
        side = torch.cuda.Stream(device=segs[0][1].device)
        side.wait_stream(torch.cuda.current_stream())
        sp = ctypes.c_void_p(side.cuda_stream)
        c_idx = (ctypes.c_int32 * len(segs))(*[i for i, _ in segs])
        c_dst = (ctypes.c_void_p * len(segs))(*[t.data_ptr() for _, t in segs])
        c_nb = (ctypes.c_int64 * len(segs))(*[t.numel() * t.element_size() for _, t in segs])
        n = len(relayout)
        n_img, ch = relayout[0][1].shape[::3] if n else (0, 0)
        hws = [buf.shape[1] * buf.shape[2] for _, buf in relayout]
        _lib.check(lib.sbev_capture_begin(sp), 'sbev_capture_begin')
        ok, st_fwd = True, 0
        try:
            ok = lib.sbev_copy_indirect(table, len(segs), c_idx, c_dst, c_nb, sp) == 0
            multi = (not lazy and 1 < n <= MAX_LEVELS and ch % 4 == 0 and _STATE['relayout_multi']
                     and all(buf.dtype == torch.float32 and hw % 4 == 0 for (_, buf), hw in zip(relayout, hws)))
            if multi:
                c_ix = (ctypes.c_int32 * n)(*[i for i, _ in relayout])
                c_out = (ctypes.c_void_p * n)(*[buf.data_ptr() for _, buf in relayout])
                ok = ok and lib.sbev_nchw_to_nhwc_f32_multi_indirect(table, n, c_ix, c_out, n_img, ch, (ctypes.c_int32 * n)(*hws), sp) == 0
            elif not lazy:
                for (idx, buf), hw in zip(relayout, hws):
                    fn = lib.sbev_nchw_to_nhwc_f32_indirect if buf.dtype == torch.float32 else lib.sbev_nchw_to_nhwc_b16_indirect
                    ok = ok and fn(table, idx, _ptr(buf), n_img, ch, hw, sp) == 0
            if insert is not None and ok:
                from . import cache
                idx, pending, pool_pyr = insert
                ok = cache.pool_insert_frames(pending.frames, pool_pyr.levels, pending.rows, pool_pyr.n_slots, sp, pending.nhwc, table, idx, check=False) == 0
            st_fwd = _forward_cached(args, ([idx for idx, _ in relayout], table) if lazy else None, sp, prefix) if ok else 0
            ok = ok and st_fwd == 0
            if finish is not None:
                cls, box = finish
                i_out = 3 + (n if insert is None else len(insert[0]))
                ok = ok and lib.sbev_finish_outputs_indirect(table, i_out, i_out + 1, _ptr(cls), _ptr(box), cls.numel(), box.numel(), sp) == 0
        finally:
            handle = ctypes.c_void_p()
            st = lib.sbev_capture_end(sp, ctypes.byref(handle) if ok else None)
        if st_fwd == _lib.EFAULT:
            _lib.check(st_fwd, 'sbev_decoder_forward (capture)')
        if not ok:
            raise _lib.SbevError('graph capture of the decoder step failed: ' + lib.sbev_last_error().decode())
        _lib.check(st, 'sbev_capture_end')
        torch.cuda.current_stream().wait_stream(side)
        return handle


class _FirstSighting:

    def __init__(self, tensors):
        self.refs = [(weakref.ref(t.untyped_storage()), t.storage_offset(), tuple(t.shape), tuple(t.stride()), t.dtype) for t in tensors]

    def same(self, tensors):
        return len(tensors) == len(self.refs) and all(
            r[0]() is not None and r[0]() is t.untyped_storage() and r[1:] == (t.storage_offset(), tuple(t.shape), tuple(t.stride()), t.dtype)
            for r, t in zip(self.refs, tensors))


class DecoderGraph:

    def __init__(self, handle, keep, cls, box):
        self._h, self._keep, self.cls, self.box = handle, keep, cls, box
        self.num_nodes = int(_lib.load().sbev_graph_num_nodes(handle))

    def replay(self):
        if self._h is None:
            raise RuntimeError('DecoderGraph was destroyed')
        st = _lib.load().sbev_graph_launch(self._h, ctypes.c_void_p(torch.cuda.current_stream().cuda_stream))
        _lib.check(st, 'sbev_graph_launch')
        return self.cls, self.box

    def destroy(self):
        if self._h is not None:
            _lib.load().sbev_graph_destroy(self._h)
            self._h = None

    def __del__(self):
        try:
            self.destroy()
        except Exception:
            pass


class _State(dict):
    def __missing__(self, key):
        if key != 'order':
            raise KeyError(key)
        return _switch_key()[4]


_STATE = _State(profile=0,
                prefix_off=os.environ.get('SBEV_NO_PREFIX_CACHE') == '1',
                lazy=not os.environ.get('SBEV_NO_SPARSE_RELAYOUT'),
                relayout_multi=not os.environ.get('SBEV_NO_RELAYOUT_MULTI'))


def _switch_key():
    buf = (ctypes.c_int32 * 32)()
    n = _lib.load().sbev_decoder_switches(buf, 32)
    assert 0 < n <= 32
    return tuple(buf[:n]) + (bool(_STATE['lazy']), bool(_STATE['relayout_multi']))


def out_fold(enable):
    return bool(_lib.load().sbev_decoder_out_fold(int(bool(enable))))


def prefix_cache(enable):
    prev = not _STATE['prefix_off']
    _STATE['prefix_off'] = not enable
    for c in list(PrefixCache._live or ()):
        with torch.cuda.device(c.device):
            c.force(not enable)
    return prev


def lazy_relayout(enable):
    prev = _STATE['lazy']
    _STATE['lazy'] = bool(enable)
    return prev


def query_order(enable):
    mode = 2 if enable == 2 and enable is not True else int(bool(enable))
    prev = int(_lib.load().sbev_decoder_query_order(mode))
    _STATE['order'] = mode
    return prev


def fuse_sample_mix(enable):
    _lib.check(_lib.load().sbev_decoder_fuse_sample_mix(int(bool(enable))), 'sbev_decoder_fuse_sample_mix')


def row_chain(enable):
    _lib.check(_lib.load().sbev_decoder_row_chain(int(bool(enable))), 'sbev_decoder_row_chain')


def chain_pair(enable):
    return bool(_lib.load().sbev_decoder_chain_pair(int(bool(enable))))


def _on_pair_fault():
    lib = _lib.load()
    lib.sbev_decoder_chain_pair(0)
    lib.sbev_decoder_chain_pair_faults_ack()
    warnings.warn('sparsebev_amd: a pair-mode tail hand-off timed out (GPU shared / preempted?); pair mode is off for the rest of the process')


def check_pair_faults():
    n = int(_lib.load().sbev_decoder_chain_pair_faults())
    if n > 0:
        _on_pair_fault()
        raise _lib.PairFaultError('%d pair-mode hand-off(s) timed out since the last check: the step(s) since then hold invalid rows; '
                                  'pair mode is off now, repeat them' % n)


def chain_pair_timeouts():
    n = _lib.load().sbev_decoder_chain_pair_timeouts()
    if n < 0:
        raise RuntimeError('sbev_decoder_chain_pair_timeouts: HIP error')
    return int(n)


def profile_sampler(enable):
    _lib.load().sbev_profile_sampler(int(enable))
    _STATE['profile'] = int(enable)


def profile_stride(every_n_calls):
    _lib.check(_lib.load().sbev_profile_stride(int(every_n_calls)), 'sbev_profile_stride')


def read_kernel_ms(kind, max_n=4096):
    buf = (ctypes.c_float * max_n)()
    n = _lib.load().sbev_profile_read(kind, buf, max_n)
    return [buf[i] for i in range(n)]


def read_sampler_ms(max_n=4096):
    return read_kernel_ms(0, max_n)
```

Measured before the change: 581.6 samples/s.

## Add compile-time fixed unit tables for common row-chain plans

Adds kernel variants for four common chain configurations in which the unit/item tables are constexpr and baked into the kernel rather than passed as runtime arguments. At launch the runtime plan is compared word by word against the fixed table, and the specialised kernel runs only when they match. The aim is to cut runtime table walking, indirect loads and branch overhead in the weight-streaming loops, and to shrink the kernel argument block. In exchange it adds more kernel instantiations, more code size and complexity, and a possible change in register pressure.

Result: faster. 602.8 samples/s, median of 6 (+3.6%).

```diff
diff --git a/include/sbev_hip.h b/include/sbev_hip.h
--- a/include/sbev_hip.h
+++ b/include/sbev_hip.h
@@ -434,6 +434,9 @@
 int sbev_decoder_chain_pack(const sbev_decoder_config* cfg, const sbev_decoder_weights* weights, float* out, sbev_stream_t stream);
 int sbev_decoder_row_chain(int enable);
 int sbev_decoder_chain_plan(const sbev_decoder_config* cfg, int kind, int with_front, int pair_ok, int cus, int32_t* out, int capacity);
+int sbev_decoder_chain_fixed(int enable);
+int64_t sbev_decoder_chain_fixed_launches(void);
+int sbev_decoder_chain_fixed_plan(const sbev_decoder_config* cfg, int kind, int with_front, int pair_ok, int cus, int32_t* out, int capacity);
 
 int sbev_decoder_chain_pair(int enable);
 int64_t sbev_decoder_chain_pair_timeouts(void);
diff --git a/sparsebev_amd/_lib.py b/sparsebev_amd/_lib.py
--- a/sparsebev_amd/_lib.py
+++ b/sparsebev_amd/_lib.py
@@ -233,6 +233,9 @@
     'sbev_decoder_chain_pack': (ctypes.c_int, [_vp, _vp, _vp, _vp]),
     'sbev_decoder_chain_plan': (ctypes.c_int, [_vp, ctypes.c_int, ctypes.c_int, ctypes.c_int, ctypes.c_int, _c_i32p, ctypes.c_int]),
     'sbev_decoder_row_chain': (ctypes.c_int, [ctypes.c_int]),
+    'sbev_decoder_chain_fixed_plan': (ctypes.c_int, [_vp, ctypes.c_int, ctypes.c_int, ctypes.c_int, ctypes.c_int, _c_i32p, ctypes.c_int]),
+    'sbev_decoder_chain_fixed': (ctypes.c_int, [ctypes.c_int]),
+    'sbev_decoder_chain_fixed_launches': (ctypes.c_int64, []),
     'sbev_decoder_chain_pair': (ctypes.c_int, [ctypes.c_int]),
     'sbev_decoder_chain_pair_timeouts': (ctypes.c_int64, []),
     'sbev_decoder_chain_pair_faults': (ctypes.c_int64, []),
diff --git a/sparsebev_amd/csrc/row_chain.hip b/sparsebev_amd/csrc/row_chain.hip
--- a/sparsebev_amd/csrc/row_chain.hip
+++ b/sparsebev_amd/csrc/row_chain.hip
@@ -2,6 +2,9 @@
 #include "sample_point.hpp"
 #include <atomic>
 #include <cstdlib>
+#include <cstring>
+#include <type_traits>
+#include <utility>
 
 namespace {
 
@@ -43,12 +46,14 @@
 #define SBEV_TRACE(i)
 #endif
 
-struct ChainArgs {
+struct UnitTab {
+    Unit units[8];
+    Unit units_b[8];
+};
+struct ChainCommon {
 #ifdef SBEV_CHAIN_TRACE
     long long* trace;
 #endif
-    Unit units[8];
-    Unit units_b[8];
     int n_units, pre, front;
     int n_pairs;
     float* pair_x;
@@ -81,6 +86,10 @@
     float eps;
     uint32_t* skip_hdr;
 };
+struct ChainArgs : UnitTab, ChainCommon {};
+struct ChainArgsFx : ChainCommon {
+    const float* image;
+};
 
 constexpr int RING_SLOTS = 3;
 constexpr int CHUNK_FLOATS = 1024;
@@ -108,7 +117,7 @@
 template <int RG> constexpr Offs offs_of() { return Offs{Lay<RG>::OFF_X2, Lay<RG>::OFF_X3, Lay<RG>::OFF_H, Lay<RG>::OFF_C, Lay<RG>::OFF_R}; }
 
 template <int RG>
-__device__ __forceinline__ void warm_l2(const ChainArgs& a, int wave, int lane) {
+__device__ __forceinline__ void warm_l2(const ChainCommon& a, int wave, int lane) {
     const int per_xcd = ((int)gridDim.x + 7) / 8;
     const int parts = per_xcd < 32 ? per_xcd : 32;
     const int part = ((int)blockIdx.x / 8) % parts;
@@ -133,21 +142,13 @@
     int u, it, step;
 };
 
-__device__ __forceinline__ int unit_items(const Unit* U, int u) { return U[u].a.items + U[u].b.items; }
-
-__device__ __forceinline__ void walk_settle(const ChainArgs& a, const Unit* U, Walk& w, int wave) {
-    while (w.u < a.n_units && w.it >= unit_items(U, w.u)) {
-        ++w.u;
-        w.it = wave;
-    }
-}
-
+__device__ __forceinline__ const float* lin_item_weights(const Lin& l, int j) {
+    const int piece = l.KHT == l.KH ? j : (j / l.KH) * l.KHT + l.kh0 + j % l.KH;
+    return l.wp + (long long)piece * (l.chunks * CHUNK_FLOATS);
+}
 __device__ __forceinline__ const float* item_weights(const Unit& un, int it) {
     const bool second = it >= un.a.items;
-    const Lin& l = second ? un.b : un.a;
-    const int j = it - (second ? un.a.items : 0);
-    const int piece = l.KHT == l.KH ? j : (j / l.KH) * l.KHT + l.kh0 + j % l.KH;
-    return l.wp + (long long)piece * (l.chunks * CHUNK_FLOATS);
+    return lin_item_weights(second ? un.b : un.a, it - (second ? un.a.items : 0));
 }
 
 __device__ __forceinline__ void issue_chunk(const float* g, unsigned lds_byte, unsigned voff) {
@@ -164,7 +165,6 @@
 }
 
 struct Stream {
-    const Unit* U;
     Walk iw;
     const float* g;
     int nchunk;
@@ -172,39 +172,53 @@
     int islot, uslot;
     unsigned ring_byte;
     unsigned voff;
-};
-
-__device__ __forceinline__ void stream_seek(const ChainArgs& a, Stream& st, int wave) {
-    walk_settle(a, st.U, st.iw, wave);
-    st.iw.step = 0;
-    if (st.iw.u < a.n_units) {
-        const Unit& un = st.U[st.iw.u];
-        st.g = item_weights(un, st.iw.it);
-        st.nchunk = st.iw.it >= un.a.items ? un.b.chunks : un.a.chunks;
-    }
-}
-
-__device__ __forceinline__ void stream_issue(const ChainArgs& a, Stream& st, int wave) {
-    if (st.iw.u >= a.n_units) return;
-    issue_chunk(st.g + st.iw.step * CHUNK_FLOATS, st.ring_byte + (unsigned)st.islot * (CHUNK_FLOATS * 4), st.voff);
-    ++st.issued;
-    st.islot = st.islot == RING_SLOTS - 1 ? 0 : st.islot + 1;
-    if (++st.iw.step == st.nchunk) {
-        st.iw.it += NWAVE;
-        stream_seek(a, st, wave);
-    }
-}
+    const float *g_cur, *g_next;
+    bool has_next, live;
+};
 
 struct RChunk { float4 q[4]; };
-__device__ __forceinline__ void stream_load(const ChainArgs& a, Stream& st, int wave, int lane, RChunk& c) {
-    const float* g = st.g + st.iw.step * CHUNK_FLOATS + lane * 4;
-#pragma unroll
-    for (int m = 0; m < 4; ++m) c.q[m] = *reinterpret_cast<const float4*>(g + 256 * m);
-    if (st.iw.u < a.n_units && ++st.iw.step == st.nchunk) {
-        st.iw.it += NWAVE;
-        stream_seek(a, st, wave);
-    }
-}
+
+struct RtTab {
+    const ChainArgs& a;
+    const Unit* U;
+
+    __device__ __forceinline__ void settle(Walk& w, int wave) const {
+        while (w.u < a.n_units && w.it >= U[w.u].a.items + U[w.u].b.items) {
+            ++w.u;
+            w.it = wave;
+        }
+    }
+    __device__ __forceinline__ void seek(Stream& st, int wave) const {
+        settle(st.iw, wave);
+        st.iw.step = 0;
+        if (st.iw.u < a.n_units) {
+            const Unit& un = U[st.iw.u];
+            st.g = item_weights(un, st.iw.it);
+            st.nchunk = st.iw.it >= un.a.items ? un.b.chunks : un.a.chunks;
+        }
+    }
+    __device__ __forceinline__ void issue(Stream& st, int wave) const {
+        if (st.iw.u >= a.n_units) return;
+        issue_chunk(st.g + st.iw.step * CHUNK_FLOATS, st.ring_byte + (unsigned)st.islot * (CHUNK_FLOATS * 4), st.voff);
+        ++st.issued;
+        st.islot = st.islot == RING_SLOTS - 1 ? 0 : st.islot + 1;
+        if (++st.iw.step == st.nchunk) {
+            st.iw.it += NWAVE;
+            seek(st, wave);
+        }
+    }
+    __device__ __forceinline__ void load(Stream& st, int wave, int lane, RChunk& c) const {
+        const float* g = st.g + st.iw.step * CHUNK_FLOATS + lane * 4;
+#pragma unroll
+        for (int m = 0; m < 4; ++m) c.q[m] = *reinterpret_cast<const float4*>(g + 256 * m);
+        if (st.iw.u < a.n_units && ++st.iw.step == st.nchunk) {
+            st.iw.it += NWAVE;
+            seek(st, wave);
+        }
+    }
+    template <class UC> __device__ __forceinline__ void begin_item(UC, Stream&, int, int) const {}
+    __device__ __forceinline__ void begin_round(Stream&, int, int) const {}
+};
 constexpr int RDEPTH = 4;
 
 #define SBEV_MF(KK, BV) acc[(KK) & 1] = __builtin_amdgcn_mfma_f32_4x4x1f32(av, BV, acc[(KK) & 1], 4, KK, 0);
@@ -212,7 +226,8 @@
 
 typedef float f32x4 __attribute__((ext_vector_type(4)));
 
-__device__ __forceinline__ void mma_item(const ChainArgs& a, Stream& st, const Lin& l, int j, float* smem, int pslot, int lane, int wave) {
+template <class TAB>
+__device__ __forceinline__ void mma_item(const TAB& a, Stream& st, const Lin& l, int j, float* smem, int pslot, int lane, int wave) {
     constexpr int R = 4, OFF_RING = Lay<1>::OFF_RING, OFF_P = Lay<1>::OFF_P;
     f32x4 acc[2] = {{0.f, 0.f, 0.f, 0.f}, {0.f, 0.f, 0.f, 0.f}};
     const int kh = j % l.KH;
@@ -232,7 +247,7 @@
         asm volatile("s_waitcnt lgkmcnt(0)" ::: "memory");
         ++st.used;
         st.uslot = st.uslot == RING_SLOTS - 1 ? 0 : st.uslot + 1;
-        stream_issue(a, st, wave);
+        a.issue(st, wave);
         __builtin_amdgcn_sched_barrier(0);
         SBEV_MSTEP(0, q0) SBEV_MSTEP(1, q1) SBEV_MSTEP(2, q2) SBEV_MSTEP(3, q3)
     }
@@ -241,8 +256,8 @@
     p[0] = t.x; p[64] = t.y; p[128] = t.z; p[192] = t.w;
 }
 
-template <int RG>
-__device__ __forceinline__ void mma_item_wide(const ChainArgs& a, Stream& st, RChunk (&rb)[RDEPTH], const Lin& l, int j, float* smem, int pslot,
+template <int RG, class TAB>
+__device__ __forceinline__ void mma_item_wide(const TAB& a, Stream& st, RChunk (&rb)[RDEPTH], const Lin& l, int j, float* smem, int pslot,
                                               int lane, int wave) {
     constexpr int NACC = RG >= 4 ? 1 : 2;
     f32x4 acc[RG][NACC];
@@ -255,7 +270,9 @@
     float avn[RG];
 #pragma unroll
     for (int rg = 0; rg < RG; ++rg) avn[rg] = arow[rg * 4 * l.ld];
+#pragma nounroll
     for (int s0 = 0; s0 < l.chunks; s0 += RDEPTH) {
+        a.begin_round(st, l.chunks, s0);
 #pragma unroll
         for (int d = 0; d < RDEPTH; ++d) {
             float av[RG];
@@ -271,7 +288,7 @@
 #undef SBEV_MWSTEP
 #undef SBEV_MW
             __builtin_amdgcn_sched_barrier(0);
-            stream_load(a, st, wave, lane, rb[d]);
+            a.load(st, wave, lane, rb[d]);
         }
     }
     float* p = smem + Lay<RG>::OFF_P + pslot * (Lay<RG>::R * 64) + lane;
@@ -378,7 +395,7 @@
 }
 
 template <int RG>
-__device__ __forceinline__ void pe0_row(const ChainArgs& a, float* smem, int row, int lane, float x0, float x1, float x2) {
+__device__ __forceinline__ void pe0_row(const ChainCommon& a, float* smem, int row, int lane, float x0, float x1, float x2) {
     constexpr int OFF_PARAM = Lay<RG>::OFF_PARAM, OFF_C = Lay<RG>::OFF_C;
     const float* pv = smem + OFF_PARAM;
     const LnW lw(pv + PV_PE1G, pv + PV_PE1B, lane);
@@ -393,8 +410,255 @@
     store_rows(smem, OFF_C, LDX, row, lane, v);
 }
 
-template <int PRE, int RG, bool PAIR = false>
-__global__ __launch_bounds__(64 * NWAVE) void row_chain_kernel(const ChainArgs a) {
+using Cfg = sbev_decoder_config;
+
+enum Mat { M_FFN0, M_FFN1, M_CLS0, M_REG0, M_CLS3, M_REG2, M_CLS6, M_REG4, M_PE3, M_ATTN_IN, M_ATTN_OUT, M_SAMP, N_MAT };
+constexpr int so_cols(const Cfg& c) { return c.G * c.P * (3 + c.L); }
+constexpr int n_embed(const Cfg& c) { return c.D; }
+constexpr int n_ffn(const Cfg& c) { return c.ffn; }
+constexpr int n_cls(const Cfg& c) { return c.num_classes; }
+constexpr int n_code(const Cfg& c) { return c.code_size; }
+constexpr int n_qkv(const Cfg& c) { return c.attn_in_rows; }
+struct MatDesc {
+    const float* sbev_decoder_weights::*w;
+    int (*N)(const Cfg&);
+    int (*K)(const Cfg&);
+};
+constexpr MatDesc kMats[N_MAT] = {
+    {&sbev_decoder_weights::ffn0_w, n_ffn, n_embed},      {&sbev_decoder_weights::ffn1_w, n_embed, n_ffn},
+    {&sbev_decoder_weights::cls0_w, n_embed, n_embed},    {&sbev_decoder_weights::reg0_w, n_embed, n_embed},
+    {&sbev_decoder_weights::cls3_w, n_embed, n_embed},    {&sbev_decoder_weights::reg2_w, n_embed, n_embed},
+    {&sbev_decoder_weights::cls6_w, n_cls, n_embed},      {&sbev_decoder_weights::reg4_w, n_code, n_embed},
+    {&sbev_decoder_weights::pe3_w, n_embed, n_embed},     {&sbev_decoder_weights::attn_in_w, n_qkv, n_embed},
+    {&sbev_decoder_weights::attn_out_w, n_embed, n_embed}, {&sbev_decoder_weights::samp_w, so_cols, n_embed}};
+
+constexpr long long packed_floats(int N, int K) { return (long long)((N + 63) / 64) * 64 * K; }
+
+struct PackMap {
+    long long at[N_MAT + 1];
+    constexpr long long vec() const { return at[N_MAT]; }
+    constexpr long long total() const { return at[N_MAT] + PV_IMAGE_FLOATS; }
+    constexpr int lines(int first, int last) const { return (int)((at[last + 1] - at[first]) / 32); }
+};
+constexpr PackMap pack_map(const Cfg& c) {
+    PackMap m{};
+    for (int i = 0; i < N_MAT; ++i) m.at[i + 1] = m.at[i] + packed_floats(kMats[i].N(c), kMats[i].K(c));
+    return m;
+}
+
+struct PLin { long long w; int in_off, ld, KH, items, chunks, kh0, KHT; };
+struct PUnit { PLin a, b; int epi, col0; };
+constexpr PLin kNone{-1, 0, LDX, 1, 0, 8, 0, 1};
+
+struct Tweaks {
+    bool tie_large;
+    int q0_forced;
+};
+constexpr Tweaks kNoTweaks{true, -1};
+
+constexpr int pieces(int rg, int cgs, int K, bool tie_large) {
+    if (rg == 1) return 0;
+    int best = 1;
+    double best_cost = 1e30;
+    for (int kh = 1; kh <= 4 && cgs * kh <= 12 && K / kh >= 16 * RDEPTH; kh *= 2) {
+        const int items = cgs * kh, full = items / NWAVE, rest = items % NWAVE;
+        const double cost = (K / (16.0 * kh)) * (full + (rest == 0 ? 0.0 : rest <= 4 ? 0.5 : 1.0));
+        if (tie_large ? cost < best_cost + 1e-9 : cost < best_cost - 1e-9) { best_cost = cost; best = kh; }
+    }
+    return best;
+}
+
+constexpr Offs offs(int rg) { return rg == 1 ? offs_of<1>() : rg == 2 ? offs_of<2>() : offs_of<4>(); }
+
+enum Share { WHOLE = -1, MEMBER0 = 0, MEMBER1 = 1 };
+
+struct UnitTables {
+    const Cfg& c;
+    const PackMap& m;
+    int rg;
+    Offs o;
+    Tweaks tw;
+
+    constexpr int pieces(int rg_, int cgs, int K) const { return ::pieces(rg_, cgs, K, tw.tie_large); }
+
+    constexpr PLin lin(int mat, int in_off, int ld, int kh = 0, int cg0 = 0, int ncg = -1) const {
+        const int N = kMats[mat].N(c), K = kMats[mat].K(c);
+        const int KH = kh > 0 ? kh : K / 128;
+        if (ncg < 0) ncg = (N + 63) / 64 - cg0;
+        return PLin{m.at[mat] + (long long)cg0 * K * 64, in_off, ld, KH, ncg * KH, K / (16 * KH), 0, KH};
+    }
+    constexpr PLin lin_khalf(int mat, int in_off, int ld, int kh, int half) const {
+        const int N = kMats[mat].N(c), K = kMats[mat].K(c);
+        return PLin{m.at[mat], in_off, ld, kh, ((N + 63) / 64) * kh, K / (32 * kh), half * kh, 2 * kh};
+    }
+
+    constexpr int front_units(PUnit* u, int n, Share sh) const {
+        const int dcg = c.D / 64, qcg = (c.attn_in_rows + 63) / 64;
+        u[n++] = PUnit{sh != MEMBER0 ? lin(M_PE3, o.c, LDX, pieces(rg, dcg, c.D)) : kNone, kNone, EPI_PE3, 0};
+        const int q0_forced = tw.q0_forced;
+        const int q0 = q0_forced >= 0 && q0_forced <= qcg ? q0_forced : (qcg > 8 ? qcg - 8 : qcg / 2);
+        const int lo = sh == MEMBER1 ? q0 : 0, hi = sh == MEMBER0 ? q0 : qcg;
+        const int cut = sh == WHOLE ? 8 : qcg + 1;
+        if (sh != WHOLE && lo == hi) u[n++] = PUnit{kNone, kNone, EPI_QKV, lo * 64};
+        for (int cg0 = lo; cg0 < hi; cg0 += cut) {
+            const int n_here = hi - cg0 < cut ? hi - cg0 : cut;
+            u[n++] = PUnit{lin(M_ATTN_IN, o.x2, LDX, pieces(rg, n_here, c.D), cg0, n_here), kNone, EPI_QKV, cg0 * 64};
+        }
+        return n;
+    }
+
+    constexpr int tail_units(PUnit* u, Share sh, bool with_front) const {
+        const int dcg = c.D / 64, fcg = c.ffn / 64;
+        const bool cls = sh != MEMBER1, reg = sh != MEMBER0;
+        const int sides = (cls ? 1 : 0) + (reg ? 1 : 0);
+        const int f_ncg = sh == WHOLE ? fcg : fcg / 2, f_cg0 = sh == WHOLE ? 0 : sh * f_ncg;
+        int n = 0;
+        u[n++] = PUnit{lin(M_FFN0, o.x2, LDX, pieces(rg, f_ncg, c.D), f_cg0, f_ncg), kNone, EPI_FFN0, 0};
+        u[n++] = PUnit{sh == WHOLE ? lin(M_FFN1, o.h, LDH, pieces(rg, dcg, c.ffn)) : lin_khalf(M_FFN1, o.h, LDH, pieces(rg, dcg, c.ffn / 2), sh),
+                       kNone, EPI_FFN1, 0};
+        const auto branch = [&](int mat_c, int in_c, int mat_r, int in_r, int cgs_side, int epi) {
+            const int kh = pieces(rg, sides * cgs_side, c.D);
+            return PUnit{cls ? lin(mat_c, in_c, LDX, kh) : kNone, reg ? lin(mat_r, in_r, LDX, kh) : kNone, epi, 0};
+        };
+        u[n++] = branch(M_CLS0, o.x3, M_REG0, o.x3, dcg, EPI_BR1);
+        u[n++] = branch(M_CLS3, o.c, M_REG2, o.r, dcg, EPI_BR2);
+        u[n++] = branch(M_CLS6, o.c, M_REG4, o.r, 1, EPI_OUT);
+        return with_front ? front_units(u, n, sh) : n;
+    }
+};
+
+struct PlanUnits {
+    int n_units;
+    PUnit units[2][8];
+};
+constexpr PlanUnits plan_units(const Cfg& c, int pre, int rg, bool pair, bool with_front, Tweaks tw) {
+    const PackMap m = pack_map(c);
+    const UnitTables t{c, m, rg, offs(rg), tw};
+    PlanUnits p{};
+    if (pre == PRE_FRONT) {
+        p.n_units = t.front_units(p.units[0], 0, WHOLE);
+    } else if (pre == PRE_ATT) {
+        p.units[0][0] = PUnit{t.lin(M_ATTN_OUT, t.o.x2, LDX, t.pieces(rg, c.D / 64, c.D)), kNone, EPI_AOUT, 0};
+        p.units[0][1] = PUnit{t.lin(M_SAMP, t.o.x3, LDX, t.pieces(rg, (so_cols(c) + 63) / 64, c.D)), kNone, EPI_SAMP, 0};
+        p.n_units = 2;
+    } else {
+        p.n_units = t.tail_units(p.units[0], pair ? MEMBER0 : WHOLE, with_front);
+        if (pair) (void)t.tail_units(p.units[1], MEMBER1, with_front);
+    }
+    return p;
+}
+
+struct FixKey {
+    int pre, rg, pair, with_front;
+    int qcg, scg;
+};
+constexpr int N_FIX = 4;
+constexpr FixKey fix_key(int i) {
+    switch (i) {
+    case 0: return FixKey{PRE_SLABS, 2, 1, 1, 13, 2};
+    case 1: return FixKey{PRE_SLABS, 2, 1, 0, 13, 2};
+    case 2: return FixKey{PRE_ATT, 1, 0, 0, 13, 2};
+    default: return FixKey{PRE_FRONT, 1, 0, 0, 13, 2};
+    }
+}
+constexpr bool same_key(const FixKey& a, const FixKey& b) {
+    return a.pre == b.pre && a.rg == b.rg && a.pair == b.pair && a.with_front == b.with_front && a.qcg == b.qcg && a.scg == b.scg;
+}
+constexpr Cfg key_cfg(const FixKey& k) {
+    Cfg c{};
+    c.D = DM; c.ffn = FF; c.code_size = 10; c.num_classes = 1;
+    c.attn_in_rows = 64 * k.qcg;
+    c.G = 1; c.P = 16 * k.scg; c.L = 1;
+    return c;
+}
+constexpr PlanUnits fixed_units(int i) {
+    const FixKey k = fix_key(i);
+    return plan_units(key_cfg(k), k.pre, k.rg, k.pair != 0, k.with_front != 0, kNoTweaks);
+}
+
+__host__ __device__ __forceinline__ Lin bound(const PLin& l, const float* pk) {
+    return Lin{l.w < 0 ? nullptr : pk + l.w, l.in_off, l.ld, l.KH, l.items, l.chunks, l.kh0, l.KHT};
+}
+
+template <int FIX, int MEM>
+struct FxTab {
+    const float* image;
+    static constexpr int N = fixed_units(FIX).n_units;
+    template <int U> static constexpr PUnit pu() { return fixed_units(FIX).units[MEM][U]; }
+    template <int U> static constexpr int items() { return pu<U>().a.items + pu<U>().b.items; }
+    template <int U> __device__ __forceinline__ Unit unit() const {
+        constexpr PUnit p = pu<U>();
+        return Unit{bound(p.a, image), bound(p.b, image), p.epi, p.col0};
+    }
+    template <int U> __device__ __forceinline__ const float* weights(int it) const {
+        constexpr PUnit p = pu<U>();
+        if constexpr (p.b.items == 0) return lin_item_weights(bound(p.a, image), it);
+        else if constexpr (p.a.items == 0) return lin_item_weights(bound(p.b, image), it);
+        else return it >= p.a.items ? lin_item_weights(bound(p.b, image), it - p.a.items) : lin_item_weights(bound(p.a, image), it);
+    }
+    template <int U> __device__ __forceinline__ bool first_from(int wave, const float*& g) const {
+        if constexpr (U >= N) {
+            return false;
+        } else {
+            if (wave < items<U>()) {
+                g = weights<U>(wave);
+                return true;
+            }
+            return first_from<U + 1>(wave, g);
+        }
+    }
+    template <int U> __device__ __forceinline__ bool next(int it, int wave, const float*& g) const {
+        if constexpr (items<U>() > NWAVE) {
+            if (it + NWAVE < items<U>()) {
+                g = weights<U>(it + NWAVE);
+                return true;
+            }
+        }
+        return first_from<U + 1>(wave, g);
+    }
+
+    __device__ __forceinline__ void seek(Stream& st, int wave) const {
+        st.iw.step = 0;
+        st.g = image;
+        st.live = first_from<0>(wave, st.g);
+        st.g_next = st.g;
+        st.has_next = false;
+    }
+    template <int U> __device__ __forceinline__ void begin_item(std::integral_constant<int, U>, Stream& st, int it, int wave) const {
+        st.g_cur = weights<U>(it);
+        st.g_next = st.g_cur;
+        st.has_next = next<U>(it, wave, st.g_next);
+    }
+    __device__ __forceinline__ void issue(Stream& st, int) const {
+        if (!st.live) return;
+        issue_chunk(st.g + st.iw.step * CHUNK_FLOATS, st.ring_byte + (unsigned)st.islot * (CHUNK_FLOATS * 4), st.voff);
+        ++st.issued;
+        st.islot = st.islot == RING_SLOTS - 1 ? 0 : st.islot + 1;
+        if (++st.iw.step == 8) {
+            st.iw.step = 0;
+            st.g = st.g_next;
+            st.live = st.has_next;
+        }
+    }
+    __device__ __forceinline__ void begin_round(Stream& st, int chunks, int s0) const {
+        st.g = s0 + RDEPTH < chunks ? st.g_cur + (s0 + RDEPTH) * CHUNK_FLOATS : st.g_next;
+        st.iw.step = 0;
+    }
+    __device__ __forceinline__ void load(Stream& st, int, int lane, RChunk& c) const {
+        const float* g = st.g + st.iw.step * CHUNK_FLOATS + lane * 4;
+#pragma unroll
+        for (int m = 0; m < 4; ++m) c.q[m] = *reinterpret_cast<const float4*>(g + 256 * m);
+        ++st.iw.step;
+    }
+};
+
+template <class F, int... I>
+__device__ __forceinline__ void for_each_unit(F&& f, std::integer_sequence<int, I...>) {
+    (f(std::integral_constant<int, I>{}), ...);
+}
+
+template <int PRE, int RG, bool PAIR, int FIX, int MEM, class A>
+__device__ __forceinline__ void chain_body(const A& a, const int pair, const int member) {
     using L = Lay<RG>;
     static_assert(!PAIR || (PRE == PRE_SLABS && RG > 1), "pair mode: the tail, wide row blocks");
     constexpr int R = L::R, RPW = L::RPW, OFF_X2 = L::OFF_X2, OFF_X3 = L::OFF_X3, OFF_H = L::OFF_H, OFF_C = L::OFF_C, OFF_R = L::OFF_R,
@@ -402,15 +666,11 @@
     extern __shared__ __attribute__((aligned(16))) float smem[];
     const int lane = threadIdx.x & 63;
     const int wave = __builtin_amdgcn_readfirstlane(threadIdx.x >> 6);
-    int pair = (int)blockIdx.x, member = 0;
-    if constexpr (PAIR) {
-        const int li = (int)blockIdx.x >> 3;
-        pair = (li >> 1) * 8 + ((int)blockIdx.x & 7);
-        member = li & 1;
-        if (pair >= a.n_pairs) return;
-        if (a.debug_drop && pair == 0 && member == 1) return;
-    }
-    const Unit* const U = (PAIR && member) ? a.units_b : a.units;
+    const auto tab = [&] {
+        if constexpr (FIX >= 0) return FxTab<FIX, MEM>{a.image};
+        else return RtTab{a, (PAIR && member) ? a.units_b : a.units};
+    }();
+    constexpr int front_fx = fix_key(FIX < 0 ? 0 : FIX).with_front;
     unsigned* const pword = PAIR ? a.pair_sync + pair : nullptr;
     float* const px = PAIR ? a.pair_x + (long long)pair * (3 * R * DM) : nullptr;
     const long long row0 = (long long)pair * R;
@@ -431,26 +691,25 @@
     SBEV_TRACE(0)
     warm_l2<RG>(a, wave, lane);
     Stream st;
-    st.U = U;
     st.iw = Walk{0, wave, 0};
     st.issued = st.used = st.islot = st.uslot = 0;
     st.ring_byte = (unsigned)(L::OFF_RING + wave * (RING_SLOTS * CHUNK_FLOATS)) * 4u;
     st.voff = (unsigned)lane * 16u;
     st.g = a.warm;
     st.nchunk = 8;
-    stream_seek(a, st, wave);
+    tab.seek(st, wave);
     RChunk rb[RDEPTH];
     if constexpr (L::WIDE) {
 #pragma unroll
         for (int d = 0; d < RDEPTH; ++d) {
 #pragma unroll
             for (int m = 0; m < 4; ++m) rb[d].q[m] = make_float4(0.f, 0.f, 0.f, 0.f);
-            stream_load(a, st, wave, lane, rb[d]);
+            tab.load(st, wave, lane, rb[d]);
         }
     } else {
-        stream_issue(a, st, wave);
-        stream_issue(a, st, wave);
-        stream_issue(a, st, wave);
+        tab.issue(st, wave);
+        tab.issue(st, wave);
+        tab.issue(st, wave);
     }
 
     const float* pv = smem + OFF_PARAM;
@@ -544,13 +803,17 @@
     __syncthreads();
 
     SBEV_TRACE(1)
-    for (int u = 0; u < a.n_units; ++u) {
-        const Unit& un = U[u];
+    const auto run_unit = [&](const Unit& un, const auto uc, const auto only) __attribute__((always_inline)) {
+        constexpr int ONLY = decltype(only)::value;
+        [[maybe_unused]] const int u = uc;
         const int items = un.a.items + un.b.items;
+#pragma nounroll
         for (int it = wave; it < items; it += NWAVE) {
-            const bool second = it >= un.a.items;
-            if constexpr (L::WIDE) mma_item_wide<RG>(a, st, rb, second ? un.b : un.a, it - (second ? un.a.items : 0), smem, it, lane, wave);
-            else mma_item(a, st, second ? un.b : un.a, it - (second ? un.a.items : 0), smem, it, lane, wave);
+            const bool second = ONLY == 0 ? it >= un.a.items : ONLY == 2;
+            const Lin& l = ONLY == 1 ? un.a : ONLY == 2 ? un.b : second ? un.b : un.a;
+            tab.begin_item(uc, st, it, wave);
+            if constexpr (L::WIDE) mma_item_wide<RG>(tab, st, rb, l, it - (second ? un.a.items : 0), smem, it, lane, wave);
+            else mma_item(tab, st, l, it - (second ? un.a.items : 0), smem, it, lane, wave);
         }
         SBEV_TRACE(2 + 4 * u)
         __syncthreads();
@@ -644,7 +907,7 @@
                         }
                         if (live) a.box_out[g * 10 + lane] = o;
                     }
-                    if (a.front) {
+                    if (FIX >= 0 ? front_fx : a.front) {
                         const int ob = (int)__float_as_uint(o);
                         const float x0 = __uint_as_float((unsigned)__builtin_amdgcn_readlane(ob, 0));
                         const float x1 = __uint_as_float((unsigned)__builtin_amdgcn_readlane(ob, 1));
@@ -744,6 +1007,16 @@
         if (PAIR && un.epi == EPI_PE3 && member == 1) pair_arrive(pword);
         __syncthreads();
         SBEV_TRACE(5 + 4 * u)
+    };
+    if constexpr (FIX >= 0) {
+        for_each_unit([&](const auto uc) __attribute__((always_inline)) {
+            constexpr int UI = decltype(uc)::value;
+            constexpr PUnit p = FxTab<FIX, MEM>::template pu<UI>();
+            const Unit un = tab.template unit<UI>();
+            run_unit(un, uc, std::integral_constant<int, p.b.items == 0 ? 1 : p.a.items == 0 ? 2 : 0>{});
+        }, std::make_integer_sequence<int, FxTab<FIX, MEM>::N>{});
+    } else {
+        for (int u = 0; u < a.n_units; ++u) run_unit(tab.U[u], u, std::integral_constant<int, 0>{});
     }
     if (PRE == PRE_ATT && a.proj.loc_bp) {
         const int GP = a.proj.G * a.proj.P;
@@ -759,6 +1032,39 @@
             const float* so = smem + OFF_H + row * 256;
             sbev_ops::sample_point(a.proj, b, t, q, gp, a.proj.bbox + g * 10, so + gp * 3, so + GP * 3 + gp * a.proj.L);
         }
+    }
+}
+
+template <bool PAIR>
+__device__ __forceinline__ bool pair_of_block(const ChainCommon& a, int& pair, int& member) {
+    pair = (int)blockIdx.x;
+    member = 0;
+    if constexpr (PAIR) {
+        const int li = (int)blockIdx.x >> 3;
+        pair = (li >> 1) * 8 + ((int)blockIdx.x & 7);
+        member = li & 1;
+        if (pair >= a.n_pairs) return false;
+        if (a.debug_drop && pair == 0 && member == 1) return false;
+    }
+    return true;
+}
+
+template <int PRE, int RG, bool PAIR = false>
+__global__ __launch_bounds__(64 * NWAVE) void row_chain_kernel(const ChainArgs a) {
+    int pair, member;
+    if (!pair_of_block<PAIR>(a, pair, member)) return;
+    chain_body<PRE, RG, PAIR, -1, -1>(a, pair, member);
+}
+
+template <int PRE, int RG, bool PAIR, int FIX>
+__global__ __launch_bounds__(64 * NWAVE) void row_chain_fixed_kernel(const ChainArgsFx a) {
+    int pair, member;
+    if (!pair_of_block<PAIR>(a, pair, member)) return;
+    if constexpr (PAIR) {
+        if (member == 0) chain_body<PRE, RG, PAIR, FIX, 0>(a, pair, 0);
+        else chain_body<PRE, RG, PAIR, FIX, 1>(a, pair, 1);
+    } else {
+        chain_body<PRE, RG, PAIR, FIX, 0>(a, pair, 0);
     }
 }
 
@@ -784,56 +1090,30 @@
     if (i < slot) dst[i] = i < n ? src[i] : 0.f;
 }
 
-using Cfg = sbev_decoder_config;
-
-enum Mat { M_FFN0, M_FFN1, M_CLS0, M_REG0, M_CLS3, M_REG2, M_CLS6, M_REG4, M_PE3, M_ATTN_IN, M_ATTN_OUT, M_SAMP, N_MAT };
-int so_cols(const Cfg& c) { return c.G * c.P * (3 + c.L); }
-int n_embed(const Cfg& c) { return c.D; }
-int n_ffn(const Cfg& c) { return c.ffn; }
-int n_cls(const Cfg& c) { return c.num_classes; }
-int n_code(const Cfg& c) { return c.code_size; }
-int n_qkv(const Cfg& c) { return c.attn_in_rows; }
-struct MatDesc {
-    const float* sbev_decoder_weights::*w;
-    int (*N)(const Cfg&);
-    int (*K)(const Cfg&);
-};
-const MatDesc kMats[N_MAT] = {
-    {&sbev_decoder_weights::ffn0_w, n_ffn, n_embed},      {&sbev_decoder_weights::ffn1_w, n_embed, n_ffn},
-    {&sbev_decoder_weights::cls0_w, n_embed, n_embed},    {&sbev_decoder_weights::reg0_w, n_embed, n_embed},
-    {&sbev_decoder_weights::cls3_w, n_embed, n_embed},    {&sbev_decoder_weights::reg2_w, n_embed, n_embed},
-    {&sbev_decoder_weights::cls6_w, n_cls, n_embed},      {&sbev_decoder_weights::reg4_w, n_code, n_embed},
-    {&sbev_decoder_weights::pe3_w, n_embed, n_embed},     {&sbev_decoder_weights::attn_in_w, n_qkv, n_embed},
-    {&sbev_decoder_weights::attn_out_w, n_embed, n_embed}, {&sbev_decoder_weights::samp_w, so_cols, n_embed}};
-
-long long packed_floats(int N, int K) { return (long long)((N + 63) / 64) * 64 * K; }
-
-struct PackMap {
-    long long at[N_MAT + 1];
-    long long vec() const { return at[N_MAT]; }
-    long long total() const { return at[N_MAT] + PV_IMAGE_FLOATS; }
-    int lines(int first, int last) const { return (int)((at[last + 1] - at[first]) / 32); }
-};
-PackMap pack_map(const Cfg& c) {
-    PackMap m{};
-    for (int i = 0; i < N_MAT; ++i) m.at[i + 1] = m.at[i] + packed_floats(kMats[i].N(c), kMats[i].K(c));
-    return m;
-}
-
 struct Inst {
     int pre, rg;
     bool pair;
+    int fix;
     void (*kern)(ChainArgs);
+    void (*kern_fx)(ChainArgsFx);
     int rows, lds;
     std::atomic<unsigned long long> raised;
 };
 template <int PRE, int RG, bool PAIR = false>
-Inst inst() { return Inst{PRE, RG, PAIR, row_chain_kernel<PRE, RG, PAIR>, Lay<RG>::R, Lay<RG>::LDS_TOTAL_FLOATS * 4, {0}}; }
+Inst inst() { return Inst{PRE, RG, PAIR, -1, row_chain_kernel<PRE, RG, PAIR>, nullptr, Lay<RG>::R, Lay<RG>::LDS_TOTAL_FLOATS * 4, {0}}; }
+template <int FIX>
+Inst inst_fixed() {
+    constexpr FixKey k = fix_key(FIX);
+    return Inst{k.pre, k.rg, k.pair != 0, FIX, nullptr, row_chain_fixed_kernel<k.pre, k.rg, k.pair != 0, FIX>, Lay<k.rg>::R,
+                Lay<k.rg>::LDS_TOTAL_FLOATS * 4, {0}};
+}
 Inst kInst[] = {inst<PRE_SLABS, 1>(), inst<PRE_FRONT, 1>(), inst<PRE_ATT, 1>(), inst<PRE_SLABS, 2>(), inst<PRE_FRONT, 2>(), inst<PRE_ATT, 2>(),
-                inst<PRE_SLABS, 4>(), inst<PRE_FRONT, 4>(), inst<PRE_ATT, 4>(), inst<PRE_SLABS, 2, true>(), inst<PRE_SLABS, 4, true>()};
-Inst* find_inst(int pre, int rg, bool pair) {
+                inst<PRE_SLABS, 4>(), inst<PRE_FRONT, 4>(), inst<PRE_ATT, 4>(), inst<PRE_SLABS, 2, true>(), inst<PRE_SLABS, 4, true>(),
+                inst_fixed<0>(), inst_fixed<1>(), inst_fixed<2>(), inst_fixed<3>()};
+static_assert(N_FIX == 4, "one inst_fixed row per fixed plan");
+Inst* find_inst(int pre, int rg, bool pair, int fix = -1) {
     for (Inst& i : kInst)
-        if (i.pre == pre && i.rg == rg && i.pair == pair) return &i;
+        if (i.pre == pre && i.rg == rg && i.pair == pair && i.fix == fix) return &i;
     return nullptr;
 }
 hipError_t raise_lds(Inst& i) {
@@ -841,21 +1121,15 @@
     if (hipGetDevice(&dev) != hipSuccess) return hipErrorInvalidDevice;
     const unsigned long long bit = 1ull << (dev & 63);
     if (i.raised.load(std::memory_order_acquire) & bit) return hipSuccess;
-    const hipError_t e = hipFuncSetAttribute(reinterpret_cast<const void*>(i.kern), hipFuncAttributeMaxDynamicSharedMemorySize, i.lds);
+    const hipError_t e = hipFuncSetAttribute(i.fix < 0 ? reinterpret_cast<const void*>(i.kern) : reinterpret_cast<const void*>(i.kern_fx), hipFuncAttributeMaxDynamicSharedMemorySize, i.lds);
     if (e == hipSuccess) i.raised.fetch_or(bit, std::memory_order_release);
     return e;
 }
 
-struct PLin { long long w; int in_off, ld, KH, items, chunks, kh0, KHT; };
-struct PUnit { PLin a, b; int epi, col0; };
-const PLin kNone{-1, 0, LDX, 1, 0, 8, 0, 1};
-
-struct ChainPlan {
+struct ChainPlan : PlanUnits {
     int pre, rg, pair;
     unsigned grid;
     int lds;
-    int n_units;
-    PUnit units[2][8];
     int n_pairs;
     long long warm;
     int warm_lines;
@@ -863,26 +1137,11 @@
     int vec_off, vec_n;
 };
 
-int pieces(int rg, int cgs, int K) {
-    if (rg == 1) return 0;
-    static const bool tie_large = getenv("SBEV_CHAIN_TIE_SMALL") == nullptr;
-    int best = 1;
-    double best_cost = 1e30;
-    for (int kh = 1; kh <= 4 && cgs * kh <= 12 && K / kh >= 16 * RDEPTH; kh *= 2) {
-        const int items = cgs * kh, full = items / NWAVE, rest = items % NWAVE;
-        const double cost = (K / (16.0 * kh)) * (full + (rest == 0 ? 0.0 : rest <= 4 ? 0.5 : 1.0));
-        if (tie_large ? cost < best_cost + 1e-9 : cost < best_cost - 1e-9) { best_cost = cost; best = kh; }
-    }
-    return best;
-}
-
 int row_groups(long long rows) {
     static const int forced = getenv("SBEV_CHAIN_RG") ? atoi(getenv("SBEV_CHAIN_RG")) : 0;
     if ((forced == 1 && rows <= 256 * 4) || (forced == 2 && rows <= 256 * 8) || forced == 4) return forced;
     return rows <= 256 * 4 ? 1 : rows <= 256 * 8 ? 2 : 4;
 }
-Offs offs(int rg) { return rg == 1 ? offs_of<1>() : rg == 2 ? offs_of<2>() : offs_of<4>(); }
-
 int pair_blocks(long long rows, int rg) {
     const long long pairs = (rows + 4 * rg - 1) / (4 * rg);
     return (int)(16 * ((pairs + 7) / 8));
@@ -894,60 +1153,6 @@
         if (pair_blocks(rows, rg) <= cus) return rg;
     return 0;
 }
-
-enum Share { WHOLE = -1, MEMBER0 = 0, MEMBER1 = 1 };
-
-struct UnitTables {
-    const Cfg& c;
-    const PackMap& m;
-    int rg;
-    Offs o;
-
-    PLin lin(int mat, int in_off, int ld, int kh = 0, int cg0 = 0, int ncg = -1) const {
-        const int N = kMats[mat].N(c), K = kMats[mat].K(c);
-        const int KH = kh > 0 ? kh : K / 128;
-        if (ncg < 0) ncg = (N + 63) / 64 - cg0;
-        return PLin{m.at[mat] + (long long)cg0 * K * 64, in_off, ld, KH, ncg * KH, K / (16 * KH), 0, KH};
-    }
-    PLin lin_khalf(int mat, int in_off, int ld, int kh, int half) const {
-        const int N = kMats[mat].N(c), K = kMats[mat].K(c);
-        return PLin{m.at[mat], in_off, ld, kh, ((N + 63) / 64) * kh, K / (32 * kh), half * kh, 2 * kh};
-    }
-
-    int front_units(PUnit* u, int n, Share sh) const {
-        const int dcg = c.D / 64, qcg = (c.attn_in_rows + 63) / 64;
-        u[n++] = PUnit{sh != MEMBER0 ? lin(M_PE3, o.c, LDX, pieces(rg, dcg, c.D)) : kNone, kNone, EPI_PE3, 0};
-        static const int q0_forced = getenv("SBEV_CHAIN_PAIR_Q0") ? atoi(getenv("SBEV_CHAIN_PAIR_Q0")) : -1;
-        const int q0 = q0_forced >= 0 && q0_forced <= qcg ? q0_forced : (qcg > 8 ? qcg - 8 : qcg / 2);
-        const int lo = sh == MEMBER1 ? q0 : 0, hi = sh == MEMBER0 ? q0 : qcg;
-        const int cut = sh == WHOLE ? 8 : qcg + 1;
-        if (sh != WHOLE && lo == hi) u[n++] = PUnit{kNone, kNone, EPI_QKV, lo * 64};
-        for (int cg0 = lo; cg0 < hi; cg0 += cut) {
-            const int n_here = hi - cg0 < cut ? hi - cg0 : cut;
-            u[n++] = PUnit{lin(M_ATTN_IN, o.x2, LDX, pieces(rg, n_here, c.D), cg0, n_here), kNone, EPI_QKV, cg0 * 64};
-        }
-        return n;
-    }
-
-    int tail_units(PUnit* u, Share sh, bool with_front) const {
-        const int dcg = c.D / 64, fcg = c.ffn / 64;
-        const bool cls = sh != MEMBER1, reg = sh != MEMBER0;
-        const int sides = (cls ? 1 : 0) + (reg ? 1 : 0);
-        const int f_ncg = sh == WHOLE ? fcg : fcg / 2, f_cg0 = sh == WHOLE ? 0 : sh * f_ncg;
-        int n = 0;
-        u[n++] = PUnit{lin(M_FFN0, o.x2, LDX, pieces(rg, f_ncg, c.D), f_cg0, f_ncg), kNone, EPI_FFN0, 0};
-        u[n++] = PUnit{sh == WHOLE ? lin(M_FFN1, o.h, LDH, pieces(rg, dcg, c.ffn)) : lin_khalf(M_FFN1, o.h, LDH, pieces(rg, dcg, c.ffn / 2), sh),
-                       kNone, EPI_FFN1, 0};
-        const auto branch = [&](int mat_c, int in_c, int mat_r, int in_r, int cgs_side, int epi) {
-            const int kh = pieces(rg, sides * cgs_side, c.D);
-            return PUnit{cls ? lin(mat_c, in_c, LDX, kh) : kNone, reg ? lin(mat_r, in_r, LDX, kh) : kNone, epi, 0};
-        };
-        u[n++] = branch(M_CLS0, o.x3, M_REG0, o.x3, dcg, EPI_BR1);
-        u[n++] = branch(M_CLS3, o.c, M_REG2, o.r, dcg, EPI_BR2);
-        u[n++] = branch(M_CLS6, o.c, M_REG4, o.r, 1, EPI_OUT);
-        return with_front ? front_units(u, n, sh) : n;
-    }
-};
 
 ChainPlan chain_plan(const Cfg& c, int pre, bool with_front, bool pair_ok, int cus) {
     const long long rows = (long long)c.B * c.Q;
@@ -962,21 +1167,16 @@
     p.grid = p.pair ? (unsigned)pair_blocks(rows, p.rg) : (unsigned)blocks;
     p.lds = in.lds;
     p.n_pairs = p.pair ? (int)blocks : 0;
-    const UnitTables t{c, m, p.rg, offs(p.rg)};
+    static const Tweaks tw{getenv("SBEV_CHAIN_TIE_SMALL") == nullptr, getenv("SBEV_CHAIN_PAIR_Q0") ? atoi(getenv("SBEV_CHAIN_PAIR_Q0")) : -1};
+    static_cast<PlanUnits&>(p) = plan_units(c, pre, p.rg, p.pair != 0, with_front, tw);
     int first = 0, last = 0;
     if (pre == PRE_FRONT) {
-        p.n_units = t.front_units(p.units[0], 0, WHOLE);
         first = M_PE3; last = M_ATTN_IN;
         p.vec = m.vec() + PV_TAIL_END; p.vec_off = PV_TAIL_END; p.vec_n = PV_FRONT_END - PV_TAIL_END;
     } else if (pre == PRE_ATT) {
-        p.units[0][0] = PUnit{t.lin(M_ATTN_OUT, t.o.x2, LDX, pieces(p.rg, c.D / 64, c.D)), kNone, EPI_AOUT, 0};
-        p.units[0][1] = PUnit{t.lin(M_SAMP, t.o.x3, LDX, pieces(p.rg, (so_cols(c) + 63) / 64, c.D)), kNone, EPI_SAMP, 0};
-        p.n_units = 2;
         first = M_ATTN_OUT; last = M_SAMP;
         p.vec = m.vec() + PV_FRONT_END; p.vec_off = 0; p.vec_n = PV_ATTN_END;
     } else {
-        p.n_units = t.tail_units(p.units[0], p.pair ? MEMBER0 : WHOLE, with_front);
-        if (p.pair) (void)t.tail_units(p.units[1], MEMBER1, with_front);
         first = M_FFN0; last = with_front ? M_ATTN_IN : M_REG4;
         p.vec = m.vec(); p.vec_off = 0; p.vec_n = with_front ? PV_FRONT_END : PV_TAIL_END;
     }
@@ -987,6 +1187,38 @@
 
 std::atomic<int> g_chain_pair{getenv("SBEV_NO_CHAIN_PAIR") ? 0 : 1};
 std::atomic<int> g_chain_pair_drop{0};
+
+constexpr PlanUnits kFixedUnits[N_FIX] = {fixed_units(0), fixed_units(1), fixed_units(2), fixed_units(3)};
+std::atomic<int> g_chain_fixed{getenv("SBEV_CHAIN_FIXED") ? (atoi(getenv("SBEV_CHAIN_FIXED")) != 0 ? 1 : 0) : 1};
+std::atomic<long long> g_chain_fixed_launches{0};
+
+void unit_words(const PUnit& pu, int32_t* out) {
+    *out++ = pu.epi;
+    *out++ = pu.col0;
+    for (const PLin* l : {&pu.a, &pu.b})
+        for (int v : {(int)l->w, l->in_off, l->ld, l->KH, l->items, l->chunks, l->kh0, l->KHT}) *out++ = v;
+}
+FixKey key_of(const Cfg& c, const ChainPlan& p, bool with_front) {
+    return FixKey{p.pre, p.rg, p.pair, p.pre == PRE_SLABS && with_front ? 1 : 0, (c.attn_in_rows + 63) / 64, (so_cols(c) + 63) / 64};
+}
+int find_fixed(const FixKey& k) {
+    for (int i = 0; i < N_FIX; ++i)
+        if (same_key(fix_key(i), k)) return i;
+    return -1;
+}
+int fixed_match(const ChainPlan& p, const FixKey& k) {
+    static const bool ab_env = getenv("SBEV_CHAIN_TIE_SMALL") || getenv("SBEV_CHAIN_PAIR_Q0") || getenv("SBEV_CHAIN_RG") || getenv("SBEV_CHAIN_PAIR16");
+    const int fix = ab_env ? -1 : find_fixed(k);
+    if (fix < 0 || kFixedUnits[fix].n_units != p.n_units) return -1;
+    for (int mem = 0; mem <= p.pair; ++mem)
+        for (int u = 0; u < p.n_units; ++u) {
+            int32_t a[18], b[18];
+            unit_words(p.units[mem][u], a);
+            unit_words(kFixedUnits[fix].units[mem][u], b);
+            if (memcmp(a, b, sizeof(a)) != 0) return -1;
+        }
+    return fix;
+}
 
 int device_cus() {
     static std::atomic<int> cus[64];
@@ -1045,10 +1277,9 @@
     return a;
 }
 
-static Lin bound(const PLin& l, const float* pk) { return Lin{l.w < 0 ? nullptr : pk + l.w, l.in_off, l.ld, l.KH, l.items, l.chunks, l.kh0, l.KHT}; }
-
-static int launch(const ChainPlan& p, ChainArgs& a, const float* pk, hipStream_t s, const char* what) {
-    Inst& in = *find_inst(p.pre, p.rg, p.pair);
+static int launch(const Cfg& c, const ChainPlan& p, ChainArgs& a, const float* pk, hipStream_t s, const char* what) {
+    const int fix = g_chain_fixed.load(std::memory_order_relaxed) ? fixed_match(p, key_of(c, p, a.front != 0)) : -1;
+    Inst& in = *find_inst(p.pre, p.rg, p.pair, fix);
     const hipError_t attr = raise_lds(in);
     if (attr != hipSuccess) {
         set_error("%s: hipFuncSetAttribute(%d bytes of LDS): %s", what, in.lds, hipGetErrorString(attr));
@@ -1074,7 +1305,15 @@
     a.trace = tr + (calls % 64) * 512;
     if (calls < 13) who[calls] = &in;
 #endif
-    hipLaunchKernelGGL(in.kern, dim3(p.grid), dim3(64 * NWAVE), in.lds, s, a);
+    if (fix >= 0) {
+        ChainArgsFx f{};
+        static_cast<ChainCommon&>(f) = a;
+        f.image = pk;
+        g_chain_fixed_launches.fetch_add(1, std::memory_order_relaxed);
+        hipLaunchKernelGGL(in.kern_fx, dim3(p.grid), dim3(64 * NWAVE), in.lds, s, f);
+    } else {
+        hipLaunchKernelGGL(in.kern, dim3(p.grid), dim3(64 * NWAVE), in.lds, s, a);
+    }
 #ifdef SBEV_CHAIN_TRACE
     if (++calls == 13) {
         (void)hipDeviceSynchronize();
@@ -1100,7 +1339,7 @@
                        float* qkvt, float eps, hipStream_t s, uint32_t* skip_hdr) {
     ChainArgs a = chain_args(c, eps);
     a.bbox = bbox; a.feat = feat; a.x = x; a.qkvt = qkvt; a.skip_hdr = skip_hdr;
-    return launch(chain_plan(c, PRE_FRONT, false, false, 0), a, w.chain_pack, s, "row chain (front)");
+    return launch(c, chain_plan(c, PRE_FRONT, false, false, 0), a, w.chain_pack, s, "row chain (front)");
 }
 
 int launch_chain_attn(const sbev_decoder_config& c, const sbev_decoder_weights& w, const float* att, const float* x, float* x1,
@@ -1114,7 +1353,7 @@
     a.proj = sbev_ops::sample_point_args(bbox, time_diff, lidar2img, c.pc_range, c.B, c.Q, c.T, c.N, c.G, c.P, c.L, c.image_h, c.image_w,
                                          c.eps_homo, loc_bp, w_bp);
     if (touch && touch_need) sbev_ops::sample_point_touch(a.proj, *touch, c.hw, touch_need);
-    return launch(chain_plan(c, PRE_ATT, false, false, 0), a, w.chain_pack, s, "row chain (attention)");
+    return launch(c, chain_plan(c, PRE_ATT, false, false, 0), a, w.chain_pack, s, "row chain (attention)");
 }
 
 int launch_chain_tail(const sbev_decoder_config& c, const sbev_decoder_weights& w, const float* slabs, int splits, const float* x1,
@@ -1130,7 +1369,7 @@
         a.pair_sync = pair_sync;
         a.debug_drop = g_chain_pair_drop.load(std::memory_order_relaxed);
     }
-    return launch(p, a, w.chain_pack, s, p.pair ? "row chain (tail, pairs)" : "row chain (tail)");
+    return launch(c, p, a, w.chain_pack, s, p.pair ? "row chain (tail, pairs)" : "row chain (tail)");
 }
 
 }
@@ -1144,24 +1383,37 @@
     return pack_map(*cfg).total();
 }
 
+extern "C" int sbev_decoder_chain_fixed(int enable) { return g_chain_fixed.exchange(enable != 0 ? 1 : 0); }
+extern "C" int64_t sbev_decoder_chain_fixed_launches(void) { return g_chain_fixed_launches.load(std::memory_order_relaxed); }
+
+static int plan_words(const ChainPlan& p, const PlanUnits& t, int32_t* out, int capacity, const char* who) {
+    const int members = p.pair ? 2 : 1;
+    const long long words = 12 + 18LL * members * t.n_units;
+    SBEV_REQUIRE(out && capacity >= words, "%s: %lld words needed", who, words);
+    for (int v : {p.pre, p.rg, p.pair, (int)p.grid, p.lds, t.n_units, p.n_pairs, (int)p.warm, p.warm_lines, (int)p.vec, p.vec_off, p.vec_n}) *out++ = v;
+    for (int mem = 0; mem < members; ++mem)
+        for (int u = 0; u < t.n_units; ++u, out += 18) unit_words(t.units[mem][u], out);
+    return (int)words;
+}
+
+static bool plan_args_ok(const sbev_decoder_config* cfg, int kind, int cus) {
+    return cfg && sbev::row_chain_supported(*cfg) && cfg->B >= 1 && cfg->Q >= 1 && (long long)cfg->B * cfg->Q <= 256 * 16 && kind >= PRE_SLABS &&
+           kind <= PRE_ATT && cus >= 0;
+}
+
+extern "C" int sbev_decoder_chain_fixed_plan(const sbev_decoder_config* cfg, int kind, int with_front, int pair_ok, int cus, int32_t* out, int capacity) {
+    if (!plan_args_ok(cfg, kind, cus)) return 0;
+    const ChainPlan p = chain_plan(*cfg, kind, with_front != 0, pair_ok != 0, cus);
+    const int fix = find_fixed(key_of(*cfg, p, with_front != 0));
+    if (fix < 0) return 0;
+    return plan_words(p, kFixedUnits[fix], out, capacity, "sbev_decoder_chain_fixed_plan");
+}
+
 extern "C" int sbev_decoder_chain_plan(const sbev_decoder_config* cfg, int kind, int with_front, int pair_ok, int cus, int32_t* out, int capacity) {
-    SBEV_REQUIRE(cfg && sbev::row_chain_supported(*cfg) && cfg->B >= 1 && cfg->Q >= 1 && (long long)cfg->B * cfg->Q <= 256 * 16 &&
-                     kind >= PRE_SLABS && kind <= PRE_ATT && cus >= 0,
+    SBEV_REQUIRE(plan_args_ok(cfg, kind, cus),
                  "sbev_decoder_chain_plan: config not covered by the row chains (1 .. 4096 rows), or kind / cus out of range");
     const ChainPlan p = chain_plan(*cfg, kind, with_front != 0, pair_ok != 0, cus);
-    const int members = p.pair ? 2 : 1;
-    const long long words = 12 + 18LL * members * p.n_units;
-    SBEV_REQUIRE(out && capacity >= words, "sbev_decoder_chain_plan: %lld words needed", words);
-    for (int v : {p.pre, p.rg, p.pair, (int)p.grid, p.lds, p.n_units, p.n_pairs, (int)p.warm, p.warm_lines, (int)p.vec, p.vec_off, p.vec_n}) *out++ = v;
-    for (int mem = 0; mem < members; ++mem)
-        for (int u = 0; u < p.n_units; ++u) {
-            const PUnit& pu = p.units[mem][u];
-            *out++ = pu.epi;
-            *out++ = pu.col0;
-            for (const PLin* l : {&pu.a, &pu.b})
-                for (int v : {(int)l->w, l->in_off, l->ld, l->KH, l->items, l->chunks, l->kh0, l->KHT}) *out++ = v;
-        }
-    return (int)words;
+    return plan_words(p, p, out, capacity, "sbev_decoder_chain_plan");
 }
 
 extern "C" int sbev_decoder_chain_pack(const sbev_decoder_config* cfg, const sbev_decoder_weights* w, float* out, sbev_stream_t stream) {
diff --git a/sparsebev_amd/runtime.py b/sparsebev_amd/runtime.py
--- a/sparsebev_amd/runtime.py
+++ b/sparsebev_amd/runtime.py
@@ -724,6 +724,14 @@
     return bool(_lib.load().sbev_decoder_chain_pair(int(bool(enable))))
 
 
+def chain_fixed(enable):
+    return bool(_lib.load().sbev_decoder_chain_fixed(int(bool(enable))))
+
+
+def chain_fixed_launches():
+    return int(_lib.load().sbev_decoder_chain_fixed_launches())
+
+
 def _on_pair_fault():
     lib = _lib.load()
     lib.sbev_decoder_chain_pair(0)
```
